# XiandaGuo/OpenStereo

Measured on NVIDIA H100. Metric: stereo_pairs_per_sec_gwcnet_256x512_d192, higher is better.
Workload: dtype f32

## Files before the change

include/openstereo_b200.h:

```cpp
#ifndef OPENSTEREO_B200_H_
#define OPENSTEREO_B200_H_

#include <stddef.h>
#include <stdint.h>

#ifdef __cplusplus
extern "C" {
#endif

#define OSB_OK 0
#define OSB_EINVAL 1
#define OSB_ECUDA 2
#define OSB_EUNSUPPORTED 3

#define OSB_ACT_NONE 0
#define OSB_ACT_RELU 1
#define OSB_ACT_LEAKY 2
#define OSB_ACT_RELU6 3

typedef void* osb_stream_t;

int osb_abi_version(void);
const char* osb_last_error(void);
uint64_t osb_launch_count(void);
int osb_tc_overflow_count(osb_stream_t stream, int reset, unsigned int* count);
int osb_tc_overflow_poll(osb_stream_t stream, unsigned int* host_pinned);
const unsigned int* osb_tc_overflow_flag(void);
float osb_set_rz_kappa(float kappa);
int osb_set_persistent_grid_cap(int cap);
const char* osb_tc_last_variant(void);
const char* osb_volume_last_variant(void);


int osb_gwc_volume_fwd(const float* ref, const float* tgt, float* out, int B, int C, int H, int W,
                       int D, int G, osb_stream_t stream);

int osb_concat_volume_fwd(const float* ref, const float* tgt, float* out, int B, int C, int H,
                          int W, int D, int mask_left, osb_stream_t stream);

int osb_gwc_concat_volume_fwd(const float* ref_gwc, const float* tgt_gwc, const float* ref_cat,
                              const float* tgt_cat, float* out, int B, int Cg, int Cc, int H, int W,
                              int D, int G, osb_stream_t stream);

int osb_corr_volume_fwd(const float* left, const float* right, float* out, int B, int C, int H,
                        int W, int D, osb_stream_t stream);


int osb_softargmin_fwd(const float* cost, float* out, int B, int D, int H, int W, float alpha,
                       float start, float step, int normalize, osb_stream_t stream);

int osb_upsample_softargmin_fwd(const float* cost, float* out, int B, int Dl, int Hl, int Wl, int D,
                                int H, int W, int align_corners, osb_stream_t stream);

int osb_upsample_softargmin_values_fwd(const float* cost, const float* values, float* out, int B, int Dl, int Hl, int Wl,
                                       int D, int H, int W, int align_corners, osb_stream_t stream);

int osb_epe_partial_fwd(const float* pred, const float* gt, float* out, int B, int HW, float maxdisp,
                        osb_stream_t stream);


int osb_conv3d_k3_bn_act_fwd(const float* x, const float* w_packed, const float* scale,
                             const float* shift, const float* residual, const float* gate, float* y,
                             int B, int Cin, int Cout, int D, int H, int W, int stride, int act,
                             osb_stream_t stream);

int osb_deconv3d_bn_act_fwd(const float* x, const float* w_packed, const float* scale,
                            const float* shift, const float* residual, float* y, int B, int Cin,
                            int Cout, int D, int H, int W, int kernel, int act, osb_stream_t stream);

int osb_conv3d_1x1_bn_act_fwd(const float* x0, const float* x1, int Cin0, const float* w_packed,
                              const float* scale, const float* shift, const float* residual,
                              const float* gate, float* y, int B, int Cin, int Cout, int D, int H,
                              int W, int act, int sigmoid_out, osb_stream_t stream);


int osb_conv3d_tc_supported(int Cin, int Cout, int W, int stride);
#define OSB_TC_MIN_WIDTH 24
int osb_tc_general_width(int W);
int osb_conv3d_tc_kc(int Cin, int Cout, int W, int stride);
int osb_conv3d_k3_tc_fwd(const float* x_ndhwc, const void* w_split, const float* scale, const float* shift,
                         const float* residual, float* y, int B, int Cin, int Cout, int D, int H, int W, int act,
                         int out_ndhwc, int res_ndhwc, osb_stream_t stream);
int osb_conv3d_k3_tc_gate_fwd(const float* x_ndhwc, const void* w_split, const float* scale, const float* shift,
                              const float* residual, const float* gate_nhwc, float* y, int B, int Cin, int Cout, int D, int H, int W,
                              int act, osb_stream_t stream);
int osb_conv3d_k3_tc_ncdhw_fwd(const float* x_ncdhw, const void* w_split, const float* scale, const float* shift,
                               const float* residual, float* y, int B, int Cin, int Cout, int D, int H, int W, int act,
                               int out_ndhwc, int res_ndhwc, osb_stream_t stream);
#define OSB_LAYOUT_NCDHW 0
#define OSB_LAYOUT_NDHWC 1
#define OSB_LAYOUT_SPLIT 2
int osb_ncdhw_to_split(const float* x, float* y_split, int B, int C, int D, int H, int W, osb_stream_t stream);
int osb_conv3d_k3_tc_split_fwd(const float* x, const void* w_split, const float* scale, const float* shift, const float* residual,
                               float* y, int B, int Cin, int Cout, int D, int H, int W, int act, int in_layout, int out_layout,
                               int res_layout, osb_stream_t stream);
int osb_conv3d_s2_tc_supported(int Cin, int Cout, int D, int H, int W);
int osb_conv3d_k3_s2_tc_fwd(const float* x_ndhwc, const void* w_split, const float* scale, const float* shift,
                            const float* residual, float* y, int B, int Cin, int Cout, int D, int H, int W, int act,
                            int out_ndhwc, int res_ndhwc, osb_stream_t stream);
int osb_deconv3d_tc_supported(int Cin, int Cout, int W);
int osb_deconv3d_k3_tc_fwd(const float* x_ndhwc, const void* w_split, const float* scale, const float* shift,
                           const float* residual, float* y, int B, int Cin, int Cout, int D, int H, int W, int act,
                           int out_ndhwc, int res_ndhwc, osb_stream_t stream);
int osb_deconv3d_k4_tc_supported(int Cin, int Cout, int W);
int osb_deconv3d_k4_tc_fwd(const float* x_ndhwc, const void* w_split, const float* scale, const float* shift,
                           const float* residual, float* y, int B, int Cin, int Cout, int cout_real, int D, int H, int W, int act,
                           int out_ndhwc, int res_ndhwc, osb_stream_t stream);
int osb_conv3d_k3_tc_cs_fwd(const float* x_ndhwc, const void* w_split, const float* scale, const float* shift, const float* residual,
                            const float* gate_nhwc, float* y, int B, int Cin, int Cout, int D, int H, int W, int act, int ystride,
                            osb_stream_t stream);
int osb_conv3d_k3_s2_tc_cs_fwd(const float* x_ndhwc, const void* w_split, const float* scale, const float* shift, float* y, int B,
                               int Cin, int Cout, int D, int H, int W, int act, int ystride, osb_stream_t stream);
int osb_deconv3d_k4_tc_cs_fwd(const float* x_ndhwc, const void* w_split, const float* scale, const float* shift, float* y, int B,
                              int Cin, int Cout, int D, int H, int W, int act, int ystride, osb_stream_t stream);
int osb_conv1x1_ndhwc_cat_fwd(const float* x0, const float* x1, int C0, int C1, const float* w_packed, const float* scale,
                              const float* shift, float* y, long long voxels, int Cout, int act, osb_stream_t stream);
int osb_conv1x1_ndhwc_fwd(const float* x, const float* w_packed, const float* scale, const float* shift, float* y,
                          long long voxels, int Cin, int Cout, int act, osb_stream_t stream);
int osb_conv3d_k3_c1_ndhwc_fwd(const float* x_ndhwc, const float* w_taps, const float* scale, const float* shift, float* y, int B,
                               int Cin, int D, int H, int W, osb_stream_t stream);
int osb_conv2d_tc_kc(int Cin, int Cout, int W, int dilation);
int osb_conv2d_k3_tc_fwd(const float* x_nhwc, const void* w_split, const float* scale, const float* shift, const float* residual,
                         float* y, int B, int Cin, int Cout, int H, int W, int dilation, int act, int out_nhwc, int res_nhwc,
                         osb_stream_t stream);
int osb_gwc_volume_sum_fwd(const float* ref, const float* tgt, float* out, int B, int C, int H, int W, int D, int G,
                           osb_stream_t stream);
int osb_group_l2_normalize_fwd(const float* x, float* y, int B, int C, int H, int W, int G, float eps, osb_stream_t stream);
int osb_sub_volume_fwd(const float* left, const float* right, float* out, int B, int C, int H, int W, int D, osb_stream_t stream);
int osb_regression_values_fwd(const float* prob, const float* values, float* out, int B, int D, int H, int W, osb_stream_t stream);

int osb_warped_concat_volume_fwd(const float* x, const float* y, const float* disp, float* out, int B, int C, int D, int H, int W,
                                 int mask_left, osb_stream_t stream);
int osb_warped_gwc_concat_volume_fwd(const float* xg, const float* yg, const float* xc, const float* yc, const float* disp,
                                     float* out, int B, int Cg, int G, int Cc, int D, int H, int W, osb_stream_t stream);

int osb_coex_regression_fwd(const float* cost, const float* spx, float* out, int B, int D, int h, int w, int top_k, int spx_is_logits,
                            osb_stream_t stream);
int osb_nearest_resize3d_fwd(const float* x, float* y, int N, int Di, int Hi, int Wi, int Do, int Ho, int Wo, osb_stream_t stream);

int osb_mbv2_block3d_fwd(const float* x, const float* w_exp, const float* scale1, const float* shift1, const float* w_dw,
                         const float* scale2, const float* shift2, const float* w_proj, const float* scale3, const float* shift3,
                         const float* residual, float* y, int B, int Cin, int Chid, int Cout, int D, int H, int W, int stride,
                         int in_layout, int out_layout, osb_stream_t stream);

int osb_gwc_volume_bwd(const float* grad_vol, const float* ref, const float* tgt, float* grad_ref, float* grad_tgt, int B, int C,
                       int H, int W, int D, int G, int reduce_sum, osb_stream_t stream);
int osb_concat_volume_bwd(const float* grad_vol, float* grad_ref, float* grad_tgt, int B, int C, int H, int W, int D, int mask_left,
                          osb_stream_t stream);
int osb_softargmin_bwd(const float* cost, const float* grad_out, float* grad_cost, int B, int D, int H, int W, float alpha,
                       float start, float step, int normalize, osb_stream_t stream);

int osb_dwconv2d_fwd(const float* x, const float* w, const float* scale, const float* shift, const float* residual, float* y, int B,
                     int C, int H, int W, int KH, int KW, int stride, int act, osb_stream_t stream);
int osb_deconv2d_k3s2_fwd(const float* x, const float* w_packed, const float* scale, const float* shift, const float* residual,
                          float* y, int B, int Cin, int Cout, int H, int W, int act, osb_stream_t stream);

int osb_avgpool_pairs_fwd(const float* x, float* y, long long outer, int n, long long inner, osb_stream_t stream);
int osb_geo_lookup_fwd(const float* geo0, const float* geo1, const float* geo2, const float* geo3, const float* corr0,
                       const float* corr1, const float* corr2, const float* corr3, const float* disp, const float* coords,
                       float* out, int B, int C, int D, int H, int W, int W2, int num_levels, int radius, osb_stream_t stream);
int osb_context_upsample_fwd(const float* disp_low, const float* up_weights, float* out, int B, int h, int w, int scale,
                             osb_stream_t stream);
int osb_ncdhw_to_ndhwc(const float* x, float* y, int B, int C, int D, int H, int W, osb_stream_t stream);
int osb_ncdhw_to_ndhwc_pad(const float* x, float* y, int B, int C, int Cpad, int D, int H, int W, osb_stream_t stream);
int osb_feature_att_gate_fwd(const float* feat_nchw, const float* w1_packed, const float* scale1, const float* shift1,
                             const float* w2_packed, const float* scale2, const float* shift2, float* gate_nhwc, int B,
                             int Cf, int Ch, int Cv, int Cpad, int HW, int act1, osb_stream_t stream);

#ifdef __cplusplus
}
#endif
#endif
```

openstereo_b200/_lib.py:

```python
import ctypes
import os

_PKG = os.path.dirname(os.path.abspath(__file__))
LIB_PATH = os.path.join(_PKG, "lib", "libopenstereo_b200.so")

_f32p = ctypes.c_void_p
_i = ctypes.c_int
_f = ctypes.c_float
_s = ctypes.c_void_p

SIGNATURES = {
    "osb_gwc_volume_fwd": [_f32p, _f32p, _f32p, _i, _i, _i, _i, _i, _i, _s],
    "osb_concat_volume_fwd": [_f32p, _f32p, _f32p, _i, _i, _i, _i, _i, _i, _s],
    "osb_gwc_concat_volume_fwd": [_f32p, _f32p, _f32p, _f32p, _f32p, _i, _i, _i, _i, _i, _i, _i, _s],
    "osb_corr_volume_fwd": [_f32p, _f32p, _f32p, _i, _i, _i, _i, _i, _s],
    "osb_softargmin_fwd": [_f32p, _f32p, _i, _i, _i, _i, _f, _f, _f, _i, _s],
    "osb_upsample_softargmin_fwd": [_f32p, _f32p, _i, _i, _i, _i, _i, _i, _i, _i, _s],
    "osb_epe_partial_fwd": [_f32p, _f32p, _f32p, _i, _i, _f, _s],
    "osb_conv3d_k3_bn_act_fwd": [_f32p] * 7 + [_i] * 8 + [_s],
    "osb_deconv3d_bn_act_fwd": [_f32p] * 6 + [_i] * 8 + [_s],
    "osb_conv3d_1x1_bn_act_fwd": [_f32p, _f32p, _i] + [_f32p] * 6 + [_i] * 8 + [_s],
    "osb_conv3d_tc_supported": [_i, _i, _i, _i],
    "osb_conv3d_tc_kc": [_i, _i, _i, _i],
    "osb_tc_general_width": [_i],
    "osb_conv3d_s2_tc_supported": [_i, _i, _i, _i, _i],
    "osb_deconv3d_tc_supported": [_i, _i, _i],
    "osb_deconv3d_k3_tc_fwd": [_f32p] * 6 + [_i] * 9 + [_s],
    "osb_conv3d_k3_s2_tc_fwd": [_f32p] * 6 + [_i] * 9 + [_s],
    "osb_conv3d_k3_tc_fwd": [_f32p] * 6 + [_i] * 9 + [_s],
    "osb_conv3d_k3_tc_ncdhw_fwd": [_f32p] * 6 + [_i] * 9 + [_s],
    "osb_conv3d_k3_tc_split_fwd": [_f32p] * 6 + [_i] * 10 + [_s],
    "osb_ncdhw_to_split": [_f32p, _f32p] + [_i] * 5 + [_s],
    "osb_conv3d_k3_tc_gate_fwd": [_f32p] * 7 + [_i] * 7 + [_s],
    "osb_deconv3d_k4_tc_supported": [_i, _i, _i],
    "osb_conv3d_k3_tc_cs_fwd": [_f32p] * 7 + [_i] * 8 + [_s],
    "osb_conv3d_k3_s2_tc_cs_fwd": [_f32p] * 5 + [_i] * 8 + [_s],
    "osb_deconv3d_k4_tc_cs_fwd": [_f32p] * 5 + [_i] * 8 + [_s],
    "osb_deconv3d_k4_tc_fwd": [_f32p] * 6 + [_i] * 10 + [_s],
    "osb_conv1x1_ndhwc_cat_fwd": [_f32p, _f32p, _i, _i, _f32p, _f32p, _f32p, _f32p, ctypes.c_longlong, _i, _i, _s],
    "osb_feature_att_gate_fwd": [_f32p] * 8 + [_i] * 7 + [_s],
    "osb_ncdhw_to_ndhwc_pad": [_f32p, _f32p, _i, _i, _i, _i, _i, _i, _s],
    "osb_conv1x1_ndhwc_fwd": [_f32p] * 5 + [ctypes.c_longlong, _i, _i, _i, _s],
    "osb_conv3d_k3_c1_ndhwc_fwd": [_f32p] * 5 + [_i] * 5 + [_s],
    "osb_avgpool_pairs_fwd": [_f32p, _f32p, ctypes.c_longlong, _i, ctypes.c_longlong, _s],
    "osb_geo_lookup_fwd": [_f32p] * 11 + [_i] * 8 + [_s],
    "osb_context_upsample_fwd": [_f32p] * 3 + [_i] * 4 + [_s],
    "osb_conv2d_tc_kc": [_i] * 4,
    "osb_conv2d_k3_tc_fwd": [_f32p] * 6 + [_i] * 9 + [_s],
    "osb_ncdhw_to_ndhwc": [_f32p, _f32p, _i, _i, _i, _i, _i, _s],
    "osb_gwc_volume_sum_fwd": [_f32p, _f32p, _f32p, _i, _i, _i, _i, _i, _i, _s],
    "osb_group_l2_normalize_fwd": [_f32p, _f32p, _i, _i, _i, _i, _i, _f, _s],
    "osb_sub_volume_fwd": [_f32p, _f32p, _f32p, _i, _i, _i, _i, _i, _s],
    "osb_regression_values_fwd": [_f32p, _f32p, _f32p, _i, _i, _i, _i, _s],
    "osb_gwc_volume_bwd": [_f32p] * 5 + [_i] * 7 + [_s],
    "osb_concat_volume_bwd": [_f32p] * 3 + [_i] * 6 + [_s],
    "osb_softargmin_bwd": [_f32p] * 3 + [_i] * 4 + [_f, _f, _f, _i, _s],
    "osb_dwconv2d_fwd": [_f32p] * 6 + [_i] * 8 + [_s],
    "osb_deconv2d_k3s2_fwd": [_f32p] * 6 + [_i] * 6 + [_s],
    "osb_upsample_softargmin_values_fwd": [_f32p] * 3 + [_i] * 8 + [_s],
    "osb_warped_concat_volume_fwd": [_f32p] * 4 + [_i] * 6 + [_s],
    "osb_warped_gwc_concat_volume_fwd": [_f32p] * 6 + [_i] * 7 + [_s],
    "osb_coex_regression_fwd": [_f32p] * 3 + [_i] * 6 + [_s],
    "osb_nearest_resize3d_fwd": [_f32p] * 2 + [_i] * 7 + [_s],
    "osb_mbv2_block3d_fwd": [_f32p] * 12 + [_i] * 10 + [_s],
}


class NativeLibraryError(RuntimeError):
    pass


def _load():
    if not os.path.exists(LIB_PATH):
        raise NativeLibraryError(
            "%s not found: build it with `python -m openstereo_b200.build` (there is no CPU/PyTorch fallback)"
            % LIB_PATH)
    lib = ctypes.CDLL(LIB_PATH)
    lib.osb_abi_version.restype = ctypes.c_int
    lib.osb_last_error.restype = ctypes.c_char_p
    lib.osb_launch_count.restype = ctypes.c_uint64
    lib.osb_tc_overflow_count.argtypes = [ctypes.c_void_p, ctypes.c_int, ctypes.POINTER(ctypes.c_uint)]
    lib.osb_tc_overflow_count.restype = ctypes.c_int
    lib.osb_tc_overflow_poll.argtypes = [ctypes.c_void_p, ctypes.c_void_p]
    lib.osb_tc_overflow_poll.restype = ctypes.c_int
    lib.osb_tc_overflow_flag.argtypes = []
    lib.osb_tc_overflow_flag.restype = ctypes.c_void_p
    lib.osb_set_rz_kappa.argtypes = [ctypes.c_float]
    lib.osb_set_rz_kappa.restype = ctypes.c_float
    lib.osb_set_persistent_grid_cap.argtypes = [ctypes.c_int]
    lib.osb_set_persistent_grid_cap.restype = ctypes.c_int
    lib.osb_tc_last_variant.argtypes = []
    lib.osb_tc_last_variant.restype = ctypes.c_char_p
    lib.osb_volume_last_variant.argtypes = []
    lib.osb_volume_last_variant.restype = ctypes.c_char_p
    for name, argtypes in SIGNATURES.items():
        try:
            fn = getattr(lib, name)
        except AttributeError as exc:
            raise NativeLibraryError("%s does not export %s" % (LIB_PATH, name)) from exc
        fn.argtypes = argtypes
        fn.restype = ctypes.c_int
    return lib


lib = _load()

_ERRORS = {1: ValueError, 2: RuntimeError, 3: NotImplementedError}


def call(name, *args):
    if len(args) != len(SIGNATURES[name]):
        raise TypeError("%s takes %d arguments (%d given)" % (name, len(SIGNATURES[name]), len(args)))
    rc = getattr(lib, name)(*args)
    if rc != 0:
# ... 7 lines not shown
```

openstereo_b200/aggregation.py:

```python
import torch

from . import ops
from .ops import ACT_LEAKY, ACT_NONE, ACT_RELU, ACT_RELU6


class _Packed:
    __slots__ = ("w", "scale", "shift", "stride", "kernel", "transposed", "cin", "cout", "_w5", "_tc")

    def __init__(self, conv, bn=None):
        self._tc = {}
        self._w5 = conv.weight.detach() if conv.weight.dim() == 5 else None
        self.cin, self.cout = (conv.in_channels, conv.out_channels)
        self.transposed = isinstance(conv, (torch.nn.ConvTranspose3d, torch.nn.ConvTranspose2d))
        self.kernel = int(conv.kernel_size[0])
        self.stride = int(conv.stride[0])
        self._validate(conv)
        wt = conv.weight
        if wt.dim() == 4:
            wt = wt.unsqueeze(2)
        if self.transposed:
            self.w = ops.pack_deconv_weight(wt)
        else:
            self.w = ops.pack_conv_weight(wt)
        if self.kernel == 1:
            self.w = self.w.reshape(self.w.shape[0], self.w.shape[2]).contiguous()
        self.scale, self.shift = (None, None)
        if bn is not None:
            if bn.training:
                raise RuntimeError("BatchNorm folding is only valid in eval mode (call model.eval())")
            self.scale, self.shift = ops.fold_bn(bn)
        if getattr(conv, "bias", None) is not None:
            bias = conv.bias.detach().float()
            self.shift = bias.contiguous() if self.shift is None else (self.shift + bias * self.scale).contiguous()


def _packed_validate(self, conv):
    ks, st = tuple(conv.kernel_size), tuple(conv.stride)
    ok = len(set(ks)) == 1 and len(set(st)) == 1 and tuple(conv.dilation) == (1,) * len(ks) and conv.groups == 1
    if self.transposed:
        op = tuple(conv.output_padding)
        ok = ok and ((ks[0] == 3 and st[0] == 2 and tuple(conv.padding) == (1,) * len(ks) and op == (1,) * len(ks))
                     or (ks[0] == 4 and st[0] == 2 and tuple(conv.padding) == (1,) * len(ks) and op == (0,) * len(ks)))
    else:
        ok = ok and ks[0] in (1, 3) and st[0] in (1, 2) and tuple(conv.padding) == (ks[0] // 2,) * len(ks)
        ok = ok and getattr(conv, "padding_mode", "zeros") == "zeros"
    if not ok:
        raise NotImplementedError("openstereo_b200: no kernel for %r (supported: Conv k1/k3, stride 1/2, padding k//2, dilation 1, "
                                  "groups 1; ConvTranspose k3 s2 p1 op1 or k4 s2 p1)" % (conv,))


_Packed._validate = _packed_validate


def _conv(layer, x, act=ACT_NONE, residual=None, gate=None):
    if layer.kernel == 1:
        return ops.conv3d_1x1(x, layer.w, layer.scale, layer.shift, residual, gate, act)
    return ops.conv3d_k3(x, layer.w, layer.scale, layer.shift, residual, gate, layer.stride, act)


USE_TENSOR_CORES = True


def _tc_weight(layer, width):
    if not USE_TENSOR_CORES or layer.transposed or layer.kernel != 3 or layer.stride != 1 or layer._w5 is None:
        return None
    kc = ops.conv3d_tc_kc(layer.cin, layer.cout, width)
    if not kc:
        return None
    if kc not in layer._tc:
        layer._tc[kc] = ops.pack_tc_weight(layer._w5, kc, pad_cout_to=16 if layer.cout < 16 else None)
    return layer._tc[kc]


def _tc_ok(layer, width):
    return _tc_weight(layer, width) is not None


def _conv_tc(layer, x_ndhwc, act=ACT_NONE, residual=None, out_ndhwc=True, res_ndhwc=True, in_ncdhw=False, out_split=False):
    wt = _tc_weight(layer, x_ndhwc.shape[4] if in_ncdhw else x_ndhwc.shape[3])
    return ops.conv3d_k3_tc(x_ndhwc, wt, layer.scale, layer.shift, residual, act, out_ndhwc, res_ndhwc, in_ncdhw,
                            out_split=out_split)


def _split_chain_ok(width, *layers):
    return USE_TENSOR_CORES and all(ops.conv3d_tc_kc(l.cin, l.cout, width) == 32 for l in layers)


def _stem_in(layer, volume, act, out_split=False):
    if ops.conv3d_tc_kc(layer.cin, layer.cout, volume.shape[-1]) == 32:
        return _conv_tc(layer, volume, act, in_ncdhw=True, out_split=out_split)
    return _conv_tc(layer, ops.to_ndhwc(volume), act)


def _conv_auto(layer, x, act=ACT_NONE, residual=None):
    if layer.stride == 1 and _tc_ok(layer, x.shape[-1]):
        return _conv_tc(layer, ops.to_ndhwc(x), act, residual, out_ndhwc=False, res_ndhwc=False)
    if (USE_TENSOR_CORES and layer.stride == 2 and layer.kernel == 3 and not layer.transposed and layer._w5 is not None
            and ops.conv3d_s2_tc_supported(layer.cin, layer.cout, x.shape[2], x.shape[3], x.shape[4])):
        if "s2" not in layer._tc:
            layer._tc["s2"] = ops.pack_tc_weight(layer._w5, 16, kw_order=(1, 0, 2))
        return ops.conv3d_k3_s2_tc(ops.to_ndhwc(x), layer._tc["s2"], layer.scale, layer.shift, residual, act)
    return _conv(layer, x, act, residual)


def _deconv(layer, x, act=ACT_NONE, residual=None):
    if (USE_TENSOR_CORES and layer.transposed and layer.kernel == 3 and layer._w5 is not None
            and ops.deconv3d_tc_supported(layer.cin, layer.cout, x.shape[-1])):
        if "dc" not in layer._tc:
            layer._tc["dc"] = ops.pack_tc_deconv_weight(layer._w5)
        return ops.deconv3d_k3_tc(ops.to_ndhwc(x), layer._tc["dc"], layer.scale, layer.shift, residual, act)
    return ops.deconv3d(x, layer.w, layer.scale, layer.shift, residual, layer.kernel, act)


def _versions(module):
    return tuple(p._version for p in module.parameters()) + tuple(b._version for b in module.buffers())


class _Engine:

    def __init__(self, module):
        self.module = module
        self._stamp = None

    def _watch(self, device):
        if USE_TENSOR_CORES:
            mon = ops.TcOverflowMonitor.get(device)
            mon.check()
            return mon
        return None

    def _ensure(self, device):
        stamp = (str(device), _versions(self.module), tuple(p.data_ptr() for p in self.module.parameters()))
        if stamp != self._stamp:
            if self.module.training:
                raise RuntimeError("openstereo_b200 engines run inference only: call model.eval()")
            with torch.no_grad():
                self._pack()
            self._stamp = stamp

    @staticmethod
    def _check(x):
        if not x.is_cuda:
            raise RuntimeError("openstereo_b200: not implemented on the CPU (no fallback); move the model to CUDA")
        return x.detach().float().contiguous()


class _GwcHourglass:
    def __init__(self, m):
        self.conv1, self.conv2 = _Packed(m.conv1[0][0], m.conv1[0][1]), _Packed(m.conv2[0][0], m.conv2[0][1])
        self.conv3, self.conv4 = _Packed(m.conv3[0][0], m.conv3[0][1]), _Packed(m.conv4[0][0], m.conv4[0][1])
        self.conv5, self.conv6 = _Packed(m.conv5[0], m.conv5[1]), _Packed(m.conv6[0], m.conv6[1])
        self.redir1, self.redir2 = _Packed(m.redir1[0], m.redir1[1]), _Packed(m.redir2[0], m.redir2[1])

    def __call__(self, x):
        c1 = _conv_auto(self.conv1, x, ACT_RELU)
        c2 = _conv_auto(self.conv2, c1, ACT_RELU)
        c3 = _conv_auto(self.conv3, c2, ACT_RELU)
        c4 = _conv_auto(self.conv4, c3, ACT_RELU)
        c5 = _deconv(self.conv5, c4, ACT_RELU, residual=_conv(self.redir2, c2))
        return _deconv(self.conv6, c5, ACT_RELU, residual=_conv(self.redir1, x))


def _hg_channels_last_ok(hg, x_shape_ndhwc):
    if not USE_TENSOR_CORES:
        return False
    b, d, h, w, c = x_shape_ndhwc
    if d % 4 or h % 4 or w % 4:
        return False
    return (ops.conv3d_s2_tc_supported(hg.conv1.cin, hg.conv1.cout, d, h, w) and _tc_ok(hg.conv2, w // 2)
            and ops.conv3d_s2_tc_supported(hg.conv3.cin, hg.conv3.cout, d // 2, h // 2, w // 2) and _tc_ok(hg.conv4, w // 4)
            and ops.deconv3d_tc_supported(hg.conv5.cin, hg.conv5.cout, w // 4)
            and ops.deconv3d_tc_supported(hg.conv6.cin, hg.conv6.cout, w // 2)
            and (hg.redir1.cin, hg.redir1.cout) in ((32, 32), (64, 64)) and (hg.redir2.cin, hg.redir2.cout) in ((32, 32), (64, 64)))


def _s2_weight(layer):
    if "s2" not in layer._tc:
        layer._tc["s2"] = ops.pack_tc_weight(layer._w5, 16, kw_order=(1, 0, 2))
    return layer._tc["s2"]


def _dc_weight(layer):
    if "dc" not in layer._tc:
        layer._tc["dc"] = ops.pack_tc_deconv_weight(layer._w5)
    return layer._tc["dc"]


def _gwc_hourglass_channels_last(hg, x):
    c1 = ops.conv3d_k3_s2_tc(x, _s2_weight(hg.conv1), hg.conv1.scale, hg.conv1.shift, None, ACT_RELU, out_ndhwc=True)
    c2 = _conv_tc(hg.conv2, c1, ACT_RELU)
    c3 = ops.conv3d_k3_s2_tc(c2, _s2_weight(hg.conv3), hg.conv3.scale, hg.conv3.shift, None, ACT_RELU, out_ndhwc=True)
    c4 = _conv_tc(hg.conv4, c3, ACT_RELU)
    r2 = ops.conv1x1_ndhwc(c2, hg.redir2.w, hg.redir2.scale, hg.redir2.shift)
    c5 = ops.deconv3d_k3_tc(c4, _dc_weight(hg.conv5), hg.conv5.scale, hg.conv5.shift, r2, ACT_RELU, out_ndhwc=True, res_ndhwc=True)
    r1 = ops.conv1x1_ndhwc(x, hg.redir1.w, hg.redir1.scale, hg.redir1.shift)
    return ops.deconv3d_k3_tc(c5, _dc_weight(hg.conv6), hg.conv6.scale, hg.conv6.shift, r1, ACT_RELU, out_ndhwc=True, res_ndhwc=True)


def _classif3_channels_last(classif3, out):
    head0, cls = classif3
    width = out.shape[3]
    if _tc_ok(cls, width):
        mid = _conv_tc(head0, out, ACT_RELU, out_split=_split_chain_ok(width, head0, cls))
        return _conv_tc(cls, mid, ACT_NONE, out_ndhwc=False, res_ndhwc=False)
    if cls.cin == 32 and cls.cout == 1 and cls._w5 is not None and cls.stride == 1:
        if "c1" not in cls._tc:
            cls._tc["c1"] = ops.pack_c1_weight(cls._w5)
        head = _conv_tc(head0, out, ACT_RELU)
        return ops.conv3d_k3_c1_ndhwc(head, cls._tc["c1"], cls.scale, cls.shift)
    head = _conv_tc(head0, out, ACT_RELU, out_ndhwc=False)
    return _conv(cls, head)


class GwcAggregation(_Engine):

    def _pack(self):
        m = self.module
        self.dres0 = [_Packed(m.dres0[0][0], m.dres0[0][1]), _Packed(m.dres0[2][0], m.dres0[2][1])]
        self.dres1 = [_Packed(m.dres1[0][0], m.dres1[0][1]), _Packed(m.dres1[2][0], m.dres1[2][1])]
        self.hg = [_GwcHourglass(m.dres2), _GwcHourglass(m.dres3), _GwcHourglass(m.dres4)]
        self.classif3 = [_Packed(m.classif3[0][0], m.classif3[0][1]), _Packed(m.classif3[2])]

    def logits(self, volume):
        volume = self._check(volume)
        self._ensure(volume.device)
        width = volume.shape[-1]
        stem_tc = all(_tc_ok(l, width) for l in (self.dres0[0], self.dres0[1], self.dres1[0], self.dres1[1]))
        b, _, dd, hh, ww = volume.shape
        if stem_tc and _tc_ok(self.classif3[0], width) and all(_hg_channels_last_ok(hg, (b, dd, hh, ww, 32)) for hg in self.hg):
            split = _split_chain_ok(width, self.dres0[0], self.dres0[1], self.dres1[0], self.dres1[1])
            c = _conv_tc(self.dres0[1], _stem_in(self.dres0[0], volume, ACT_RELU, out_split=split), ACT_RELU, out_split=split)
            out = _conv_tc(self.dres1[1], _conv_tc(self.dres1[0], c, ACT_RELU, out_split=split), ACT_NONE, residual=c)
            for hg in self.hg:
                out = _gwc_hourglass_channels_last(hg, out)
            return _classif3_channels_last(self.classif3, out)
        if stem_tc:
            c = _conv_tc(self.dres0[1], _stem_in(self.dres0[0], volume, ACT_RELU), ACT_RELU)
            cost0 = _conv_tc(self.dres1[1], _conv_tc(self.dres1[0], c, ACT_RELU), ACT_NONE, residual=c, out_ndhwc=False)
        else:
            c = _conv(self.dres0[1], _conv(self.dres0[0], volume, ACT_RELU), ACT_RELU)
            cost0 = _conv(self.dres1[1], _conv(self.dres1[0], c, ACT_RELU), ACT_NONE, residual=c)
        out = cost0
        for hg in self.hg:
            out = hg(out)
        if _tc_ok(self.classif3[0], width):
            head = _conv_tc(self.classif3[0], ops.to_ndhwc(out), ACT_RELU, out_ndhwc=False)
        else:
            head = _conv(self.classif3[0], out, ACT_RELU)
        return _conv(self.classif3[1], head)

    def __call__(self, volume, h, w):
        mon = self._watch(volume.device)
        out = ops.upsample_softargmin(self.logits(volume), self.module.maxdisp, h, w, align_corners=False)
        if mon is not None:
            mon.poll()
        return out


class CascadeAggregation(GwcAggregation):

    def __call__(self, cost, fine_d, fine_h, fine_w, disp_range_samples):
        mon = self._watch(cost.device)
        assert tuple(disp_range_samples.shape[1:]) == (fine_d, fine_h, fine_w)
        out = ops.upsample_softargmin_values(self.logits(cost), disp_range_samples, align_corners=False)
        if mon is not None:
            mon.poll()
        return out


class _PSMHourglass:
    def __init__(self, m):
        self.conv1, self.conv2 = _Packed(m.conv1[0], m.conv1[1]), _Packed(m.conv2[0], m.conv2[1])
        self.conv3, self.conv4 = _Packed(m.conv3[0], m.conv3[1]), _Packed(m.conv4[0], m.conv4[1])
        self.conv5, self.conv6 = _Packed(m.conv5[0], m.conv5[1]), _Packed(m.conv6[0], m.conv6[1])

    def __call__(self, x, presqu, postsqu, skip):
        out = _conv_auto(self.conv1, x, ACT_RELU)
        pre = _conv_auto(self.conv2, out, ACT_RELU, residual=postsqu)
        out = _conv_auto(self.conv4, _conv_auto(self.conv3, pre, ACT_RELU), ACT_RELU)
        post = _deconv(self.conv5, out, ACT_RELU, residual=presqu if presqu is not None else pre)
        return _deconv(self.conv6, post, ACT_NONE, residual=skip), pre, post


def _psm_hg_channels_last_ok(hg, shape_ndhwc):
    if not USE_TENSOR_CORES:
        return False
    b, d, h, w, c = shape_ndhwc
    if d % 4 or h % 4 or w % 4 or any(l._w5 is None for l in (hg.conv1, hg.conv2, hg.conv3, hg.conv4, hg.conv5, hg.conv6)):
        return False
    return (ops.conv3d_s2_tc_supported(hg.conv1.cin, hg.conv1.cout, d, h, w) and _tc_ok(hg.conv2, w // 2)
            and ops.conv3d_s2_tc_supported(hg.conv3.cin, hg.conv3.cout, d // 2, h // 2, w // 2) and _tc_ok(hg.conv4, w // 4)
            and hg.conv5.kernel == 3 and hg.conv6.kernel == 3
            and ops.deconv3d_tc_supported(hg.conv5.cin, hg.conv5.cout, w // 4)
            and ops.deconv3d_tc_supported(hg.conv6.cin, hg.conv6.cout, w // 2))


def _psm_hourglass_channels_last(hg, x, presqu, postsqu, skip):
    out = ops.conv3d_k3_s2_tc(x, _s2_weight(hg.conv1), hg.conv1.scale, hg.conv1.shift, None, ACT_RELU, out_ndhwc=True)
    pre = _conv_tc(hg.conv2, out, ACT_RELU, residual=postsqu)
    out = ops.conv3d_k3_s2_tc(pre, _s2_weight(hg.conv3), hg.conv3.scale, hg.conv3.shift, None, ACT_RELU, out_ndhwc=True)
    out = _conv_tc(hg.conv4, out, ACT_RELU)
    post = ops.deconv3d_k3_tc(out, _dc_weight(hg.conv5), hg.conv5.scale, hg.conv5.shift, presqu if presqu is not None else pre, ACT_RELU,
                              out_ndhwc=True, res_ndhwc=True)
    out = ops.deconv3d_k3_tc(post, _dc_weight(hg.conv6), hg.conv6.scale, hg.conv6.shift, skip, ACT_NONE, out_ndhwc=True, res_ndhwc=True)
    return out, pre, post


class PSMAggregation(_Engine):

    def _pack(self):
        m = self.module
        self.dres0 = [_Packed(m.dres0[0][0], m.dres0[0][1]), _Packed(m.dres0[1][0], m.dres0[1][1])]
        self.dres1 = [_Packed(m.dres1[0][0], m.dres1[0][1]), _Packed(m.dres1[1][0], m.dres1[1][1])]
        self.hg = [_PSMHourglass(m.dres2), _PSMHourglass(m.dres3), _PSMHourglass(m.dres4)]
        self.heads = [[_Packed(c[0][0], c[0][1]), _Packed(c[1])] for c in (m.classif1, m.classif2, m.classif3)]

    def logits(self, raw_cost):
        raw_cost = self._check(raw_cost)
        self._ensure(raw_cost.device)
        width = raw_cost.shape[-1]
        stem_tc = all(_tc_ok(l, width) for l in (self.dres0[0], self.dres0[1], self.dres1[0], self.dres1[1]))
        b, _, dd, hh, ww = raw_cost.shape
        if (stem_tc and all(_psm_hg_channels_last_ok(hg, (b, dd, hh, ww, 32)) for hg in self.hg)
                and all(_tc_ok(a, width) and _tc_ok(bb, width) for a, bb in self.heads)):
            c = _conv_tc(self.dres0[1], _stem_in(self.dres0[0], raw_cost, ACT_RELU), ACT_RELU)
            cost0 = _conv_tc(self.dres1[1], _conv_tc(self.dres1[0], c, ACT_RELU), ACT_NONE, residual=c)
            out1, pre1, post1 = _psm_hourglass_channels_last(self.hg[0], cost0, None, None, cost0)
            out2, pre2, post2 = _psm_hourglass_channels_last(self.hg[1], out1, pre1, post1, cost0)
            out3, _, _ = _psm_hourglass_channels_last(self.hg[2], out2, pre2, post2, cost0)
            costs, prev = [], None
            for (a, bb), x in zip(self.heads, (out1, out2, out3)):
                prev = _conv_tc(bb, _conv_tc(a, x, ACT_RELU), ACT_NONE, residual=prev, out_ndhwc=False, res_ndhwc=False)
                costs.append(prev)
            return costs
        if stem_tc:
            c = _conv_tc(self.dres0[1], _stem_in(self.dres0[0], raw_cost, ACT_RELU), ACT_RELU)
            cost0 = _conv_tc(self.dres1[1], _conv_tc(self.dres1[0], c, ACT_RELU), ACT_NONE, residual=c, out_ndhwc=False)
        else:
            c = _conv(self.dres0[1], _conv(self.dres0[0], raw_cost, ACT_RELU), ACT_RELU)
            cost0 = _conv(self.dres1[1], _conv(self.dres1[0], c, ACT_RELU), ACT_NONE, residual=c)
        out1, pre1, post1 = self.hg[0](cost0, None, None, cost0)
        out2, pre2, post2 = self.hg[1](out1, pre1, post1, cost0)
        out3, pre3, post3 = self.hg[2](out2, pre2, post2, cost0)

        def head(i, x, prev):
            a, b = self.heads[i]
            if _tc_ok(a, width) and _tc_ok(b, width):
                return _conv_tc(b, _conv_tc(a, ops.to_ndhwc(x), ACT_RELU), ACT_NONE, residual=prev, out_ndhwc=False, res_ndhwc=False)
            if _tc_ok(a, width):
                return _conv(b, _conv_tc(a, ops.to_ndhwc(x), ACT_RELU, out_ndhwc=False), residual=prev)
            return _conv(b, _conv(a, x, ACT_RELU), residual=prev)

        cost1 = head(0, out1, None)
        cost2 = head(1, out2, cost1)
        cost3 = head(2, out3, cost2)
        return [cost1, cost2, cost3]

    def __call__(self, raw_cost):
        b, c, d, h, w = raw_cost.shape
        max_disp = self.module.max_disp
        mon = self._watch(raw_cost.device)
        out = [ops.upsample_softargmin(cost, max_disp, 4 * h, 4 * w, align_corners=True)
               for cost in self.logits(raw_cost)]
        if mon is not None:
            mon.poll()
        return out


class _FeatureAtt:
    def __init__(self, m):
        blk = m.feat_att[0].block
        self.a = _Packed(blk[0], blk[1])
        self.b = _Packed(m.feat_att[1])
        self.act = ACT_LEAKY if any(isinstance(l, torch.nn.LeakyReLU) for l in blk) else ACT_NONE

    def __call__(self, feat):
        hidden = ops.conv3d_1x1(feat, self.a.w, self.a.scale, self.a.shift, act=ACT_LEAKY)
        return ops.conv3d_1x1(hidden, self.b.w, self.b.scale, self.b.shift, sigmoid_out=True)


def _block(m):
    layers = list(m.block)
    bn = layers[1] if len(layers) > 1 and isinstance(layers[1], torch.nn.BatchNorm3d) else None
# ... 509 lines not shown
```

openstereo_b200/csrc/api.cu:

```cuda
#include <atomic>
#include <cstdarg>
#include <cstring>

#include "common.cuh"

namespace osb {

static thread_local char g_error[512] = "";
static std::atomic<uint64_t> g_launches{0};

void set_error(const char* fmt, ...) {
  va_list ap;
  va_start(ap, fmt);
  vsnprintf(g_error, sizeof(g_error), fmt, ap);
  va_end(ap);
}

static std::atomic<float> g_rz_kappa{1.57e-8f};
float rz_kappa() { return g_rz_kappa.load(std::memory_order_relaxed); }

static std::atomic<int> g_grid_cap{0};
long long cap_persistent_grid(long long grid) {
  const int cap = g_grid_cap.load(std::memory_order_relaxed);
  return (cap > 0 && grid > cap) ? cap : grid;
// ... 18 lines not shown
  unsigned int* fresh = nullptr;
  if (cudaMalloc(&fresh, sizeof(unsigned int)) != cudaSuccess || cudaMemset(fresh, 0, sizeof(unsigned int)) != cudaSuccess) {
    set_error("tc_overflow_flag: %s", cudaGetErrorString(cudaGetLastError()));
    return nullptr;
  }
  unsigned int* expected = nullptr;
  if (!g_overflow[dev].compare_exchange_strong(expected, fresh, std::memory_order_acq_rel)) {
    (void)cudaFree(fresh);
    return expected;
  }
  return fresh;
}

int device_index() {
  int dev = 0;
  if (cudaGetDevice(&dev) != cudaSuccess) {
    (void)cudaGetLastError();
    return 0;
  }
  return dev;
}

int sm_count() {
  static std::atomic<int> cache[64];
  const int dev = device_index();
  int n = cache[dev & 63].load(std::memory_order_relaxed);
  if (n > 0) return n;
  if (cudaDeviceGetAttribute(&n, cudaDevAttrMultiProcessorCount, dev) != cudaSuccess || n <= 0) {
    (void)cudaGetLastError();
    n = 132;
  }
  cache[dev & 63].store(n, std::memory_order_relaxed);
  return n;
}

void count_launch(int n) { g_launches.fetch_add((uint64_t)n, std::memory_order_relaxed); }

int check_launch(const char* what) {
  cudaError_t e = cudaGetLastError();
  if (e == cudaSuccess) return OSB_OK;
  set_error("%s: launch failed: %s", what, cudaGetErrorString(e));
  return OSB_ECUDA;
}

typedef CUresult (*EncodeTiledFn)(CUtensorMap*, CUtensorMapDataType, cuuint32_t, void*, const cuuint64_t*,
                                  const cuuint64_t*, const cuuint32_t*, const cuuint32_t*, CUtensorMapInterleave,
                                  CUtensorMapSwizzle, CUtensorMapL2promotion, CUtensorMapFloatOOBfill);

static EncodeTiledFn encode_fn() {
  static EncodeTiledFn fn = [] {
    void* p = nullptr;
    cudaDriverEntryPointQueryResult q;
    cudaError_t e = cudaGetDriverEntryPoint("cuTensorMapEncodeTiled", &p, cudaEnableDefault, &q);
    if (e != cudaSuccess || q != cudaDriverEntryPointSuccess) {
      (void)cudaGetLastError();
      return (EncodeTiledFn) nullptr;
    }
    return reinterpret_cast<EncodeTiledFn>(p);
  }();
  return fn;
}

bool make_tensor_map_3d(CUtensorMap* out, const void* base, uint64_t d0, uint64_t d1, uint64_t d2, uint64_t stride1_bytes,
                        uint64_t stride2_bytes, uint32_t box0, uint32_t box1, uint32_t box2) {
  EncodeTiledFn fn = encode_fn();
  if (!fn) {
    set_error("cuTensorMapEncodeTiled not available from the driver");
    return false;
  }
  const cuuint64_t dims[3] = {d0, d1, d2};
  const cuuint64_t strides[2] = {stride1_bytes, stride2_bytes};
  const cuuint32_t box[3] = {box0, box1, box2};
  const cuuint32_t elem[3] = {1, 1, 1};
  CUresult r = fn(out, CU_TENSOR_MAP_DATA_TYPE_FLOAT32, 3, const_cast<void*>(base), dims, strides, box, elem,
                  CU_TENSOR_MAP_INTERLEAVE_NONE, CU_TENSOR_MAP_SWIZZLE_NONE, CU_TENSOR_MAP_L2_PROMOTION_L2_128B,
                  CU_TENSOR_MAP_FLOAT_OOB_FILL_NONE);
  if (r != CUDA_SUCCESS) {
    set_error("cuTensorMapEncodeTiled failed with CUresult %d", (int)r);
    return false;
  }
  return true;
}

bool make_tensor_map_split(CUtensorMap* out, const void* base, int C, int W, int H, int BD, int kc) {
  EncodeTiledFn fn = encode_fn();
  if (!fn) {
    set_error("cuTensorMapEncodeTiled not available from the driver");
    return false;
  }
  const uint64_t vox = 2ull * C * sizeof(uint16_t);
  const cuuint64_t dims[4] = {2ull * C, (cuuint64_t)W, (cuuint64_t)H, (cuuint64_t)BD};
  const cuuint64_t strides[3] = {vox, vox * W, vox * W * H};
  const cuuint32_t box[4] = {2u * kc, (cuuint32_t)W, 1, 1};
  const cuuint32_t elem[4] = {1, 1, 1, 1};
  CUresult r = fn(out, CU_TENSOR_MAP_DATA_TYPE_FLOAT16, 4, const_cast<void*>(base), dims, strides, box, elem,
                  CU_TENSOR_MAP_INTERLEAVE_NONE, kc == 32 ? CU_TENSOR_MAP_SWIZZLE_128B : CU_TENSOR_MAP_SWIZZLE_64B,
                  CU_TENSOR_MAP_L2_PROMOTION_L2_128B, CU_TENSOR_MAP_FLOAT_OOB_FILL_NONE);
  if (r != CUDA_SUCCESS) {
    set_error("cuTensorMapEncodeTiled (split activations) failed with CUresult %d", (int)r);
    return false;
  }
  return true;
}

}

extern "C" {
int osb_abi_version(void) { return 1; }
const char* osb_last_error(void) { return osb::g_error; }
uint64_t osb_launch_count(void) { return osb::g_launches.load(std::memory_order_relaxed); }
float osb_set_rz_kappa(float kappa) {
  const float old = osb::g_rz_kappa.load(std::memory_order_relaxed);
  if (kappa >= 0.f && kappa < 1e-6f) osb::g_rz_kappa.store(kappa, std::memory_order_relaxed);
  return old;
}
int osb_set_persistent_grid_cap(int cap) { return osb::g_grid_cap.exchange(cap > 0 ? cap : 0, std::memory_order_relaxed); }
const char* osb_tc_last_variant(void) { return osb::g_tc_variant; }
int osb_tc_overflow_count(osb_stream_t stream, int reset, unsigned int* count) {
  using namespace osb;
  OSB_REQUIRE(count, "tc_overflow_count: null pointer");
  unsigned int* flag = tc_overflow_flag();
  if (!flag) return OSB_ECUDA;
  cudaStream_t st = (cudaStream_t)stream;
  cudaError_t e = cudaMemcpyAsync(count, flag, sizeof(unsigned int), cudaMemcpyDeviceToHost, st);
  if (e == cudaSuccess && reset) e = cudaMemsetAsync(flag, 0, sizeof(unsigned int), st);
  if (e == cudaSuccess) e = cudaStreamSynchronize(st);
  if (e != cudaSuccess) {
    set_error("tc_overflow_count: %s", cudaGetErrorString(e));
    return OSB_ECUDA;
  }
  return OSB_OK;
}
const unsigned int* osb_tc_overflow_flag(void) { return osb::tc_overflow_flag(); }
int osb_tc_overflow_poll(osb_stream_t stream, unsigned int* host_pinned) {
  using namespace osb;
  OSB_REQUIRE(host_pinned, "tc_overflow_poll: null pointer");
  unsigned int* flag = tc_overflow_flag();
  if (!flag) return OSB_ECUDA;
  cudaError_t e = cudaMemcpyAsync(host_pinned, flag, sizeof(unsigned int), cudaMemcpyDeviceToHost, (cudaStream_t)stream);
  if (e != cudaSuccess) {
    set_error("tc_overflow_poll: %s", cudaGetErrorString(e));
    return OSB_ECUDA;
  }
  return OSB_OK;
}
}
```

openstereo_b200/csrc/common.cuh:

```cuda
#pragma once
#include <cuda.h>
#include <cuda_runtime.h>
#include <stdint.h>
#include <stdio.h>

#include <string>

#include "../../include/openstereo_b200.h"

namespace osb {

void set_error(const char* fmt, ...);
void count_launch(int n = 1);
int check_launch(const char* what);
int device_index();
int sm_count();
long long cap_persistent_grid(long long grid);
std::string tc_variant_name(const char* fmt, ...);
void set_tc_variant(const char* name);
struct PerDeviceFlag {
  bool done[64] = {};
  bool& here() { return done[device_index() & 63]; }
};

#define OSB_REQUIRE(cond, ...)          \
  do {                                  \
    if (!(cond)) {                      \
      ::osb::set_error(__VA_ARGS__);    \
      return OSB_EINVAL;                \
    }                                   \
  } while (0)

__device__ __forceinline__ uint32_t smem_u32(const void* p) {
  return static_cast<uint32_t>(__cvta_generic_to_shared(p));
}

__device__ __forceinline__ void mbar_init(uint64_t* bar, uint32_t count) {
  asm volatile("mbarrier.init.shared::cta.b64 [%0], %1;" ::"r"(smem_u32(bar)), "r"(count));
}
__device__ __forceinline__ void fence_mbar_init() {
  asm volatile("fence.mbarrier_init.release.cluster;" ::: "memory");
}
__device__ __forceinline__ void fence_proxy_async() {
  asm volatile("fence.proxy.async.shared::cta;" ::: "memory");
}
__device__ __forceinline__ void mbar_arrive_expect_tx(uint64_t* bar, uint32_t bytes) {
  asm volatile("mbarrier.arrive.expect_tx.shared::cta.b64 _, [%0], %1;" ::"r"(smem_u32(bar)), "r"(bytes)
               : "memory");
}
__device__ __forceinline__ void mbar_wait(uint64_t* bar, uint32_t parity) {
  asm volatile(
      "{\n"
      ".reg .pred p;\n"
      "WAIT_LOOP:\n"
      "mbarrier.try_wait.parity.shared::cta.b64 p, [%0], %1;\n"
      "@p bra DONE;\n"
      "bra WAIT_LOOP;\n"
      "DONE:\n"
      "}\n" ::"r"(smem_u32(bar)),
      "r"(parity)
      : "memory");
}
__device__ __forceinline__ void tma_load_3d(void* smem_dst, const CUtensorMap* map, uint64_t* bar, int c0,
                                            int c1, int c2) {
  asm volatile(
      "cp.async.bulk.tensor.3d.shared::cluster.global.mbarrier::complete_tx::bytes [%0], [%1, {%3, %4, %5}], [%2];"
      ::"r"(smem_u32(smem_dst)),
      "l"(reinterpret_cast<uint64_t>(map)), "r"(smem_u32(bar)), "r"(c0), "r"(c1), "r"(c2)
      : "memory");
}
__device__ __forceinline__ void tma_load_4d(void* smem_dst, const CUtensorMap* map, uint64_t* bar, int c0, int c1, int c2, int c3) {
  asm volatile(
      "cp.async.bulk.tensor.4d.shared::cluster.global.mbarrier::complete_tx::bytes [%0], [%1, {%3, %4, %5, %6}], [%2];"
      ::"r"(smem_u32(smem_dst)),
      "l"(reinterpret_cast<uint64_t>(map)), "r"(smem_u32(bar)), "r"(c0), "r"(c1), "r"(c2), "r"(c3)
      : "memory");
}
__device__ __forceinline__ void tma_prefetch_desc(const CUtensorMap* map) {
  asm volatile("prefetch.tensormap [%0];" ::"l"(reinterpret_cast<uint64_t>(map)) : "memory");
}

__device__ __forceinline__ void st_cs_f4(float* p, float4 v) { __stcs(reinterpret_cast<float4*>(p), v); }

bool make_tensor_map_3d(CUtensorMap* out, const void* base, uint64_t d0, uint64_t d1, uint64_t d2, uint64_t stride1_bytes,
                        uint64_t stride2_bytes, uint32_t box0, uint32_t box1, uint32_t box2);
bool make_tensor_map_split(CUtensorMap* out, const void* base, int C, int W, int H, int BD, int kc);

}
```

openstereo_b200/csrc/conv3d_tc.cu:

```cuda
#include <type_traits>

#include "tc_common.cuh"

namespace osb {

constexpr int TC_W = 128;
constexpr int TC_KC = 32;
constexpr int TC_TILES = TC_WGS;
constexpr int TC_ROWS = TC_TILES + 2;
constexpr int TC_STAGES = 4;
constexpr int TC_RAW = 2;
constexpr int TC_ROW_BYTES = TC_W * TC_KC * 4;

struct TcParams {
  CUtensorMap xmap;
  const float* x;
  const void* w;
  const float* scale;
  const float* shift;
  const float* residual;
  float* y;
  int B, D, H, Cin, Cout;
  int act;
  float kappa;
// ... 283 lines not shown
          const int din = d + kd - 1;
          if (din < 0 || din >= p.D) continue;
          for (int ch = 0; ch < nchunk; ++ch, ++phc) {
            for (int kh = 0; kh < 3; ++kh) {
              const uint32_t slot = (phc & 1) * 3 + kh;
              const size_t slice = ((size_t)kd * nchunk + ch) * 3 + kh;
              mbar_wait_relaxed(&b_empty[slot], ((phc >> 1) & 1) ^ 1);
              mbar_arrive_expect_tx(&b_full[slot], B_SLICE);
              bulk_g2s(b_buf + slot * B_SLICE, wsrc + slice * B_SLICE, B_SLICE, &b_full[slot]);
            }
          }
        }
      }
    }
    else if (warp == 4 * TC_WGS + 5 && p.bulk_rows && elect_one()) {
      RowIter ld{(int)blockIdx.x, 0, 0, -1};
      if (ld.it < p.items) ld.kd = (((ld.it / p.hblocks) % p.D) == 0) ? 1 : 0;
      uint32_t rawc = 0;
      while (advance(ld)) {
        const int hb = ld.it % p.hblocks;
        const int d = (ld.it / p.hblocks) % p.D;
        const int b = ld.it / (p.hblocks * p.D);
        const int hin = hb * TC_TILES - 1 + ld.r, din = d + ld.kd - 1;
        const uint32_t slot = rawc % TC_RAW, par = (rawc / TC_RAW) & 1;
        mbar_wait_relaxed(&raw_empty[slot], par ^ 1);
        if (hin >= 0 && hin < p.H && p.in_ncdhw) {
          const size_t plane = (size_t)p.D * p.H * TC_W;
          const float* src = p.x + (((size_t)b * p.Cin + ld.ch * TC_KC) * p.D + din) * p.H * TC_W + (size_t)hin * TC_W;
          mbar_arrive_expect_tx(&raw_full[slot], TC_ROW_BYTES);
          for (int c = 0; c < TC_KC; ++c)
            bulk_g2s(raw_buf + slot * TC_ROW_BYTES + c * (TC_W * 4), src + c * plane, TC_W * 4, &raw_full[slot]);
        } else if (hin >= 0 && hin < p.H) {
          const float* src = p.x + (((size_t)b * p.D + din) * p.H + hin) * (size_t)(TC_W * TC_KC);
          mbar_arrive_expect_tx(&raw_full[slot], TC_ROW_BYTES);
          bulk_g2s(raw_buf + slot * TC_ROW_BYTES, src, TC_ROW_BYTES, &raw_full[slot]);
        } else {
          mbar_arrive(&raw_full[slot]);
        }
        ++rawc;
      }
    }
    __syncwarp();
  }
}

__global__ void __launch_bounds__(256) ncdhw_to_ndhwc_kernel(const float* __restrict__ x, float* __restrict__ y, int C, int Cp,
                                                             size_t vol, uint16_t* __restrict__ ys, unsigned int* overflow) {
  __shared__ float tile[32][33];
  const int b = blockIdx.z;
  const size_t v0 = (size_t)blockIdx.x * 32;
  const int c0 = blockIdx.y * 32;
  const int tx = threadIdx.x & 31, ty = threadIdx.x >> 5;
  float amax = 0.f;
  for (int i = ty; i < 32; i += 8) {
    const int c = c0 + i;
    const size_t v = v0 + tx;
    tile[i][tx] = (c < C && v < vol) ? __ldg(x + ((size_t)b * C + c) * vol + v) : 0.f;
  }
  __syncthreads();
  for (int i = ty; i < 32; i += 8) {
    const size_t v = v0 + i;
    const int c = c0 + tx;
    if (c >= Cp || v >= vol) continue;
    if (!ys) {
      y[((size_t)b * vol + v) * Cp + c] = tile[tx][i];
      continue;
    }
    const float s = tile[tx][i] * TC_ACT_SCALE;
    const uint32_t hl = cvt_f16x2_sat(s, s - f16x2_to_float2(cvt_f16x2_sat(s, 0.f)).x);
    uint16_t* vox = ys + ((size_t)b * vol + v) * 2 * Cp;
    vox[split_index(c)] = (uint16_t)(hl & 0xFFFFu);
    vox[split_index(c) + SPLIT_GRANULE] = (uint16_t)(hl >> 16);
    amax = fmaxf(amax, fabsf(s));
  }
  if (ys) tc_report_overflow(overflow, amax);
}

template <int COUT>
int launch_tc(const TcArgs& a, cudaStream_t stream) {
  TcParams p{};
  p.Cout = a.Cout, p.in_ncdhw = a.in_ncdhw;
  p.in_split = a.in_split, p.out_split = a.out_split, p.res_split = a.res_split;
  p.bulk_rows = !a.in_split && (a.in_ncdhw || a.Cin == TC_KC);
  if (a.in_split && !make_tensor_map_split(&p.xmap, a.x, a.Cin, TC_W, a.H, a.B * a.D, TC_KC)) return OSB_ECUDA;
  p.hblocks = (a.H + TC_TILES - 1) / TC_TILES;
  static const std::string variant = tc_variant_name("tc<%d>", COUT);
  return launch_persistent<conv3d_tc_kernel<COUT>>(a, p, (long long)a.B * a.D * p.hblocks, TcCfg<COUT>::SMEM, variant.c_str(), stream);
}
template int launch_tc<32>(const TcArgs&, cudaStream_t);
template int launch_tc<16>(const TcArgs&, cudaStream_t);

}

extern "C" {

int osb_tc_general_width(int W) { return W >= OSB_TC_MIN_WIDTH ? 1 : 0; }

int osb_conv3d_tc_kc(int Cin, int Cout, int W, int stride) {
  return stride == 1 ? osb::select_conv3d_tc(Cin, Cout, W, 1, false, false).kc : 0;
}

int osb_conv3d_tc_supported(int Cin, int Cout, int W, int stride) { return osb_conv3d_tc_kc(Cin, Cout, W, stride) != 0; }

int osb_ncdhw_to_ndhwc_pad(const float* x, float* y, int B, int C, int Cpad, int D, int H, int W, osb_stream_t stream) {
  using namespace osb;
  OSB_REQUIRE(x && y, "ncdhw_to_ndhwc: null pointer");
  OSB_REQUIRE(B > 0 && C > 0 && Cpad >= C && D > 0 && H > 0 && W > 0 && B <= 65535, "ncdhw_to_ndhwc: bad shape");
  const size_t vol = (size_t)D * H * W;
  dim3 grid((unsigned)((vol + 31) / 32), (Cpad + 31) / 32, B);
  ncdhw_to_ndhwc_kernel<<<grid, 256, 0, (cudaStream_t)stream>>>(x, y, C, Cpad, vol, nullptr, nullptr);
  count_launch();
  return check_launch("ncdhw_to_ndhwc_kernel");
}

int osb_ncdhw_to_split(const float* x, float* y_split, int B, int C, int D, int H, int W, osb_stream_t stream) {
  using namespace osb;
  OSB_REQUIRE(x && y_split, "ncdhw_to_split: null pointer");
  OSB_REQUIRE(B > 0 && C > 0 && C % SPLIT_GRANULE == 0 && D > 0 && H > 0 && W > 0 && B <= 65535,
              "ncdhw_to_split: bad shape (C must be a multiple of %d)", SPLIT_GRANULE);
  unsigned int* flag = tc_overflow_flag();
  if (!flag) return OSB_ECUDA;
  const size_t vol = (size_t)D * H * W;
  dim3 grid((unsigned)((vol + 31) / 32), (C + 31) / 32, B);
  ncdhw_to_ndhwc_kernel<<<grid, 256, 0, (cudaStream_t)stream>>>(x, nullptr, C, C, vol, reinterpret_cast<uint16_t*>(y_split), flag);
  count_launch();
  return check_launch("ncdhw_to_ndhwc_kernel");
}

int osb_ncdhw_to_ndhwc(const float* x, float* y, int B, int C, int D, int H, int W, osb_stream_t stream) {
  return osb_ncdhw_to_ndhwc_pad(x, y, B, C, C, D, H, W, stream);
}

static int conv3d_k3_tc_impl(osb::TcArgs a, int dilation, osb_stream_t stream) {
  using namespace osb;
  const int kc = select_conv3d_tc(a.Cin, a.Cout, a.W, dilation, false, false).kc;
  OSB_REQUIRE(kc, "conv3d_k3_tc: unsupported shape Cin=%d Cout=%d W=%d dilation=%d", a.Cin, a.Cout, a.W, dilation);
  OSB_REQUIRE(!a.in_ncdhw || kc == 32, "conv3d_k3_tc: NCDHW input is served by the W = 128 kernel only");
  OSB_REQUIRE((!a.ystride && !a.gate) || kc == 16, "conv3d_k3_tc: a channel slice or gate needs the 16-channel-chunk kernels");
  OSB_REQUIRE(a.Cout > 16 || (!a.out_ndhwc && (!a.residual || !a.res_ndhwc)), "conv3d_k3_tc: Cout <= 16 writes (and adds) NCDHW tensors only");
  OSB_REQUIRE(!(a.in_split || a.out_split || a.res_split) || (kc == 32 && !a.ystride && !a.gate),
              "conv3d_k3_tc: split activations are served by the W = 128 kernel only");
  OSB_REQUIRE(!a.in_split || !a.in_ncdhw, "conv3d_k3_tc: an input is either NCDHW or split");
  OSB_REQUIRE((!a.out_split || a.out_ndhwc) && (!a.res_split || a.res_ndhwc), "conv3d_k3_tc: split tensors are channels-last");
  OSB_REQUIRE(!(a.out_split || a.res_split) || (a.out_ndhwc && (!a.residual || a.res_ndhwc)),
              "conv3d_k3_tc: a split output or residual needs a channels-last output and residual");
  const TcLaunch launch = select_conv3d_tc(a.Cin, a.Cout, a.W, dilation, a.gate != nullptr, a.slice()).launch;
  const int rc = check_tc_args("conv3d_k3_tc", a, launch);
  return rc != OSB_OK ? rc : launch(a, (cudaStream_t)stream);
}

int osb_conv3d_k3_tc_fwd(const float* x_ndhwc, const void* w_split, const float* scale, const float* shift,
                         const float* residual, float* y, int B, int Cin, int Cout, int D, int H, int W, int act,
                         int out_ndhwc, int res_ndhwc, osb_stream_t stream) {
  return conv3d_k3_tc_impl({x_ndhwc, w_split, scale, shift, residual, nullptr, y, B, Cin, Cout, D, H, W, act, out_ndhwc, res_ndhwc, 0, 0,
                            Cout}, 1, stream);
}

int osb_conv3d_k3_tc_gate_fwd(const float* x_ndhwc, const void* w_split, const float* scale, const float* shift,
                              const float* residual, const float* gate_nhwc, float* y, int B, int Cin, int Cout, int D, int H, int W,
                              int act, osb_stream_t stream) {
  OSB_REQUIRE(gate_nhwc, "conv3d_k3_tc_gate: null gate");
  return conv3d_k3_tc_impl({x_ndhwc, w_split, scale, shift, residual, gate_nhwc, y, B, Cin, Cout, D, H, W, act, 1, 1, 0, 0, Cout}, 1,
                           stream);
}

int osb_conv3d_k3_tc_cs_fwd(const float* x_ndhwc, const void* w_split, const float* scale, const float* shift, const float* residual,
                            const float* gate_nhwc, float* y, int B, int Cin, int Cout, int D, int H, int W, int act, int ystride,
                            osb_stream_t stream) {
  return conv3d_k3_tc_impl({x_ndhwc, w_split, scale, shift, residual, gate_nhwc, y, B, Cin, Cout, D, H, W, act, 1, 1, 0, ystride, Cout},
                           1, stream);
}

int osb_conv3d_k3_tc_ncdhw_fwd(const float* x_ncdhw, const void* w_split, const float* scale, const float* shift,
                               const float* residual, float* y, int B, int Cin, int Cout, int D, int H, int W, int act,
                               int out_ndhwc, int res_ndhwc, osb_stream_t stream) {
  return conv3d_k3_tc_impl({x_ncdhw, w_split, scale, shift, residual, nullptr, y, B, Cin, Cout, D, H, W, act, out_ndhwc, res_ndhwc, 1, 0,
                            Cout}, 1, stream);
}

int osb_conv3d_k3_tc_split_fwd(const float* x, const void* w_split, const float* scale, const float* shift, const float* residual,
                               float* y, int B, int Cin, int Cout, int D, int H, int W, int act, int in_layout, int out_layout,
                               int res_layout, osb_stream_t stream) {
  auto known = [](int l) { return l == OSB_LAYOUT_NCDHW || l == OSB_LAYOUT_NDHWC || l == OSB_LAYOUT_SPLIT; };
  OSB_REQUIRE(known(in_layout) && known(out_layout) && known(res_layout), "conv3d_k3_tc_split: unknown layout");
  osb::TcArgs a{x, w_split, scale, shift, residual, nullptr, y, B, Cin, Cout, D, H, W, act, out_layout != OSB_LAYOUT_NCDHW, res_layout != OSB_LAYOUT_NCDHW,
                in_layout == OSB_LAYOUT_NCDHW, 0, Cout};
  a.in_split = in_layout == OSB_LAYOUT_SPLIT, a.out_split = out_layout == OSB_LAYOUT_SPLIT, a.res_split = res_layout == OSB_LAYOUT_SPLIT;
  return conv3d_k3_tc_impl(a, 1, stream);
}

int osb_conv2d_tc_kc(int Cin, int Cout, int W, int dilation) { return osb::select_conv3d_tc(Cin, Cout, W, dilation, false, false).kc; }

int osb_conv2d_k3_tc_fwd(const float* x_nhwc, const void* w_split, const float* scale, const float* shift, const float* residual,
                         float* y, int B, int Cin, int Cout, int H, int W, int dilation, int act, int out_nhwc, int res_nhwc,
                         osb_stream_t stream) {
  return conv3d_k3_tc_impl({x_nhwc, w_split, scale, shift, residual, nullptr, y, B, Cin, Cout, 1, H, W, act, out_nhwc, res_nhwc, 0, 0,
                            Cout}, dilation, stream);
}
}
```

openstereo_b200/csrc/conv3d_tcg.cu:

```cuda
#include "tc_common.cuh"

namespace osb {

struct TcgParams {
  const float* x;
  const void* w;
  const float* scale;
  const float* shift;
  const float* residual;
  const float* gate;
  float* y;
  int B, D, H, Cin;
  int act;
  float kappa;
  unsigned int* overflow;
  int out_ndhwc, res_ndhwc;
  int items, hblocks;
  int Wr, ctiles;
  int ystride;
};

template <int COUT, int KC, int W, int TILES, int DIL = 1, bool GW = false>
struct TcgCfg {
  static_assert(!GW || W == 128, "general-width tiles are 128-column segments of one image row");
  static constexpr int HALO = GW ? DIL : 0;
  static constexpr int CSTEP = 128 - 2 * HALO;
  static_assert(DIL == 1 || (W == 128 && DIL == 2 && COUT >= 64), "dilation 2 is instantiated for full-width rows only");
  static constexpr int R = 128 / W;
  static constexpr int ROWB = KC * 4;
  static constexpr int UNIT_BYTES = 128 * ROWB;
  static constexpr int N3 = 3 * COUT;
  static constexpr int G = 32;
  static constexpr int NG = COUT / G;
  static constexpr int NG3 = 3 * G;
  static constexpr int B_SLICE = N3 * ROWB;
  static constexpr int B_SUB = NG3 * ROWB;
  static constexpr int NT = TC_WGS * TILES;
  static constexpr int TS = R * DIL;
  static constexpr int HSPAN = NT * TS;
  __host__ __device__ static constexpr int row0(int hb) { return (hb / DIL) * HSPAN + (hb % DIL) * R; }
  __host__ static int hblocks(int H) { return DIL * ((H + HSPAN - 1) / HSPAN); }
  static constexpr int NLW = 4;
  static constexpr int XCHG_FLOATS = 2 * frag_xchg_floats<G, DIL>();
  static constexpr int FIXED_SMEM = 1024 + TC_BSLOTS * 3 * B_SUB + 1024 + TC_WGS * XCHG_FLOATS * 4 + 4 * TC_WGS * FRAG_TP_FLOATS * 4 +
                                    2 * COUT * 4;
  static constexpr int STAGES = (232448 - FIXED_SMEM) / UNIT_BYTES < 10 ? (232448 - FIXED_SMEM) / UNIT_BYTES : 10;
  static_assert(STAGES >= NLW, "the ring must hold at least one unit per loader warp");
  static constexpr int S_FIRST = -DIL;
  static constexpr int S_LAST = (NT - 1) * TS + DIL;
  static constexpr int KSTEPS = KC / 16;
  static constexpr int A_OFF = 0;
  static constexpr int B_OFF = A_OFF + STAGES * UNIT_BYTES;
  static constexpr int BAR_OFF = B_OFF + TC_BSLOTS * 3 * B_SUB;
  static constexpr int THREADS = TC_WG_THREADS;
  static constexpr size_t SMEM = 1024 + (size_t)BAR_OFF + 1024 + TC_WGS * XCHG_FLOATS * 4 + 4 * TC_WGS * FRAG_TP_FLOATS * 4 + 2 * COUT * 4;
  static_assert(SMEM <= 232448, "shared memory budget of one CTA exceeded");
  static_assert(TILES == 1, "a consumer warpgroup holds one accumulator tile");
  static_assert(DIL == 1 || R == 1, "interleaved row blocks assume one image row per tile");
  static_assert(COUT % G == 0, "output channels come in groups of 32");
  static_assert(B_SUB % 1024 == 0 && UNIT_BYTES % 1024 == 0, "operand tiles must stay 1024-byte aligned");
  static constexpr int tile_of(int s, int kh) {
    const int num = s - (kh - 1) * DIL;
    return (num >= 0 && num % TS == 0 && num / TS < NT) ? num / TS : -1;
  }
  static constexpr bool used(int s) { return tile_of(s, 0) >= 0 || tile_of(s, 1) >= 0 || tile_of(s, 2) >= 0; }
  static constexpr int units_per_phase() {
    int n = 0;
    for (int s = S_FIRST; s <= S_LAST; ++s) n += used(s) ? 1 : 0;
    return n;
  }
  static constexpr int NU = units_per_phase();
  static constexpr int unit_s(int j) {
    int k = 0;
    for (int s = S_FIRST; s <= S_LAST; ++s)
      if (used(s)) {
        if (k == j) return s;
        ++k;
      }
    return S_LAST;
  }
};

template <int COUT, int KC, int W, int TILES, int DIL = 1, bool GW = false, bool GATE = false>
__global__ void __launch_bounds__(TcgCfg<COUT, KC, W, TILES, DIL, GW>::THREADS, 1) conv3d_tcg_kernel(const TcgParams p) {
  using C = TcgCfg<COUT, KC, W, TILES, DIL, GW>;
  extern __shared__ __align__(1024) uint8_t smem_raw[];
  uint8_t* smem = reinterpret_cast<uint8_t*>((reinterpret_cast<uintptr_t>(smem_raw) + 1023) & ~static_cast<uintptr_t>(1023));
  uint8_t* a_buf = smem + C::A_OFF;
  uint8_t* b_buf = smem + C::B_OFF;
  uint64_t* bars = reinterpret_cast<uint64_t*>(smem + C::BAR_OFF);
  uint64_t* a_ready = bars;
  uint64_t* a_empty = a_ready + C::STAGES;
  uint64_t* b_full = a_empty + C::STAGES;
  uint64_t* b_empty = b_full + TC_BSLOTS * 3;
  float* xchg = reinterpret_cast<float*>(smem + C::BAR_OFF + 1024);
  float* tiles = xchg + TC_WGS * C::XCHG_FLOATS;
  float* s_scale = tiles + 4 * TC_WGS * FRAG_TP_FLOATS;
  float* s_shift = s_scale + COUT;

  const int warp = threadIdx.x >> 5, lane = threadIdx.x & 31;
  const int nchunk = p.Cin / KC;
  const int Wp = GW ? p.Wr : W;
  const int YS = (W < 32 && p.ystride) ? p.ystride : COUT;
  const int ctiles = GW ? p.ctiles : 1;

  if (threadIdx.x == 0) {
    for (int s = 0; s < C::STAGES; ++s) {
      mbar_init(&a_ready[s], 32);
      mbar_init(&a_empty[s], 4 * TC_WGS);
    }
    for (int k = 0; k < TC_BSLOTS * 3; ++k) {
      mbar_init(&b_full[k], 1);
      mbar_init(&b_empty[k], 4 * TC_WGS);
    }
    fence_mbar_init();
  }
  for (int c = threadIdx.x; c < COUT; c += blockDim.x) {
    s_scale[c] = p.scale ? p.scale[c] : 1.f;
    s_shift[c] = p.shift ? p.shift[c] : 0.f;
  }
  __syncthreads();

  if (warp < 4 * TC_WGS) {
    setmaxnreg_inc<TC_CONSUMER_REGS>();
    const int wg = warp >> 2;
    xchg += wg * C::XCHG_FLOATS;
    const int bar_xchg = 1 + wg;
    const uint64_t dbase = (KC == 32) ? desc_sw128_base() : desc_sw64_base();
    constexpr uint32_t A_HALF = 64 * C::ROWB / 16;
    const uint32_t b16 = (smem_u32(b_buf) & 0x3FFFF) >> 4;
    const int q = warp & 3;
    uint32_t unitc = 0, phc = 0, exc = 0;
    for (int it = blockIdx.x; it < p.items; it += gridDim.x) {
      const int cg = (it % C::NG) * C::G;
      const int it0 = it / C::NG;
      const int ct = it0 % ctiles;
      const int hb = (it0 / ctiles) % p.hblocks;
      const int d = (it0 / (ctiles * p.hblocks)) % p.D;
      const int b = it0 / (ctiles * p.hblocks * p.D);
      auto tile_row = [&](int m, int& h, int& col) {
        h = C::row0(hb) + wg * C::TS + m / W;
        col = GW ? ct * C::CSTEP - C::HALO + m : m % W;
        return h < p.H && (!GW || (m >= C::HALO && m < 128 - C::HALO && col < Wp));
      };
      {
        int h, col;
        if (tile_row(q * 32 + lane, h, col)) {
          const ptrdiff_t vox = (((ptrdiff_t)b * p.D + d) * p.H + h) * Wp + col;
          if (p.residual && p.res_ndhwc) asm volatile("prefetch.global.L2 [%0];" ::"l"(p.residual + vox * YS + cg));
          if (GATE && p.gate) asm volatile("prefetch.global.L2 [%0];" ::"l"(p.gate + (((ptrdiff_t)b * p.H + h) * Wp + col) * YS + cg));
        }
      }
      float acc[2][C::NG3 / 2];
      uint32_t accum = 0;
      for (int kd = 0; kd < 3; ++kd) {
        const int din = d + kd - 1;
        if (din < 0 || din >= p.D) continue;
        for (int ch = 0; ch < nchunk; ++ch, ++phc) {
#pragma unroll
          for (int s = C::S_FIRST; s <= C::S_LAST; ++s) {
            if (!C::used(s)) continue;
            const uint32_t slot = unitc % C::STAGES, par = (unitc / C::STAGES) & 1;
            mbar_wait(&a_ready[slot], par);
            const uint64_t da0 = dbase | (uint64_t)((smem_u32(a_buf + slot * C::UNIT_BYTES) & 0x3FFFF) >> 4);
#pragma unroll
            for (int kh = 0; kh < 3; ++kh) {
              if (C::tile_of(s, kh) != wg) continue;
              const uint32_t bslot = (phc & 1) * 3 + kh;
              mbar_wait(&b_full[bslot], (phc >> 1) & 1);
              const uint64_t db0 = dbase | (uint64_t)(b16 + (bslot * C::B_SUB) / 16);
              wg_fence();
#pragma unroll
              for (int ks = 0; ks < C::KSTEPS; ++ks)
                wg_mma_split<C::NG3>(acc, da0 + TcK<KC>::A_KSTEP * ks, A_HALF, TcK<KC>::A_LO, db0 + 2 * ks, TcK<KC>::B_LO, ks > 0 ? 1u : accum);
              wg_commit();
              wg_wait_all();
              accum = 1;
              wg_release(&b_empty[bslot], lane);
            }
            wg_release(&a_empty[slot], lane);
            ++unitc;
          }
        }
      }
      const float corr = 1.f + p.kappa * (float)(((d > 0) + 1 + (d + 1 < p.D)) * nchunk * 3 * C::KSTEPS * 3);
      frag_unshift<C::G, DIL, W>(acc, xchg + (exc & 1) * (C::XCHG_FLOATS / 2), q, lane, corr, bar_xchg);
      ++exc;
      const size_t plane = (size_t)p.D * p.H * Wp;
      auto rows = [&](int m, ptrdiff_t& yo, ptrdiff_t& ro, ptrdiff_t& go) {
        int h, col;
        const bool ok = tile_row(m, h, col);
        const ptrdiff_t vox = (((ptrdiff_t)b * p.D + d) * p.H + h) * Wp + col;
        const ptrdiff_t ncdhw = (ptrdiff_t)b * COUT * plane + ((ptrdiff_t)d * p.H + h) * Wp + col;
        yo = p.out_ndhwc ? vox * YS : ncdhw;
        ro = p.res_ndhwc ? vox * YS : ncdhw;
        go = (((ptrdiff_t)b * p.H + h) * Wp + col) * YS;
        return ok;
      };
      frag_epilogue<C::G>(acc, lane, q, tiles + warp * FRAG_TP_FLOATS, s_scale + cg, s_shift + cg, p.act, p.y + (p.out_ndhwc ? (size_t)cg : cg * plane),
                          p.out_ndhwc ? 1 : plane, p.residual ? p.residual + (p.res_ndhwc ? (size_t)cg : cg * plane) : nullptr,
                          p.res_ndhwc ? 1 : plane, (GATE && p.gate) ? p.gate + cg : nullptr, rows, C::G);
    }
  }
  else if (warp < 4 * TC_WGS + C::NLW) {
    setmaxnreg_dec<TC_LOADER_REGS>();
    const int lw = warp - 4 * TC_WGS;
    static_assert(KC == 16, "lane_voxel / unit-row mapping below is written for 64-byte operand rows");
    constexpr int CPR = KC / 4;
    constexpr int VPL = 32 / CPR;
    constexpr int NLD = 128 / VPL;
    static_assert(W % VPL == 0, "a load instruction must not straddle image rows");
    const int v0 = lane_voxel<KC>(lane), c = lane % CPR;
    float amax = 0.f;
    uint32_t ubase = 0;
    int first = lw;
    auto fill = [&](const float* base, size_t rstride, size_t cstride, int h_first, int h_step, uint32_t u, int col0) {
      float4 v[NLD];
#pragma unroll
      for (int j = 0; j < NLD; ++j) {
        const int hin = h_first + h_step * ((VPL * j) / W);
        const size_t off = (size_t)((VPL * j) / W) * rstride + (size_t)((VPL * j) % W) * cstride;
        bool ok = hin >= 0 && hin < p.H;
        if (GW) ok = ok && (unsigned)(col0 + VPL * j) < (unsigned)Wp;
        v[j] = ok ? __ldg(reinterpret_cast<const float4*>(base + (ptrdiff_t)off)) : make_float4(0.f, 0.f, 0.f, 0.f);
      }
      const uint32_t slot = u % C::STAGES, ph = (u / C::STAGES) & 1;
      mbar_wait_relaxed(&a_empty[slot], ph ^ 1);
      uint8_t* tile = a_buf + slot * C::UNIT_BYTES;
#pragma unroll
      for (int j = 0; j < NLD; ++j) stage_f16_split<KC>(tile, v0 + VPL * j, c, v[j], amax);
      fence_proxy_async();
      mbar_arrive(&a_ready[slot]);
    };
    for (int it = blockIdx.x; it < p.items; it += gridDim.x) {
      const int it0 = it / C::NG;
      const int ct = it0 % ctiles;
      const int hb = (it0 / ctiles) % p.hblocks;
      const int d = (it0 / (ctiles * p.hblocks)) % p.D;
      const int b = it0 / (ctiles * p.hblocks * p.D);
      const int h0 = C::row0(hb);
      const int col0 = ct * C::CSTEP - C::HALO + v0;
      for (int kd = 0; kd < 3; ++kd) {
        const int din = d + kd - 1;
        if (din < 0 || din >= p.D) continue;
        const float* plane = p.x + ((size_t)b * p.D + din) * p.H * (size_t)Wp * p.Cin;
        for (int ch = 0; ch < nchunk; ++ch) {
#pragma unroll 1
          for (int j = first; j < C::NU; j += C::NLW) {
            const int s = C::unit_s(j);
            const float* base = plane + ((ptrdiff_t)(h0 + s) * Wp + col0) * p.Cin + ch * KC + c * 4;
            fill(base, (size_t)Wp * p.Cin, (size_t)p.Cin, h0 + s, 1, ubase + j, col0);
          }
          ubase += C::NU;
          first = (first + C::NLW - C::NU % C::NLW) % C::NLW;
        }
      }
    }
    tc_report_overflow(p.overflow, amax);
  }
  else {
    setmaxnreg_dec<TC_PRODUCER_REGS>();
    if (warp == 4 * TC_WGS + C::NLW && elect_one()) {
      const uint8_t* wsrc = reinterpret_cast<const uint8_t*>(p.w);
      uint32_t phc = 0;
      for (int it = blockIdx.x; it < p.items; it += gridDim.x) {
        const int cg = (it % C::NG) * C::G;
        const int d = (it / C::NG / (ctiles * p.hblocks)) % p.D;
        for (int kd = 0; kd < 3; ++kd) {
          const int din = d + kd - 1;
          if (din < 0 || din >= p.D) continue;
          for (int ch = 0; ch < nchunk; ++ch, ++phc) {
            for (int kh = 0; kh < 3; ++kh) {
              const uint32_t slot = (phc & 1) * 3 + kh;
              const size_t slice = ((size_t)kd * nchunk + ch) * 3 + kh;
              mbar_wait_relaxed(&b_empty[slot], ((phc >> 1) & 1) ^ 1);
              mbar_arrive_expect_tx(&b_full[slot], C::B_SUB);
#pragma unroll
              for (int kw = 0; kw < 3; ++kw)
                bulk_g2s(b_buf + slot * C::B_SUB + kw * C::G * C::ROWB, wsrc + slice * C::B_SLICE + (size_t)(kw * COUT + cg) * C::ROWB,
                         C::G * C::ROWB, &b_full[slot]);
            }
          }
        }
      }
    }
    __syncwarp();
  }
}

template <int COUT, int KC, int W, int TILES, int DIL = 1, bool GW = false, bool GATE = false>
static int launch_tcg(const TcArgs& a, cudaStream_t stream) {
  using C = TcgCfg<COUT, KC, W, TILES, DIL, GW>;
  TcgParams p{};
  p.gate = a.gate, p.ystride = a.ystride;
  p.hblocks = C::hblocks(a.H);
  p.Wr = GW ? a.W : W;
  p.ctiles = GW ? (a.W + C::CSTEP - 1) / C::CSTEP : 1;
  static const std::string variant = tc_variant_name("tcg<%d,%d,%d,%d,%d,%d,%d>", COUT, KC, W, TILES, DIL, (int)GW, (int)GATE);
  return launch_persistent<conv3d_tcg_kernel<COUT, KC, W, TILES, DIL, GW, GATE>>(
      a, p, (long long)a.B * a.D * p.hblocks * p.ctiles * C::NG, C::SMEM, variant.c_str(), stream);
}

TcRoute select_conv3d_tc(int Cin, int Cout, int W, int dilation, bool gate, bool slice) {
  if (dilation == 1 && W == 128 && Cin % 32 == 0 && Cin >= 32 && !gate && !slice) {
    if (Cout == 32) return {launch_tc<32>, 32};
    if (Cout >= 1 && Cout <= 16) return {launch_tc<16>, 32};
  }
  if (Cin % 16 != 0 || Cin < 16) return {};
  if (dilation == 2)
    return (W == 128 && Cout == 128 && !gate && !slice) ? TcRoute{launch_tcg<128, 16, 128, 1, 2>, 16} : TcRoute{};
  if (dilation != 1) return {};
  if (W == 16) {
    if (Cout == 96) return {launch_tcg<96, 16, 16, 1, 1, false, true>, 16};
    if (Cout == 64) return {launch_tcg<64, 16, 16, 1, 1, false, true>, 16};
    return {};
  }
  if (slice) return {};
  if (gate) {
    if (W == 64 && Cout == 64) return {launch_tcg<64, 16, 64, 1, 1, false, true>, 16};
    if (W == 32 && Cout == 96) return {launch_tcg<96, 16, 32, 1, 1, false, true>, 16};
    return {};
  }
  if (W == 64 && Cout == 64) return {launch_tcg<64, 16, 64, 1>, 16};
  if (W == 32 && Cout == 64) return {launch_tcg<64, 16, 32, 1>, 16};
  if (W == 32 && Cout == 128) return {launch_tcg<128, 16, 32, 1>, 16};
  if (W == 32 && Cout == 96) return {launch_tcg<96, 16, 32, 1>, 16};
  if (W == 128 && Cout == 64) return {launch_tcg<64, 16, 128, 1>, 16};
  if (W == 128 && Cout == 128) return {launch_tcg<128, 16, 128, 1>, 16};
  if (!osb_tc_general_width(W)) return {};
  if (Cout == 32) return {launch_tcg<32, 16, 128, 1, 1, true>, 16};
  if (Cout == 64) return {launch_tcg<64, 16, 128, 1, 1, true>, 16};
  if (Cout == 128) return {launch_tcg<128, 16, 128, 1, 1, true>, 16};
  return {};
}

}
```

openstereo_b200/csrc/conv3d_tcs2.cu:

```cuda
#include "tc_common.cuh"

namespace osb {

struct Tcs2Params {
  const float* x;
  const void* w;
  const float* scale;
  const float* shift;
  const float* residual;
  float* y;
  int B, D, H, Cin;
  int act;
  float kappa;
  unsigned int* overflow;
  int out_ndhwc, res_ndhwc;
  int items, hblocks;
  int Wr, ctiles;
  int ystride;
};

template <int COUT, int KC, int W, int TILES, bool GW = false>
struct Tcs2Cfg {
  static_assert(!GW || W == 128, "general-width tiles are 128-column segments of one output row");
  static constexpr int HALO = GW ? 1 : 0;
  static constexpr int CSTEP = 128 - HALO;
  static constexpr int R = 128 / W;
  static constexpr int ROWB = KC * 4;
  static constexpr int UNIT_BYTES = 128 * ROWB;
  static constexpr int N3 = 3 * COUT;
  static constexpr int G = 32;
  static constexpr int NG = COUT / G;
  static constexpr int NP = (NG + TC_WGS - 1) / TC_WGS;
  static constexpr int B_SLICE = N3 * ROWB;
  static constexpr int B_SUB = 3 * G * ROWB;
  static constexpr int B_SLOT = TC_WGS * B_SUB;
  static constexpr int PC = 16;
  static constexpr int NPASS = G / PC;
  static constexpr int LD = 3 * PC + 4;
  static constexpr int XCHG_FLOATS = 2 * 4 * PC;
  static constexpr int NLW = 4;
  static constexpr int FIXED_SMEM = 1024 + TC_BSLOTS * 3 * B_SLOT + TC_WGS * 128 * LD * 4 + 1024 + TC_WGS * XCHG_FLOATS * 4 + 3 * COUT * 4;
  static constexpr int STAGES = (232448 - FIXED_SMEM) / UNIT_BYTES < 10 ? (232448 - FIXED_SMEM) / UNIT_BYTES : 10;
  static_assert(STAGES >= NLW, "the ring must hold at least one unit per loader warp");
  static constexpr int NU = TILES * 3 * 2;
  static constexpr int HBLK = TILES * R;
  static constexpr int KSTEPS = KC / 16;
  static constexpr int A_OFF = 0;
  static constexpr int B_OFF = A_OFF + STAGES * UNIT_BYTES;
  static constexpr int STAGE_OFF = B_OFF + TC_BSLOTS * 3 * B_SLOT;
  static constexpr int BAR_OFF = STAGE_OFF + TC_WGS * 128 * LD * 4;
  static constexpr int THREADS = TC_WG_THREADS;
  static constexpr size_t SMEM = 1024 + (size_t)BAR_OFF + 1024 + TC_WGS * XCHG_FLOATS * 4 + 3 * COUT * 4;
  static_assert(SMEM <= 232448, "shared memory budget of one CTA exceeded");
  static_assert(TILES == 1, "a consumer warpgroup holds one accumulator tile");
  static_assert(COUT % G == 0, "output channels come in groups of 32");
  static_assert(32 * LD >= TP_WARP_FLOATS, "store_ndhwc_chunk32 transposes through the warp's own rows of the staging tile");
  static_assert(B_SUB % 1024 == 0 && UNIT_BYTES % 1024 == 0, "operand tiles must stay 1024-byte aligned");
};

template <int N>
__device__ __forceinline__ void s2_stage16(float* stage, int ld, const float (&acc)[2][N / 2], int c0, int dst, int wq, int lane) {
#pragma unroll
  for (int h = 0; h < 2; ++h) {
    float* r0 = stage + (64 * h + 16 * wq + (lane >> 2)) * ld + 2 * (lane & 3) + dst;
#pragma unroll
    for (int jj = 0; jj < 2; ++jj) {
      const int j = c0 / 8 + jj;
      *reinterpret_cast<float2*>(r0 + 8 * jj) = make_float2(acc[h][4 * j], acc[h][4 * j + 1]);
      *reinterpret_cast<float2*>(r0 + 8 * ld + 8 * jj) = make_float2(acc[h][4 * j + 2], acc[h][4 * j + 3]);
    }
  }
}

template <int COUT, int KC, int W, int TILES, bool GW = false>
__global__ void __launch_bounds__(Tcs2Cfg<COUT, KC, W, TILES, GW>::THREADS, 1) conv3d_tcs2_kernel(const Tcs2Params p) {
  using C = Tcs2Cfg<COUT, KC, W, TILES, GW>;
  extern __shared__ __align__(1024) uint8_t smem_raw[];
  uint8_t* smem = smem_raw + ((1024u - (smem_u32(smem_raw) & 1023u)) & 1023u);
  uint8_t* a_buf = smem + C::A_OFF;
  uint8_t* b_buf = smem + C::B_OFF;
  float* stage = reinterpret_cast<float*>(smem + C::STAGE_OFF);
  uint64_t* bars = reinterpret_cast<uint64_t*>(smem + C::BAR_OFF);
  uint64_t* a_ready = bars;
  uint64_t* a_empty = a_ready + C::STAGES;
  uint64_t* b_full = a_empty + C::STAGES;
  uint64_t* b_empty = b_full + TC_BSLOTS * 3;
  float* xchg = reinterpret_cast<float*>(smem + C::BAR_OFF + 1024);
  float* s_scale = xchg + TC_WGS * C::XCHG_FLOATS;
  float* s_shift = s_scale + COUT;
  float* zeros = s_shift + COUT;

  const int warp = threadIdx.x >> 5, lane = threadIdx.x & 31;
  const int nchunk = p.Cin / KC;
  const int Wp = GW ? p.Wr : W;
  const int YS = (W < 32 && p.ystride) ? p.ystride : COUT;
  const int ctiles = GW ? p.ctiles : 1;

  if (threadIdx.x == 0) {
    for (int s = 0; s < C::STAGES; ++s) {
      mbar_init(&a_ready[s], 32);
      mbar_init(&a_empty[s], 4 * TC_WGS);
// ... 38 lines not shown
      float acc_e[2][C::G / 2], acc_o[2][C::G];
      uint32_t accum_e = 0, accum_o = 0;
      for (int kd = 0; kd < 3; ++kd) {
        const int din = 2 * d + kd - 1;
        if (din < 0 || din >= p.D) continue;
        for (int ch = 0; ch < nchunk; ++ch, ++phc) {
#pragma unroll
          for (int kh = 0; kh < 3; ++kh) {
            const uint32_t bslot = (phc & 1) * 3 + kh;
#pragma unroll
            for (int par = 0; par < 2; ++par) {
              const uint32_t slot = unitc % C::STAGES, ph = (unitc / C::STAGES) & 1;
              mbar_wait(&a_ready[slot], ph);
              if (par == 0) mbar_wait(&b_full[bslot], (phc >> 1) & 1);
              if (has_group) {
                const uint64_t da0 = dbase | (uint64_t)((smem_u32(a_buf + slot * C::UNIT_BYTES) & 0x3FFFF) >> 4);
                const uint64_t db0 = dbase | (uint64_t)(b16 + (bslot * C::B_SLOT + wg * C::B_SUB + (par ? C::G * C::ROWB : 0)) / 16);
                wg_fence();
#pragma unroll
                for (int ks = 0; ks < C::KSTEPS; ++ks) {
                  if (par == 0) wg_mma_split<C::G>(acc_e, da0 + TcK<KC>::A_KSTEP * ks, A_HALF, TcK<KC>::A_LO, db0 + 2 * ks, TcK<KC>::B_LO, ks > 0 ? 1u : accum_e);
                  else wg_mma_split<2 * C::G>(acc_o, da0 + TcK<KC>::A_KSTEP * ks, A_HALF, TcK<KC>::A_LO, db0 + 2 * ks, TcK<KC>::B_LO, ks > 0 ? 1u : accum_o);
                }
                wg_commit();
                wg_wait_all();
                if (par == 0) accum_e = 1;
                else accum_o = 1;
              }
              wg_release(&a_empty[slot], lane);
              if (par == 1) wg_release(&b_empty[bslot], lane);
              ++unitc;
            }
          }
        }
      }
      if (!has_group) continue;
      const int h = hb * C::HBLK + rr;
      const bool live = h < Ho;
      const int col = GW ? ct * C::CSTEP - C::HALO + m : wcol;
      const bool cvalid = !GW || (m >= C::HALO && col < Wp);
      const uint32_t vmask = GW ? __ballot_sync(0xffffffffu, cvalid) : 0xffffffffu;
      const float corr = 1.f + p.kappa * (float)(((d > 0) + 1 + (2 * d + 1 < p.D)) * nchunk * 3 * C::KSTEPS * 3);
      const ptrdiff_t vox = (((ptrdiff_t)b * Do + d) * Ho + h) * Wp + col;
      const size_t plane = (size_t)Do * Ho * Wp;
      const ptrdiff_t ncdhw0 = (ptrdiff_t)b * COUT * plane + ((ptrdiff_t)d * Ho + h) * Wp + col;
      float out[32];
#pragma unroll
      for (int pass = 0; pass < C::NPASS; ++pass) {
        named_bar_sync(bar_stage, 128);
        s2_stage16<C::G>(stage, C::LD, acc_e, pass * C::PC, 0, q, lane);
        s2_stage16<2 * C::G>(stage, C::LD, acc_o, pass * C::PC, C::PC, q, lane);
        s2_stage16<2 * C::G>(stage, C::LD, acc_o, C::G + pass * C::PC, 2 * C::PC, q, lane);
        named_bar_sync(bar_stage, 128);
        const float* srow = stage + m * C::LD;
        float* xb = xchg + (exc & 1) * (4 * C::PC);
        ++exc;
        if (lane == 31) {
#pragma unroll
          for (int i = 0; i < C::PC; i += 4)
            *reinterpret_cast<float4*>(xb + q * C::PC + i) = *reinterpret_cast<const float4*>(srow + C::PC + i);
        }
        named_bar_sync(bar_xchg, 128);
        const float* xl = has_left_q ? xb + (q - 1) * C::PC : zeros;
#pragma unroll
        for (int i0 = 0; i0 < C::PC; i0 += 4) {
          const float4 l4 = *reinterpret_cast<const float4*>(xl + i0);
          const float4 p14 = *reinterpret_cast<const float4*>(srow + i0);
          const float4 p04 = *reinterpret_cast<const float4*>(srow + C::PC + i0);
          const float4 p24 = *reinterpret_cast<const float4*>(srow + 2 * C::PC + i0);
          const float le[4] = {l4.x, l4.y, l4.z, l4.w};
          const float p0[4] = {p04.x, p04.y, p04.z, p04.w}, p1[4] = {p14.x, p14.y, p14.z, p14.w}, p2[4] = {p24.x, p24.y, p24.z, p24.w};
#pragma unroll
          for (int k = 0; k < 4; ++k) {
            float left = __shfl_up_sync(0xffffffffu, p0[k], 1);
            left = (lane == 0) ? le[k] : left;
            if (W < 32) left = (wcol == 0) ? 0.f : left;
            out[pass * C::PC + i0 + k] = ((left + p1[k]) + p2[k]) * corr;
          }
        }
      }
      const uint32_t vm = (W < 32) ? __ballot_sync(0xffffffffu, live) : (live ? vmask : 0u);
      if (vm && p.out_ndhwc && (!p.residual || p.res_ndhwc)) {
        store_ndhwc_chunk32(stage + q * 32 * C::LD, lane, out, p.y + (vox - lane) * YS + cg,
                            p.residual ? p.residual + (vox - lane) * YS + cg : nullptr, YS, s_scale + cg, s_shift + cg, p.act, vm);
      } else if (live && cvalid) {
#pragma unroll
        for (int i = 0; i < 32; ++i) out[i] = fmaf(out[i], s_scale[cg + i], s_shift[cg + i]);
        if (p.residual) {
          if (p.res_ndhwc) {
            const float4* rp = reinterpret_cast<const float4*>(p.residual + vox * YS + cg);
#pragma unroll
            for (int i = 0; i < 8; ++i) {
              const float4 rv = __ldg(rp + i);
              out[4 * i] += rv.x, out[4 * i + 1] += rv.y, out[4 * i + 2] += rv.z, out[4 * i + 3] += rv.w;
            }
          } else {
#pragma unroll
            for (int i = 0; i < 32; ++i) out[i] += __ldg(p.residual + ncdhw0 + (size_t)(cg + i) * plane);
          }
        }
        if (p.act == OSB_ACT_RELU) {
#pragma unroll
          for (int i = 0; i < 32; ++i) out[i] = fmaxf(out[i], 0.f);
        } else if (p.act == OSB_ACT_LEAKY) {
#pragma unroll
          for (int i = 0; i < 32; ++i) out[i] = out[i] > 0.f ? out[i] : 0.01f * out[i];
        }
        if (p.out_ndhwc) {
          float4* yp = reinterpret_cast<float4*>(p.y + vox * YS + cg);
#pragma unroll
          for (int i = 0; i < 8; ++i) yp[i] = make_float4(out[4 * i], out[4 * i + 1], out[4 * i + 2], out[4 * i + 3]);
        } else {
#pragma unroll
          for (int i = 0; i < 32; ++i) p.y[ncdhw0 + (size_t)(cg + i) * plane] = out[i];
        }
      }
    }
  }
  else if (warp < 4 * TC_WGS + C::NLW) {
    setmaxnreg_dec<TC_LOADER_REGS>();
    const int lw = warp - 4 * TC_WGS;
    static_assert(KC == 16, "lane_voxel / unit-row mapping below is written for 64-byte operand rows");
    constexpr int CPR = KC / 4;
    constexpr int VPL = 32 / CPR;
    constexpr int NLD = 128 / VPL;
    static_assert(W % VPL == 0, "a load instruction must not straddle image rows");
    const int v0 = lane_voxel<KC>(lane), c = lane % CPR;
    float amax = 0.f;
    const int WI = 2 * Wp;
    const int Do = p.D / 2;
    uint32_t ubase = 0;
    int first = lw;
    auto fill = [&](const float* base, size_t rstride, size_t cstride, int h_first, int h_step, uint32_t u, int col0) {
      float4 v[NLD];
#pragma unroll
      for (int j = 0; j < NLD; ++j) {
        const int hin = h_first + h_step * ((VPL * j) / W);
        const size_t off = (size_t)((VPL * j) / W) * rstride + (size_t)((VPL * j) % W) * cstride;
        bool ok = hin >= 0 && hin < p.H;
        if (GW) ok = ok && (unsigned)(col0 + VPL * j) < (unsigned)Wp;
        v[j] = ok ? __ldg(reinterpret_cast<const float4*>(base + (ptrdiff_t)off)) : make_float4(0.f, 0.f, 0.f, 0.f);
      }
      const uint32_t slot = u % C::STAGES, ph = (u / C::STAGES) & 1;
      mbar_wait_relaxed(&a_empty[slot], ph ^ 1);
      uint8_t* tile = a_buf + slot * C::UNIT_BYTES;
#pragma unroll
      for (int j = 0; j < NLD; ++j) stage_f16_split<KC>(tile, v0 + VPL * j, c, v[j], amax);
      fence_proxy_async();
      mbar_arrive(&a_ready[slot]);
    };
    for (int it = blockIdx.x; it < p.items; it += gridDim.x) {
      const int it0 = it / C::NP;
      const int ct = it0 % ctiles;
      const int hb = (it0 / ctiles) % p.hblocks;
      const int od = (it0 / (ctiles * p.hblocks)) % Do;
      const int b = it0 / (ctiles * p.hblocks * Do);
      const int h0 = hb * C::HBLK;
      const int col0 = ct * C::CSTEP - C::HALO + v0;
      for (int kd = 0; kd < 3; ++kd) {
        const int din = 2 * od + kd - 1;
        if (din < 0 || din >= p.D) continue;
        const float* plane = p.x + ((size_t)b * p.D + din) * p.H * (size_t)WI * p.Cin;
        for (int ch = 0; ch < nchunk; ++ch) {
#pragma unroll 1
          for (int j = first; j < C::NU; j += C::NLW) {
            const int t = j / 6, kh = (j >> 1) % 3, par = j & 1;
            const int h_first = 2 * (h0 + t * C::R) + kh - 1;
            const float* base = plane + ((ptrdiff_t)h_first * WI + 2 * col0 + par) * p.Cin + ch * KC + c * 4;
            fill(base, (size_t)2 * WI * p.Cin, (size_t)2 * p.Cin, h_first, 2, ubase + j, col0);
          }
          ubase += C::NU;
          first = (first + C::NLW - C::NU % C::NLW) % C::NLW;
        }
      }
    }
    tc_report_overflow(p.overflow, amax);
  }
  else {
    setmaxnreg_dec<TC_PRODUCER_REGS>();
    if (warp == 4 * TC_WGS + C::NLW && elect_one()) {
      const uint8_t* wsrc = reinterpret_cast<const uint8_t*>(p.w);
      uint32_t phc = 0;
      for (int it = blockIdx.x; it < p.items; it += gridDim.x) {
        const int g0 = (it % C::NP) * TC_WGS;
        const int ngr = min(TC_WGS, C::NG - g0);
        const int od = (it / C::NP / (ctiles * p.hblocks)) % (p.D / 2);
        for (int kd = 0; kd < 3; ++kd) {
          const int din = 2 * od + kd - 1;
          if (din < 0 || din >= p.D) continue;
          for (int ch = 0; ch < nchunk; ++ch, ++phc) {
            for (int kh = 0; kh < 3; ++kh) {
              const uint32_t slot = (phc & 1) * 3 + kh;
              const size_t slice = ((size_t)kd * nchunk + ch) * 3 + kh;
              mbar_wait_relaxed(&b_empty[slot], ((phc >> 1) & 1) ^ 1);
              mbar_arrive_expect_tx(&b_full[slot], ngr * C::B_SUB);
              for (int t = 0; t < ngr; ++t)
#pragma unroll
                for (int kw = 0; kw < 3; ++kw)
                  bulk_g2s(b_buf + slot * C::B_SLOT + t * C::B_SUB + kw * C::G * C::ROWB,
                           wsrc + slice * C::B_SLICE + (size_t)(kw * COUT + (g0 + t) * C::G) * C::ROWB, C::G * C::ROWB, &b_full[slot]);
            }
          }
        }
      }
    }
    __syncwarp();
  }
}

template <int COUT, int KC, int W, int TILES, bool GW = false>
static int launch_tcs2(const TcArgs& a, cudaStream_t stream) {
  using C = Tcs2Cfg<COUT, KC, W, TILES, GW>;
  Tcs2Params p{};
  p.ystride = a.ystride;
  p.hblocks = (a.H / 2 + C::HBLK - 1) / C::HBLK;
  p.Wr = GW ? a.W / 2 : W;
  p.ctiles = GW ? (p.Wr + C::CSTEP - 1) / C::CSTEP : 1;
  static const std::string variant = tc_variant_name("tcs2<%d,%d,%d,%d,%d>", COUT, KC, W, TILES, (int)GW);
  return launch_persistent<conv3d_tcs2_kernel<COUT, KC, W, TILES, GW>>(
      a, p, (long long)a.B * (a.D / 2) * p.hblocks * p.ctiles * C::NP, C::SMEM, variant.c_str(), stream);
}

static TcLaunch select_conv3d_s2_tc(int Cin, int Cout, int D, int H, int W, bool slice) {
  if (Cin % 16 != 0 || Cin < 16 || D % 2 || H % 2 || W % 2) return nullptr;
  if (W == 32 && Cout == 96) return launch_tcs2<96, 16, 16, 1>;
  if (W == 32 && Cout == 64) return launch_tcs2<64, 16, 16, 1>;
  if (slice) return nullptr;
  if (W == 128 && Cout == 64) return launch_tcs2<64, 16, 64, 1>;
  if (W == 64 && Cout == 64) return launch_tcs2<64, 16, 32, 1>;
  if (W == 64 && Cout == 128) return launch_tcs2<128, 16, 32, 1>;
  if (W == 64 && Cout == 96) return launch_tcs2<96, 16, 32, 1>;
  if (!osb_tc_general_width(W / 2)) return nullptr;
  if (Cout == 64) return launch_tcs2<64, 16, 128, 1, true>;
  if (Cout == 128) return launch_tcs2<128, 16, 128, 1, true>;
  return nullptr;
}

static int conv3d_k3_s2_tc_impl(TcArgs a, cudaStream_t stream) {
  OSB_REQUIRE(select_conv3d_s2_tc(a.Cin, a.Cout, a.D, a.H, a.W, false), "conv3d_k3_s2_tc: unsupported shape Cin=%d Cout=%d D=%d H=%d W=%d",
              a.Cin, a.Cout, a.D, a.H, a.W);
  const TcLaunch launch = select_conv3d_s2_tc(a.Cin, a.Cout, a.D, a.H, a.W, a.slice());
  const int rc = check_tc_args("conv3d_k3_s2_tc", a, launch);
  return rc != OSB_OK ? rc : launch(a, stream);
}

}

extern "C" {

int osb_conv3d_s2_tc_supported(int Cin, int Cout, int D, int H, int W) {
  return osb::select_conv3d_s2_tc(Cin, Cout, D, H, W, false) ? 1 : 0;
}

int osb_conv3d_k3_s2_tc_fwd(const float* x_ndhwc, const void* w_split, const float* scale, const float* shift,
                            const float* residual, float* y, int B, int Cin, int Cout, int D, int H, int W, int act,
                            int out_ndhwc, int res_ndhwc, osb_stream_t stream) {
  return osb::conv3d_k3_s2_tc_impl({x_ndhwc, w_split, scale, shift, residual, nullptr, y, B, Cin, Cout, D, H, W, act, out_ndhwc, res_ndhwc,
                                    0, 0, Cout}, (cudaStream_t)stream);
}

int osb_conv3d_k3_s2_tc_cs_fwd(const float* x_ndhwc, const void* w_split, const float* scale, const float* shift, float* y, int B,
                               int Cin, int Cout, int D, int H, int W, int act, int ystride, osb_stream_t stream) {
  return osb::conv3d_k3_s2_tc_impl({x_ndhwc, w_split, scale, shift, nullptr, nullptr, y, B, Cin, Cout, D, H, W, act, 1, 1, 0, ystride,
                                    Cout}, (cudaStream_t)stream);
}
}
```

openstereo_b200/csrc/tc_common.cuh:

```cuda
#pragma once
#include "common.cuh"

namespace osb {

__device__ __forceinline__ void mbar_wait_relaxed(uint64_t* bar, uint32_t parity) {
  uint32_t done;
  for (;;) {
    asm volatile(
        "{\n.reg .pred p;\nmbarrier.try_wait.parity.shared::cta.b64 p, [%1], %2;\nselp.u32 %0, 1, 0, p;\n}\n"
        : "=r"(done)
        : "r"(smem_u32(bar)), "r"(parity)
        : "memory");
    if (done) return;
    __nanosleep(64);
  }
}
__device__ __forceinline__ void mbar_arrive(uint64_t* bar) {
  asm volatile("mbarrier.arrive.shared::cta.b64 _, [%0];" ::"r"(smem_u32(bar)) : "memory");
}
__device__ __forceinline__ uint64_t desc_sw128_base() {
  uint64_t d = 0;
  d |= (uint64_t)1 << 16;
  d |= (uint64_t)(1024 >> 4) << 32;
  d |= (uint64_t)1 << 62;
// ... 105 lines not shown
  const uint32_t n = valid ? 16u : 0u;
  asm volatile("cp.async.ca.shared.global [%0], [%1], 16, %2;" ::"r"(smem_u32(smem_dst)), "l"(gsrc), "r"(n) : "memory");
}
__device__ __forceinline__ void cp_async_commit() { asm volatile("cp.async.commit_group;" ::: "memory"); }
template <int N>
__device__ __forceinline__ void cp_async_wait() {
  asm volatile("cp.async.wait_group %0;" ::"n"(N) : "memory");
}
constexpr int TC_BSLOTS = 2;
__device__ __forceinline__ void named_bar_sync(int id, int threads) {
  asm volatile("bar.sync %0, %1;" ::"r"(id), "r"(threads) : "memory");
}
__device__ __forceinline__ void named_bar_arrive(int id, int threads) {
  asm volatile("bar.arrive %0, %1;" ::"r"(id), "r"(threads) : "memory");
}
constexpr int TC_WGS = 2;
constexpr int TC_CONSUMER_REGS = 184;
constexpr int TC_LOADER_REGS = 112;
constexpr int TC_PRODUCER_REGS = 32;
constexpr int TC_WG_THREADS = 512;
template <int N>
__device__ __forceinline__ void setmaxnreg_inc() {
  asm volatile("setmaxnreg.inc.sync.aligned.u32 %0;" ::"n"(N));
}
template <int N>
__device__ __forceinline__ void setmaxnreg_dec() {
  asm volatile("setmaxnreg.dec.sync.aligned.u32 %0;" ::"n"(N));
}
__device__ __forceinline__ bool elect_one() {
  uint32_t pred;
  asm volatile("{\n.reg .pred p;\nelect.sync _|p, 0xffffffff;\nselp.u32 %0, 1, 0, p;\n}\n" : "=r"(pred));
  return pred != 0;
}
constexpr float TC_ACT_SCALE = 16.f;
constexpr float TC_F16_MAX = 65504.f;
__device__ __forceinline__ uint32_t cvt_f16x2_sat(float a, float b) {
  uint32_t r;
  asm("cvt.rn.satfinite.f16x2.f32 %0, %1, %2;" : "=r"(r) : "f"(b), "f"(a));
  return r;
}
__device__ __forceinline__ float2 f16x2_to_float2(uint32_t h) {
  float2 f;
  asm("{\n.reg .b16 l, u;\nmov.b32 {l, u}, %2;\ncvt.f32.f16 %0, l;\ncvt.f32.f16 %1, u;\n}\n" : "=f"(f.x), "=f"(f.y) : "r"(h));
  return f;
}
__device__ __forceinline__ void f16_split4(const float4 v, uint2& hi, uint2& lo, float& amax) {
  const float x0 = v.x * TC_ACT_SCALE, x1 = v.y * TC_ACT_SCALE, x2 = v.z * TC_ACT_SCALE, x3 = v.w * TC_ACT_SCALE;
  amax = fmaxf(amax, fmaxf(fmaxf(fabsf(x0), fabsf(x1)), fmaxf(fabsf(x2), fabsf(x3))));
  hi.x = cvt_f16x2_sat(x0, x1);
  hi.y = cvt_f16x2_sat(x2, x3);
  const float2 h01 = f16x2_to_float2(hi.x), h23 = f16x2_to_float2(hi.y);
  lo.x = cvt_f16x2_sat(x0 - h01.x, x1 - h01.y);
  lo.y = cvt_f16x2_sat(x2 - h23.x, x3 - h23.y);
}
unsigned int* tc_overflow_flag();
__device__ __forceinline__ void tc_report_overflow(unsigned int* flag, float amax) {
  if (amax > TC_F16_MAX) atomicAdd(flag, 1u);
}

float rz_kappa();


template <int KC>
__device__ __forceinline__ int swz_offset(int row, int c) {
  if constexpr (KC == 32) return row * 128 + ((c ^ (row & 7)) << 4);
  else return row * 64 + ((c ^ ((row >> 1) & 3)) << 4);
}


constexpr int SPLIT_GRANULE = 16;
__device__ __forceinline__ int split_index(int c) { return (c / SPLIT_GRANULE) * 2 * SPLIT_GRANULE + c % SPLIT_GRANULE; }
__device__ __forceinline__ void split_store4(uint16_t* vox, int c, const float4 v, float& amax) {
  uint2 hi, lo;
  f16_split4(v, hi, lo, amax);
  *reinterpret_cast<uint2*>(vox + split_index(c)) = hi;
  *reinterpret_cast<uint2*>(vox + split_index(c) + SPLIT_GRANULE) = lo;
}
__device__ __forceinline__ float4 split_load4(const uint16_t* vox, int c) {
  const uint2 hi = __ldg(reinterpret_cast<const uint2*>(vox + split_index(c)));
  const uint2 lo = __ldg(reinterpret_cast<const uint2*>(vox + split_index(c) + SPLIT_GRANULE));
  const float2 h01 = f16x2_to_float2(hi.x), h23 = f16x2_to_float2(hi.y), l01 = f16x2_to_float2(lo.x), l23 = f16x2_to_float2(lo.y);
  constexpr float inv = 1.f / TC_ACT_SCALE;
  return make_float4((h01.x + l01.x) * inv, (h01.y + l01.y) * inv, (h23.x + l23.x) * inv, (h23.y + l23.y) * inv);
}

template <int KC>
__device__ __forceinline__ void stage_f16_split(uint8_t* tile, int row, int q, const float4 v, float& amax) {
  uint2 hi, lo;
  f16_split4(v, hi, lo, amax);
  const int sub = (q & 1) << 3, chunk = 4 * (q >> 2) + ((q >> 1) & 1);
  *reinterpret_cast<uint2*>(tile + swz_offset<KC>(row, chunk) + sub) = hi;
  *reinterpret_cast<uint2*>(tile + swz_offset<KC>(row, chunk + 2) + sub) = lo;
}
template <int KC>
__device__ __forceinline__ int lane_voxel(int lane) {
  if constexpr (KC == 32) return (((lane >> 3) & 1) << 1) | (lane >> 4);
  else return ((lane >> 2) & 1) | (((lane >> 3) & 1) << 2) | ((lane >> 4) << 1);
}
template <int KC>
struct TcK {
  static constexpr int KSTEPS = KC / 16;
  static constexpr int A_KSTEP = 4;
  static constexpr int A_LO = 2;
  static constexpr int B_LO = KC / 8;
};

template <int G, int DIL>
constexpr int frag_xchg_floats() { return 8 * 2 * DIL * G; }
template <int G, int DIL, int W>
__device__ __forceinline__ void frag_unshift(float (&acc)[2][3 * G / 2], float* xb, int wq, int lane, float corr, int bar) {
  constexpr int SIDE = DIL * G;
  const int l4 = lane >> 2, c0 = 2 * (lane & 3);
#pragma unroll
  for (int h = 0; h < 2; ++h) {
    float* grp = xb + (4 * h + wq) * 2 * SIDE;
    if (l4 >= 8 - DIL) {
#pragma unroll
      for (int j = 0; j < G / 8; ++j)
        *reinterpret_cast<float2*>(grp + (l4 - 8 + DIL) * G + 8 * j + c0) = make_float2(acc[h][4 * j + 2], acc[h][4 * j + 3]);
    }
    if (l4 < DIL) {
#pragma unroll
      for (int j = 0; j < G / 8; ++j)
        *reinterpret_cast<float2*>(grp + SIDE + l4 * G + 8 * j + c0) =
            make_float2(acc[h][4 * (j + G / 4)], acc[h][4 * (j + G / 4) + 1]);
    }
  }
  named_bar_sync(bar, 128);
  const int src_l = (lane - 4 * DIL) & 31, src_r = (lane + 4 * DIL) & 31;
  const bool wrap_l = l4 >= 8 - DIL, wrap_r = l4 < DIL;
#pragma unroll
  for (int h = 0; h < 2; ++h) {
    const int g = 4 * h + wq;
    const float* xl = xb + (g > 0 ? g - 1 : 0) * 2 * SIDE + (l4 < DIL ? l4 : 0) * G + c0;
    const float* xr = xb + (g < 7 ? g + 1 : 7) * 2 * SIDE + SIDE + (l4 >= 8 - DIL ? l4 - 8 + DIL : 0) * G + c0;
    const int mlo = (64 * h + 16 * wq + l4) % W, mhi = (64 * h + 16 * wq + 8 + l4) % W;
#pragma unroll
    for (int j = 0; j < G / 8; ++j) {
      const float2 sl = *reinterpret_cast<const float2*>(xl + 8 * j);
      const float2 sr = *reinterpret_cast<const float2*>(xr + 8 * j);
#pragma unroll
      for (int c2 = 0; c2 < 2; ++c2) {
        const float p0lo = acc[h][4 * j + c2], p0hi = acc[h][4 * j + 2 + c2];
        const float p2lo = acc[h][4 * (j + G / 4) + c2], p2hi = acc[h][4 * (j + G / 4) + 2 + c2];
        float llo = __shfl_sync(0xffffffffu, p0lo, src_l);
        float lhi = __shfl_sync(0xffffffffu, wrap_l ? p0lo : p0hi, src_l);
        float rlo = __shfl_sync(0xffffffffu, wrap_r ? p2hi : p2lo, src_r);
        float rhi = __shfl_sync(0xffffffffu, p2hi, src_r);
        llo = (l4 < DIL) ? (c2 ? sl.y : sl.x) : llo;
        rhi = (l4 >= 8 - DIL) ? (c2 ? sr.y : sr.x) : rhi;
        llo = (mlo < DIL) ? 0.f : llo;
        lhi = (mhi < DIL) ? 0.f : lhi;
        rlo = (mlo >= W - DIL) ? 0.f : rlo;
        rhi = (mhi >= W - DIL) ? 0.f : rhi;
        float& olo = acc[h][4 * (j + G / 8) + c2];
        float& ohi = acc[h][4 * (j + G / 8) + 2 + c2];
        olo = ((llo + olo) + rlo) * corr;
        ohi = ((lhi + ohi) + rhi) * corr;
      }
    }
  }
}
constexpr int FRAG_TP_STRIDE = 40;
constexpr int FRAG_TP_FLOATS = 16 * FRAG_TP_STRIDE;
template <int G, class Rows>
__device__ __forceinline__ void frag_epilogue(const float (&acc)[2][3 * G / 2], int lane, int wq, float* tbuf, const float* sc,
                                              const float* sh, int act, float* y, size_t ycs, const float* res, size_t rcs,
                                              const float* gate, Rows rows, int nch, bool y_split = false, bool res_split = false,
                                              unsigned int* overflow = nullptr) {
  const int c0 = 2 * (lane & 3), l4 = lane >> 2;
  if constexpr (G == 32) {
    if (ycs == 1 && (!res || rcs == 1)) {
      const int c4 = 4 * (lane & 7), sub = lane >> 3;
      const float4 a = *reinterpret_cast<const float4*>(sc + c4);
      const float4 b = *reinterpret_cast<const float4*>(sh + c4);
      float amax = 0.f;
#pragma unroll
      for (int h = 0; h < 2; ++h) {
        __syncwarp();
#pragma unroll
        for (int j = 0; j < 4; ++j)
#pragma unroll
          for (int rh = 0; rh < 2; ++rh)
            *reinterpret_cast<float2*>(tbuf + (8 * rh + l4) * FRAG_TP_STRIDE + 8 * j + c0) =
                make_float2(acc[h][4 * (j + 4) + 2 * rh], acc[h][4 * (j + 4) + 2 * rh + 1]);
        __syncwarp();
        float4 o[4];
        ptrdiff_t yo[4], ro[4], go[4];
        bool ok[4];
#pragma unroll
        for (int i = 0; i < 4; ++i) {
          ok[i] = rows(64 * h + 16 * wq + 4 * i + sub, yo[i], ro[i], go[i]);
          o[i] = *reinterpret_cast<const float4*>(tbuf + (4 * i + sub) * FRAG_TP_STRIDE + c4);
          o[i].x = fmaf(o[i].x, a.x, b.x), o[i].y = fmaf(o[i].y, a.y, b.y), o[i].z = fmaf(o[i].z, a.z, b.z), o[i].w = fmaf(o[i].w, a.w, b.w);
        }
        if (res) {
          float4 r[4];
#pragma unroll
          for (int i = 0; i < 4; ++i)
            r[i] = !ok[i] ? make_float4(0.f, 0.f, 0.f, 0.f)
                 : res_split ? split_load4(reinterpret_cast<const uint16_t*>(res + ro[i]), c4)
                             : __ldg(reinterpret_cast<const float4*>(res + ro[i] + c4));
#pragma unroll
          for (int i = 0; i < 4; ++i) o[i].x += r[i].x, o[i].y += r[i].y, o[i].z += r[i].z, o[i].w += r[i].w;
        }
        if (act == OSB_ACT_RELU) {
#pragma unroll
          for (int i = 0; i < 4; ++i) o[i].x = fmaxf(o[i].x, 0.f), o[i].y = fmaxf(o[i].y, 0.f), o[i].z = fmaxf(o[i].z, 0.f), o[i].w = fmaxf(o[i].w, 0.f);
        } else if (act == OSB_ACT_LEAKY) {
#pragma unroll
          for (int i = 0; i < 4; ++i) {
            o[i].x = o[i].x > 0.f ? o[i].x : 0.01f * o[i].x, o[i].y = o[i].y > 0.f ? o[i].y : 0.01f * o[i].y;
            o[i].z = o[i].z > 0.f ? o[i].z : 0.01f * o[i].z, o[i].w = o[i].w > 0.f ? o[i].w : 0.01f * o[i].w;
          }
        }
        if (gate) {
          float4 g[4];
#pragma unroll
          for (int i = 0; i < 4; ++i) g[i] = ok[i] ? __ldg(reinterpret_cast<const float4*>(gate + go[i] + c4)) : make_float4(1.f, 1.f, 1.f, 1.f);
#pragma unroll
          for (int i = 0; i < 4; ++i) o[i].x *= g[i].x, o[i].y *= g[i].y, o[i].z *= g[i].z, o[i].w *= g[i].w;
        }
#pragma unroll
        for (int i = 0; i < 4; ++i) {
          if (!ok[i]) continue;
          if (y_split) split_store4(reinterpret_cast<uint16_t*>(y + yo[i]), c4, o[i], amax);
          else *reinterpret_cast<float4*>(y + yo[i] + c4) = o[i];
        }
      }
      if (y_split) tc_report_overflow(overflow, amax);
      return;
    }
  }
#pragma unroll
  for (int h = 0; h < 2; ++h) {
    float2 rv[G / 8][2], gv[G / 8][2];
#pragma unroll
    for (int j = 0; j < G / 8; ++j)
#pragma unroll
      for (int rh = 0; rh < 2; ++rh) {
        const int c = 8 * j + c0;
        ptrdiff_t yo, ro, go;
        const bool live = rows(64 * h + 16 * wq + l4 + 8 * rh, yo, ro, go);
        rv[j][rh] = make_float2(0.f, 0.f);
        gv[j][rh] = make_float2(1.f, 1.f);
        if (res) {
          if (rcs == 1) {
            if (live) rv[j][rh] = __ldg(reinterpret_cast<const float2*>(res + ro + c));
          } else {
            if (live && c < nch) rv[j][rh].x = __ldg(res + ro + (size_t)c * rcs);
            if (live && c + 1 < nch) rv[j][rh].y = __ldg(res + ro + (size_t)(c + 1) * rcs);
          }
        }
        if (gate && live) gv[j][rh] = __ldg(reinterpret_cast<const float2*>(gate + go + c));
      }
#pragma unroll
    for (int j = 0; j < G / 8; ++j) {
      const int c = 8 * j + c0;
      const float2 a = *reinterpret_cast<const float2*>(sc + c);
      const float2 b = *reinterpret_cast<const float2*>(sh + c);
#pragma unroll
      for (int rh = 0; rh < 2; ++rh) {
        ptrdiff_t yo, ro, go;
        const bool live = rows(64 * h + 16 * wq + l4 + 8 * rh, yo, ro, go);
        float v0 = fmaf(acc[h][4 * (j + G / 8) + 2 * rh], a.x, b.x);
        float v1 = fmaf(acc[h][4 * (j + G / 8) + 2 * rh + 1], a.y, b.y);
        if (res) v0 += rv[j][rh].x, v1 += rv[j][rh].y;
        if (act == OSB_ACT_RELU) {
          v0 = fmaxf(v0, 0.f), v1 = fmaxf(v1, 0.f);
        } else if (act == OSB_ACT_LEAKY) {
          v0 = v0 > 0.f ? v0 : 0.01f * v0, v1 = v1 > 0.f ? v1 : 0.01f * v1;
        }
        if (gate) v0 *= gv[j][rh].x, v1 *= gv[j][rh].y;
        if (!live) continue;
        if (ycs == 1) {
          *reinterpret_cast<float2*>(y + yo + c) = make_float2(v0, v1);
        } else {
          if (c < nch) y[yo + (size_t)c * ycs] = v0;
          if (c + 1 < nch) y[yo + (size_t)(c + 1) * ycs] = v1;
        }
      }
    }
  }
}

constexpr int TP_STRIDE = 36;
constexpr int TP_WARP_FLOATS = 32 * TP_STRIDE;

__device__ __forceinline__ void store_ndhwc_chunk32(float* tbuf, int lane, const float (&sum)[32], float* y0, const float* res0,
                                                    size_t vstride, const float* sc, const float* sh, int act,
                                                    uint32_t vmask = 0xffffffffu, const float* gate0 = nullptr) {
  const int c4 = 4 * (lane & 7), sub = lane >> 3;
  __syncwarp();
  float4* row = reinterpret_cast<float4*>(tbuf + lane * TP_STRIDE);
#pragma unroll
  for (int i = 0; i < 8; ++i) row[i] = make_float4(sum[4 * i], sum[4 * i + 1], sum[4 * i + 2], sum[4 * i + 3]);
  __syncwarp();
  const float4 a = *reinterpret_cast<const float4*>(sc + c4);
  const float4 b = *reinterpret_cast<const float4*>(sh + c4);
  float4 o[8];
#pragma unroll
  for (int j = 0; j < 8; ++j) {
    o[j] = *reinterpret_cast<const float4*>(tbuf + (4 * j + sub) * TP_STRIDE + c4);
    o[j].x = fmaf(o[j].x, a.x, b.x), o[j].y = fmaf(o[j].y, a.y, b.y), o[j].z = fmaf(o[j].z, a.z, b.z), o[j].w = fmaf(o[j].w, a.w, b.w);
  }
  if (res0) {
    float4 r[8];
#pragma unroll
    for (int j = 0; j < 8; ++j)
      r[j] = ((vmask >> (4 * j + sub)) & 1u) ? __ldg(reinterpret_cast<const float4*>(res0 + (size_t)(4 * j + sub) * vstride + c4))
                                             : make_float4(0.f, 0.f, 0.f, 0.f);
#pragma unroll
    for (int j = 0; j < 8; ++j) o[j].x += r[j].x, o[j].y += r[j].y, o[j].z += r[j].z, o[j].w += r[j].w;
  }
  if (act == OSB_ACT_RELU) {
#pragma unroll
    for (int j = 0; j < 8; ++j) o[j].x = fmaxf(o[j].x, 0.f), o[j].y = fmaxf(o[j].y, 0.f), o[j].z = fmaxf(o[j].z, 0.f), o[j].w = fmaxf(o[j].w, 0.f);
  } else if (act == OSB_ACT_LEAKY) {
#pragma unroll
    for (int j = 0; j < 8; ++j) {
      o[j].x = o[j].x > 0.f ? o[j].x : 0.01f * o[j].x, o[j].y = o[j].y > 0.f ? o[j].y : 0.01f * o[j].y;
      o[j].z = o[j].z > 0.f ? o[j].z : 0.01f * o[j].z, o[j].w = o[j].w > 0.f ? o[j].w : 0.01f * o[j].w;
    }
  }
  if (gate0) {
#pragma unroll
    for (int j = 0; j < 8; ++j) {
      if (!((vmask >> (4 * j + sub)) & 1u)) continue;
      const float4 g = __ldg(reinterpret_cast<const float4*>(gate0 + (size_t)(4 * j + sub) * vstride + c4));
      o[j].x *= g.x, o[j].y *= g.y, o[j].z *= g.z, o[j].w *= g.w;
    }
  }
#pragma unroll
  for (int j = 0; j < 8; ++j)
    if ((vmask >> (4 * j + sub)) & 1u) *reinterpret_cast<float4*>(y0 + (size_t)(4 * j + sub) * vstride + c4) = o[j];
}

struct TcArgs {
  const float* x;
  const void* w;
  const float* scale;
  const float* shift;
  const float* residual;
  const float* gate;
  float* y;
  int B, Cin, Cout, D, H, W;
  int act, out_ndhwc, res_ndhwc;
  int in_ncdhw;
  int ystride;
  int cout_real;
  float kappa;
  unsigned int* overflow;
  int in_split = 0, out_split = 0, res_split = 0;
  bool slice() const { return ystride != 0 && ystride != Cout; }
};
using TcLaunch = int (*)(const TcArgs&, cudaStream_t);

inline int check_tc_args(const char* what, TcArgs& a, TcLaunch launch) {
  auto aligned = [](const void* p) { return (reinterpret_cast<uintptr_t>(p) & 15) == 0; };
  OSB_REQUIRE(a.x && a.w && a.y, "%s: null pointer", what);
  OSB_REQUIRE(a.B > 0 && a.D > 0 && a.H > 0, "%s: empty shape", what);
  OSB_REQUIRE(a.act >= 0 && a.act <= 2, "%s: unknown activation %d", what, a.act);
  OSB_REQUIRE(aligned(a.x) && aligned(a.w) && aligned(a.y) && aligned(a.residual) && aligned(a.gate),
              "%s: pointers must be 16-byte aligned", what);
  const bool channels_last = a.out_ndhwc && (!a.residual || a.res_ndhwc);
  OSB_REQUIRE(a.ystride == 0 || (a.ystride >= a.Cout && a.ystride % 4 == 0 && channels_last),
              "%s: a channel slice (ystride %d) needs channels-last tensors", what, a.ystride);
  OSB_REQUIRE(!a.gate || channels_last, "%s: the gate operand needs a channels-last output (and residual)", what);
  OSB_REQUIRE(a.cout_real == a.Cout || (a.cout_real >= 1 && a.cout_real < a.Cout && !a.out_ndhwc && (!a.residual || !a.res_ndhwc)),
              "%s: only NCDHW tensors may hold fewer (%d) channels than the packed %d", what, a.cout_real, a.Cout);
  if (!launch) {
    set_error("%s: no instantiation serves Cout=%d W=%d with gate=%d ystride=%d", what, a.Cout, a.W, a.gate != nullptr, a.ystride);
    return OSB_EUNSUPPORTED;
  }
  a.kappa = rz_kappa();
  a.overflow = tc_overflow_flag();
  return a.overflow ? OSB_OK : OSB_ECUDA;
}

template <auto KERNEL, class P>
int launch_persistent(const TcArgs& a, P p, long long items, size_t smem, const char* variant, cudaStream_t stream) {
  OSB_REQUIRE(items < (1ll << 31), "%s: too many work items", variant);
  static PerDeviceFlag configured;
  if (!configured.here()) {
    const cudaError_t e = cudaFuncSetAttribute(KERNEL, cudaFuncAttributeMaxDynamicSharedMemorySize, (int)smem);
    if (e != cudaSuccess) {
      set_error("%s: cannot reserve %zu bytes of shared memory: %s", variant, smem, cudaGetErrorString(e));
      return OSB_ECUDA;
    }
    configured.here() = true;
  }
  p.x = a.x, p.w = a.w, p.scale = a.scale, p.shift = a.shift, p.residual = a.residual, p.y = a.y;
  p.B = a.B, p.D = a.D, p.H = a.H, p.Cin = a.Cin, p.act = a.act, p.out_ndhwc = a.out_ndhwc, p.res_ndhwc = a.res_ndhwc;
  p.kappa = a.kappa, p.overflow = a.overflow;
  p.items = (int)items;
  const int sms = sm_count();
  set_tc_variant(variant);
  KERNEL<<<(int)cap_persistent_grid(p.items < sms ? p.items : sms), TC_WG_THREADS, smem, stream>>>(p);
  count_launch();
  const cudaError_t e = cudaGetLastError();
  if (e != cudaSuccess) {
    cudaFuncAttributes fa{};
    (void)cudaFuncGetAttributes(&fa, KERNEL);
    set_error("%s: launch failed: %s (threads %d, kernel maxThreadsPerBlock %d, regs %d, static smem %zu, dynamic smem %zu, "
              "max dynamic %d)", variant, cudaGetErrorString(e), TC_WG_THREADS, fa.maxThreadsPerBlock, fa.numRegs,
              fa.sharedSizeBytes, smem, fa.maxDynamicSharedSizeBytes);
    return OSB_ECUDA;
  }
  return OSB_OK;
}

struct TcRoute {
  TcLaunch launch;
  int kc;
};
TcRoute select_conv3d_tc(int Cin, int Cout, int W, int dilation, bool gate, bool slice);
template <int COUT>
int launch_tc(const TcArgs& a, cudaStream_t stream);

}
```

openstereo_b200/host_models.py:

```python
import torch
import torch.nn as nn
import torch.nn.functional as F

from . import aggregation as _agg
from . import ops
from .aggregation import GwcAggregation, PSMAggregation


USE_TC_BACKBONE = True


def _cfg_get(cfgs, key, default=None):
    if isinstance(cfgs, dict):
        return cfgs.get(key, default)
    return getattr(cfgs, key, default)


def _cb(cin, cout, k, stride, pad, dilation, bias=False):
    return nn.Sequential(nn.Conv2d(cin, cout, kernel_size=k, stride=stride, padding=dilation if dilation > 1 else pad,
                                   dilation=dilation, bias=bias), nn.BatchNorm2d(cout))


def _front_tc_ok(net, x):
    return (getattr(net, "_osb_folded", False) and x.is_cuda and x.dim() == 4 and x.shape[2] == 2 * ops.TC_WIDTH and x.shape[3] % 2 == 0
            and _agg.USE_TENSOR_CORES and USE_TC_BACKBONE and x.dtype == torch.float32 and ops.conv3d_tc_kc(32, 32, ops.TC_WIDTH) == 32)


def _front_tc(net, x):
    convs = [m for m in net.firstconv.modules() if isinstance(m, nn.Conv2d)]
    blocks = list(net.layer1.children())
    y = F.relu(convs[0](x))
    t = y.permute(0, 3, 2, 1).contiguous()
    t = _tc2d(net, convs[2], _tc2d(net, convs[1], t, ops.ACT_RELU, transpose=True), ops.ACT_RELU, transpose=True)
    for i, blk in enumerate(blocks):
        c1, c2 = _block_convs(blk)
        assert blk.downsample is None
        t = _tc2d(net, c2, _tc2d(net, c1, t, ops.ACT_RELU, transpose=True), ops.ACT_NONE, residual=t, last=(i == len(blocks) - 1),
                  transpose=True)
    return t.transpose(2, 3).contiguous()


def _tc2d(net, conv, t, act, residual=None, last=False, transpose=False):
    cache = net.__dict__.setdefault("_osb_tc2d", {})
    dil = conv.dilation[0]
    if id(conv) not in cache:
        assert conv.kernel_size == (3, 3) and conv.stride == (1, 1) and conv.padding == (dil, dil) and conv.dilation == (dil, dil)
        w5 = torch.zeros(conv.out_channels, conv.in_channels, 3, 3, 3, dtype=torch.float32, device=conv.weight.device)
        w2 = conv.weight.detach().float()
        w5[:, :, 1] = w2.transpose(2, 3) if transpose else w2
        kc = ops.conv2d_tc_kc(conv.in_channels, conv.out_channels, ops.TC_WIDTH, dil)
        cache[id(conv)] = (ops.pack_tc_weight(w5, kc), None if conv.bias is None else conv.bias.detach().float().contiguous())
    wp, bias = cache[id(conv)]
    return ops.conv2d_k3_tc(t, wp, None, bias, residual, act, dil, out_nhwc=not last, res_nhwc=True)


def _block_convs(blk):
    c1 = [m for m in blk.conv1.modules() if isinstance(m, nn.Conv2d)][0]
    c2 = [m for m in blk.conv2.modules() if isinstance(m, nn.Conv2d)][0]
    return c1, c2


def _block_tc_ok(blk, c):
    if blk.downsample is not None:
        return False
    c1, c2 = _block_convs(blk)
    dil = c1.dilation[0]
    return all(cv.kernel_size == (3, 3) and cv.stride == (1, 1) and cv.dilation == (dil, dil) and cv.padding == (dil, dil)
               and cv.in_channels == c and cv.out_channels == c for cv in (c1, c2)) and ops.conv2d_tc_kc(c, c, ops.TC_WIDTH, dil) != 0


def _stage_tc(net, stage, x):
    blocks = list(stage.children())
    usable = getattr(net, "_osb_folded", False) and x.is_cuda and x.dtype == torch.float32 and _agg.USE_TENSOR_CORES and USE_TC_BACKBONE
    y, rest = x, blocks
    if not (usable and x.shape[3] == ops.TC_WIDTH and _block_tc_ok(blocks[0], x.shape[1])):
        y, rest = blocks[0](x), blocks[1:]
    c = y.shape[1]
    if not (usable and rest and y.shape[3] == ops.TC_WIDTH and all(_block_tc_ok(b, c) for b in rest)):
        for b in rest:
            y = b(y)
        return y
    t = ops.to_ndhwc(y.unsqueeze(2).contiguous()).squeeze(1)
    for i, b in enumerate(rest):
        c1, c2 = _block_convs(b)
        t = _tc2d(net, c2, _tc2d(net, c1, t, ops.ACT_RELU), ops.ACT_NONE, residual=t, last=(i == len(rest) - 1))
    return t


def _lastconv_tc_ok(net, x):
    convs = [m for m in net.lastconv.modules() if isinstance(m, nn.Conv2d)]
    return (getattr(net, "_osb_folded", False) and x.is_cuda and x.dtype == torch.float32 and _agg.USE_TENSOR_CORES and USE_TC_BACKBONE
            and x.shape[3] == ops.TC_WIDTH and len(convs) == 2 and convs[0].kernel_size == (3, 3) and convs[0].stride == (1, 1)
            and convs[0].dilation == (1, 1) and convs[0].padding == (1, 1) and convs[1].kernel_size == (1, 1)
            and ops.conv2d_tc_kc(convs[0].in_channels, convs[0].out_channels, ops.TC_WIDTH, 1) != 0)


def _lastconv_tc(net, x):
    convs = [m for m in net.lastconv.modules() if isinstance(m, nn.Conv2d)]
    t = ops.to_ndhwc(x.unsqueeze(2).contiguous()).squeeze(1)
    return convs[1](_tc2d(net, convs[0], t, ops.ACT_RELU, last=True))


def gwc_extract(net, x):
    x = _front_tc(net, x) if _front_tc_ok(net, x) else net.layer1(net.firstconv(x))
    l2 = _stage_tc(net, net.layer2, x)
    l3 = _stage_tc(net, net.layer3, l2)
    l4 = _stage_tc(net, net.layer4, l3)
    gwc = torch.cat((l2, l3, l4), dim=1)
    out = {"gwc_feature": gwc}
    if net.concat_feature:
        out["concat_feature"] = _lastconv_tc(net, gwc) if _lastconv_tc_ok(net, gwc) else net.lastconv(gwc)
    return out


def psm_extract(net, x):
    o2 = _front_tc(net, x) if _front_tc_ok(net, x) else net.layer1(net.firstconv(x))
    o4_0 = _stage_tc(net, net.layer2, o2)
    o8 = _stage_tc(net, net.layer4, _stage_tc(net, net.layer3, o4_0))
    size = (o8.size()[2], o8.size()[3])
    up = [F.interpolate(getattr(net, "branch%d" % i)(o8), size, mode="bilinear", align_corners=True) for i in (1, 2, 3, 4)]
    cat = torch.cat((o4_0, o8, up[3], up[2], up[1], up[0]), 1)
    return _lastconv_tc(net, cat) if _lastconv_tc_ok(net, cat) else net.lastconv(cat)


class _ResBlock(nn.Module):

    def __init__(self, conv1, conv2, downsample):
        super().__init__()
        self.conv1, self.conv2, self.downsample = conv1, conv2, downsample

    def forward(self, x):
        out = self.conv2(self.conv1(x))
        if self.downsample is not None:
            x = self.downsample(x)
        out += x
        return out


def _stage(make_block, make_down, inplanes, planes, blocks, stride):
    down = make_down(inplanes, planes, stride) if (stride != 1 or inplanes != planes) else None
    layers = [make_block(inplanes, planes, stride, down)]
    layers += [make_block(planes, planes, 1, None) for _ in range(1, blocks)]
    return nn.Sequential(*layers)


class _GwcFeatureExtraction(nn.Module):
    def __init__(self, concat_feature, concat_channels):
        super().__init__()
        self.concat_feature = concat_feature
        r = lambda: nn.ReLU(inplace=True)
        self.firstconv = nn.Sequential(_cb(3, 32, 3, 2, 1, 1), r(), _cb(32, 32, 3, 1, 1, 1), r(), _cb(32, 32, 3, 1, 1, 1), r())

        def block(dil):
            return lambda i, o, s, d: _ResBlock(nn.Sequential(_cb(i, o, 3, s, 1, dil), r()), _cb(o, o, 3, 1, 1, dil), d)

        down = lambda i, o, s: nn.Sequential(nn.Conv2d(i, o, kernel_size=1, stride=s, bias=False), nn.BatchNorm2d(o))
        self.layer1 = _stage(block(1), down, 32, 32, 3, 1)
        self.layer2 = _stage(block(1), down, 32, 64, 16, 2)
        self.layer3 = _stage(block(1), down, 64, 128, 3, 1)
        self.layer4 = _stage(block(2), down, 128, 128, 3, 1)
        if concat_feature:
            self.lastconv = nn.Sequential(_cb(320, 128, 3, 1, 1, 1), r(),
                                          nn.Conv2d(128, concat_channels, kernel_size=1, padding=0, stride=1, bias=False))

    def forward(self, x):
        return gwc_extract(self, x)


# ... 245 lines not shown
```

openstereo_b200/ops.py:

```python
import math

import torch

from . import _lib

ACT_NONE, ACT_RELU, ACT_LEAKY, ACT_RELU6 = 0, 1, 2, 3
TC_WIDTH = 128
TC_KC = 32


_LAUNCH_DEVICE = [None]


def _stream(t):
    _LAUNCH_DEVICE[0] = t.device.index
    return torch.cuda.current_stream(t.device).cuda_stream


def _same_device(*tensors):
    devs = {t.device for t in tensors if t is not None}
    if len(devs) > 1:
        raise RuntimeError("openstereo_b200: operands live on different devices: %s" % sorted(str(d) for d in devs))


# ... 533 lines not shown
    w = w.contiguous()
    hi = w.to(torch.float16)
    lo = (w - hi.float()).to(torch.float16)
    return hi, lo


class TcWeight:
    __slots__ = ("data", "inv", "kc", "cout", "cout_real", "ksize", "_eff")

    def __init__(self, data, inv, kc, cout, cout_real=None, ksize=3):
        self.data, self.inv, self.kc, self.cout, self._eff = data, inv, kc, cout, None
        self.cout_real = cout if cout_real is None else cout_real
        self.ksize = ksize

    def eff_scale(self, scale):
        key = None if scale is None else (scale.data_ptr(), scale._version)
        if self._eff is None or self._eff[0] != key:
            if scale is not None and scale.numel() < self.inv.numel():
                scale = torch.cat((scale.float(), scale.new_ones(self.inv.numel() - scale.numel()).float()))
            eff = self.inv if scale is None else scale.float() * self.inv
            self._eff = (key, eff.contiguous())
        return self._eff[1]


def pack_tc_weight(weight, kc=None, kw_order=(0, 1, 2), pad_cout_to=None):
    w = weight.detach().float()
    cout_real, cin = w.shape[:2]
    k = int(w.shape[2])
    if pad_cout_to is not None and cout_real < pad_cout_to:
        w = torch.cat((w, w.new_zeros((pad_cout_to - cout_real,) + tuple(w.shape[1:]))), 0)
    cout = w.shape[0]
    kc = TC_KC if kc is None else kc
    assert kc in (16, 32) and cin % kc == 0 and k in (3, 4) and tuple(w.shape[2:]) == (k, k, k) and len(kw_order) == k
    amax = w.abs().amax(dim=(1, 2, 3, 4))
    _, ex = torch.frexp(amax)
    e = torch.where(amax > 0, TC_WEIGHT_TOP_LOG2 - ex, torch.zeros_like(ex)).clamp(-40, 40)
    ws = torch.ldexp(w, e.view(-1, 1, 1, 1, 1))
    hi, lo = f16_split(ws)
    both = torch.stack((hi, lo), 0)
    both = both[..., list(kw_order)]
    both = both.contiguous().view(2, cout, cin // kc, kc, k, k, k)
    both = both.permute(4, 2, 5, 6, 1, 0, 3)
    data = both.reshape(k, cin // kc, k, k * cout, 2 * kc).contiguous()
    cpr = (2 * kc) // 8
    rows = torch.arange(k * cout, device=data.device)
    key = (rows & 7) if kc == 32 else ((rows >> 1) & 3)
    src = torch.arange(cpr, device=data.device).view(1, cpr) ^ key.view(-1, 1)
    data = data.view(k, cin // kc, k, k * cout, cpr, 8)
    data = torch.gather(data, 4, src.view(1, 1, 1, k * cout, cpr, 1).expand(k, cin // kc, k, k * cout, cpr, 8).contiguous())
    data = data.reshape(k, cin // kc, k, k * cout, 2 * kc).contiguous()
    inv = torch.ldexp(torch.ones_like(amax), -(e + TC_ACT_SCALE_LOG2))
    return TcWeight(data, inv.contiguous(), kc, cout, cout_real, ksize=k)


def _tc_args(w_split, cin, kc, scale):
    assert isinstance(w_split, TcWeight) and w_split.kc == kc
    k = w_split.ksize
    assert tuple(w_split.data.shape) == (k, cin // kc, k, k * w_split.cout, 2 * kc) and w_split.data.dtype == torch.float16
    assert w_split.data.is_contiguous() and w_split.data.is_cuda
    return w_split.data.data_ptr(), w_split.eff_scale(scale)


def to_ndhwc(x, pad_to=None):
    assert x.is_cuda and x.dtype == torch.float32 and x.is_contiguous() and x.dim() == 5
    b, c, d, h, w = x.shape
    cp = c if pad_to is None else int(pad_to)
    assert cp >= c
    y = torch.empty((b, d, h, w, cp), dtype=torch.float32, device=x.device)
    if cp == c:
        _call("osb_ncdhw_to_ndhwc", x.data_ptr(), y.data_ptr(), b, c, d, h, w, _stream(y))
    else:
        _call("osb_ncdhw_to_ndhwc_pad", x.data_ptr(), y.data_ptr(), b, c, cp, d, h, w, _stream(y))
    return y


SPLIT_GRANULE = 16
LAYOUT_NCDHW, LAYOUT_NDHWC, LAYOUT_SPLIT = 0, 1, 2


def is_split(t):
    return t.dtype == torch.float16 and t.dim() == 5


def to_split(x):
    assert x.is_cuda and x.dtype == torch.float32 and x.is_contiguous() and x.dim() == 5
    b, c, d, h, w = x.shape
    assert c % SPLIT_GRANULE == 0, "split activations need a multiple of %d channels" % SPLIT_GRANULE
    y = torch.empty((b, d, h, w, 2 * c), dtype=torch.float16, device=x.device)
    _call("osb_ncdhw_to_split", x.data_ptr(), y.data_ptr(), b, c, d, h, w, _stream(y))
    return y


def from_split(x_split):
    assert is_split(x_split) and x_split.shape[4] % (2 * SPLIT_GRANULE) == 0
    g = x_split.shape[4] // (2 * SPLIT_GRANULE)
    v = x_split.view(*x_split.shape[:4], g, 2, SPLIT_GRANULE).float()
    return ((v[..., 0, :] + v[..., 1, :]) * (1.0 / 16)).reshape(*x_split.shape[:4], g * SPLIT_GRANULE).contiguous()


def conv3d_k3_tc(x_ndhwc, w_split, scale=None, shift=None, residual=None, act=ACT_NONE, out_ndhwc=True, res_ndhwc=True,
                 in_ncdhw=False, gate=None, out_split=False):
    assert x_ndhwc.is_cuda and x_ndhwc.dtype in (torch.float32, torch.float16) and x_ndhwc.is_contiguous() and x_ndhwc.dim() == 5
    in_split = is_split(x_ndhwc)
    assert not (in_split and in_ncdhw)
    if in_ncdhw:
        b, cin, d, h, w = x_ndhwc.shape
    else:
        b, d, h, w, cin = x_ndhwc.shape
        if in_split:
            cin = w_split.data.shape[1] * w_split.kc
            if x_ndhwc.shape[4] != 2 * cin:
                raise ValueError("conv3d_k3_tc: an fp16 input is read as split activations (ops.to_split), 2 * Cin = %d entries per "
                                 "voxel for this weight; got %d" % (2 * cin, x_ndhwc.shape[4]))
    cout = w_split.cout_real
    kc = conv3d_tc_kc(cin, cout, w)
    assert kc
    wptr, scale = _tc_args(w_split, cin, kc, scale)
    if shift is not None and shift.numel() < w_split.cout:
        shift = torch.cat((shift.float(), shift.new_zeros(w_split.cout - shift.numel()).float()))
    res_split = residual is not None and is_split(residual)
    if residual is not None:
        want = (b, d, h, w, 2 * cout if res_split else cout) if res_ndhwc else (b, cout, d, h, w)
        assert tuple(residual.shape) == want and residual.is_contiguous() and (res_split or residual.dtype == torch.float32)
    if in_split or out_split or res_split:
        assert gate is None and (out_ndhwc or not out_split)
        shape = (b, d, h, w, 2 * cout if out_split else cout) if out_ndhwc else (b, cout, d, h, w)
        y = torch.empty(shape, dtype=torch.float16 if out_split else torch.float32, device=x_ndhwc.device)
        layout = lambda split, ndhwc: LAYOUT_SPLIT if split else (LAYOUT_NDHWC if ndhwc else LAYOUT_NCDHW)
        _call("osb_conv3d_k3_tc_split_fwd", x_ndhwc.data_ptr(), wptr, _ptr(scale), _ptr(shift), _ptr(residual), y.data_ptr(),
              b, cin, cout, d, h, w, act, layout(in_split, not in_ncdhw), layout(out_split, out_ndhwc), layout(res_split, res_ndhwc),
              _stream(y), profile_as="osb_conv3d_k3_tc_ncdhw_fwd" if in_ncdhw else "osb_conv3d_k3_tc_fwd")
        return y
    shape = (b, d, h, w, cout) if out_ndhwc else (b, cout, d, h, w)
    y = torch.empty(shape, dtype=torch.float32, device=x_ndhwc.device)
    assert not in_ncdhw or kc == 32
    if gate is not None:
        assert kc == 16 and out_ndhwc and res_ndhwc and not in_ncdhw
        assert tuple(gate.shape) == (b, h, w, cout) and gate.is_contiguous() and gate.dtype == torch.float32 and gate.is_cuda
        _call("osb_conv3d_k3_tc_gate_fwd", x_ndhwc.data_ptr(), wptr, _ptr(scale), _ptr(shift), _ptr(residual), gate.data_ptr(),
              y.data_ptr(), b, cin, cout, d, h, w, act, _stream(y))
        return y
    _call("osb_conv3d_k3_tc_ncdhw_fwd" if in_ncdhw else "osb_conv3d_k3_tc_fwd", x_ndhwc.data_ptr(), wptr, _ptr(scale), _ptr(shift), _ptr(residual),
          y.data_ptr(), b, cin, cout, d, h, w, act, 1 if out_ndhwc else 0, 1 if res_ndhwc else 0, _stream(y))
    return y


def conv3d_s2_tc_supported(cin, cout, d, h, w):
    return bool(_lib.lib.osb_conv3d_s2_tc_supported(int(cin), int(cout), int(d), int(h), int(w)))


def conv3d_k3_s2_tc(x_ndhwc, w_split, scale=None, shift=None, residual=None, act=ACT_NONE, out_ndhwc=False, res_ndhwc=False):
    assert x_ndhwc.is_cuda and x_ndhwc.dtype == torch.float32 and x_ndhwc.is_contiguous() and x_ndhwc.dim() == 5
    b, d, h, w, cin = x_ndhwc.shape
    cout = w_split.cout
    wptr, scale = _tc_args(w_split, cin, 16, scale)
    do, ho, wo = d // 2, h // 2, w // 2
    shape = (b, do, ho, wo, cout) if out_ndhwc else (b, cout, do, ho, wo)
    y = torch.empty(shape, dtype=torch.float32, device=x_ndhwc.device)
    if residual is not None:
        want = (b, do, ho, wo, cout) if res_ndhwc else (b, cout, do, ho, wo)
        assert tuple(residual.shape) == want and residual.is_contiguous()
    _call("osb_conv3d_k3_s2_tc_fwd", x_ndhwc.data_ptr(), wptr, _ptr(scale), _ptr(shift), _ptr(residual),
          y.data_ptr(), b, cin, cout, d, h, w, act, 1 if out_ndhwc else 0, 1 if res_ndhwc else 0, _stream(y))
    return y


def deconv3d_tc_supported(cin, cout, w):
    return bool(_lib.lib.osb_deconv3d_tc_supported(int(cin), int(cout), int(w)))


def pack_tc_deconv_weight(weight):
    w = weight.detach().float().permute(1, 0, 2, 3, 4).contiguous()
    return pack_tc_weight(w, 16, kw_order=(1, 2, 0) if w.shape[2] == 3 else (1, 3, 2, 0))


def deconv3d_k4_tc_supported(cin, cout, w):
    return bool(_lib.lib.osb_deconv3d_k4_tc_supported(int(cin), int(cout), int(w)))


def deconv3d_k4_tc(x_ndhwc, w_split, scale=None, shift=None, residual=None, act=ACT_NONE, out_ndhwc=True, res_ndhwc=True,
                   cout_real=None):
    assert x_ndhwc.is_cuda and x_ndhwc.dtype == torch.float32 and x_ndhwc.is_contiguous() and x_ndhwc.dim() == 5
    b, d, h, w, cin = x_ndhwc.shape
    cout = w_split.cout
    creal = cout if cout_real is None else int(cout_real)
    assert w_split.ksize == 4 and (out_ndhwc is False or creal == cout)
    wptr, scale = _tc_args(w_split, cin, 16, scale)
    shape = (b, 2 * d, 2 * h, 2 * w, cout) if out_ndhwc else (b, creal, 2 * d, 2 * h, 2 * w)
    y = torch.empty(shape, dtype=torch.float32, device=x_ndhwc.device)
    if residual is not None:
        want = (b, 2 * d, 2 * h, 2 * w, cout) if res_ndhwc else (b, creal, 2 * d, 2 * h, 2 * w)
        assert tuple(residual.shape) == want and residual.is_contiguous()
    _call("osb_deconv3d_k4_tc_fwd", x_ndhwc.data_ptr(), wptr, _ptr(scale), _ptr(shift), _ptr(residual),
          y.data_ptr(), b, cin, cout, creal, d, h, w, act, 1 if out_ndhwc else 0, 1 if res_ndhwc else 0, _stream(y))
    return y


def tc_slice(kind, x_ndhwc, w_split, scale, shift, y, coff, act=ACT_NONE, gate=None):
    assert x_ndhwc.is_cuda and x_ndhwc.dtype == torch.float32 and x_ndhwc.is_contiguous() and x_ndhwc.dim() == 5
    assert y.is_contiguous() and y.dtype == torch.float32 and y.dim() == 5
    b, d, h, w, cin = x_ndhwc.shape
    cout, ctot = w_split.cout, y.shape[-1]
    assert 0 <= coff and coff + cout <= ctot and coff % 4 == 0
    wptr, scale = _tc_args(w_split, cin, 16, scale)
    yp = y.data_ptr() + 4 * coff
    if kind == "s1":
        assert tuple(y.shape[:4]) == (b, d, h, w)
        gp = None
        if gate is not None:
            assert tuple(gate.shape) == (b, h, w, ctot) and gate.is_contiguous()
            gp = gate.data_ptr() + 4 * coff
        _call("osb_conv3d_k3_tc_cs_fwd", x_ndhwc.data_ptr(), wptr, _ptr(scale), _ptr(shift), None, gp, yp, b, cin, cout, d, h, w, act,
              ctot, _stream(y))
    elif kind == "s2":
        assert tuple(y.shape[:4]) == (b, d // 2, h // 2, w // 2) and gate is None
        _call("osb_conv3d_k3_s2_tc_cs_fwd", x_ndhwc.data_ptr(), wptr, _ptr(scale), _ptr(shift), yp, b, cin, cout, d, h, w, act, ctot,
              _stream(y))
    else:
        assert kind == "dc4" and tuple(y.shape[:4]) == (b, 2 * d, 2 * h, 2 * w) and gate is None and w_split.ksize == 4
        _call("osb_deconv3d_k4_tc_cs_fwd", x_ndhwc.data_ptr(), wptr, _ptr(scale), _ptr(shift), yp, b, cin, cout, d, h, w, act, ctot,
              _stream(y))
    return y


def feature_att_gate(feat, w1, scale1, shift1, w2, scale2, shift2, pad_to=None, act1=ACT_LEAKY):
    assert feat.is_cuda and feat.dtype == torch.float32 and feat.is_contiguous() and feat.dim() == 4
    b, cf, h, w = feat.shape
    ch, cv = w1.shape[1], w2.shape[1]
    assert w1.shape[0] == cf and w2.shape[0] == ch and w1.is_contiguous() and w2.is_contiguous()
    cp = cv if pad_to is None else int(pad_to)
    gate = torch.empty((b, h, w, cp), dtype=torch.float32, device=feat.device)
    _call("osb_feature_att_gate_fwd", feat.data_ptr(), w1.data_ptr(), _ptr(scale1), _ptr(shift1), w2.data_ptr(), _ptr(scale2),
          _ptr(shift2), gate.data_ptr(), b, cf, ch, cv, cp, h * w, act1, _stream(gate))
    return gate


def conv1x1_ndhwc_cat(x0, x1, w_packed, scale=None, shift=None, act=ACT_NONE):
    assert x0.is_cuda and x0.dtype == torch.float32 and x0.is_contiguous() and x1.is_contiguous() and x0.shape[:-1] == x1.shape[:-1]
    c0, c1 = x0.shape[-1], x1.shape[-1]
    cin, cout = w_packed.shape
    assert cin == c0 + c1 and w_packed.is_contiguous()
    y = torch.empty(x0.shape[:-1] + (cout,), dtype=torch.float32, device=x0.device)
    _call("osb_conv1x1_ndhwc_cat_fwd", x0.data_ptr(), x1.data_ptr(), c0, c1, w_packed.data_ptr(), _ptr(scale), _ptr(shift),
          y.data_ptr(), x0.numel() // c0, cout, act, _stream(y))
# ... 37 lines not shown
    y = torch.empty((b, 1, d, h, w), dtype=torch.float32, device=x_ndhwc.device)
    _call("osb_conv3d_k3_c1_ndhwc_fwd", x_ndhwc.data_ptr(), w_taps.data_ptr(), _ptr(scale), _ptr(shift), y.data_ptr(), b, cin, d, h, w,
          _stream(y))
    return y


def dwconv2d(x, weight, scale=None, shift=None, residual=None, stride=1, act=ACT_NONE, out=None):
    assert x.is_cuda and x.dtype == torch.float32 and x.is_contiguous() and x.dim() == 4
    b, c, h, w = x.shape
    kh, kw = weight.shape[-2:]
    wt = weight.detach().float().reshape(c, kh, kw).contiguous()
    ho, wo = (h - 1) // stride + 1, (w - 1) // stride + 1
    y = torch.empty((b, c, ho, wo), dtype=torch.float32, device=x.device) if out is None else out
    if residual is not None:
        assert residual.shape == y.shape and residual.is_contiguous()
    _call("osb_dwconv2d_fwd", x.data_ptr(), wt.data_ptr(), _ptr(scale), _ptr(shift), _ptr(residual), y.data_ptr(), b, c, h, w,
          int(kh), int(kw), int(stride), act, _stream(y))
    return y


def pack_deconv2d_weight(weight):
    ci, co = weight.shape[:2]
    assert tuple(weight.shape[2:]) == (3, 3)
    return weight.detach().float().permute(0, 2, 3, 1).reshape(ci, 9, co).contiguous()


def deconv2d_k3s2(x, w_packed, scale=None, shift=None, residual=None, act=ACT_NONE):
    assert x.is_cuda and x.dtype == torch.float32 and x.is_contiguous() and x.dim() == 4
    b, cin, h, w = x.shape
    assert w_packed.shape[0] == cin and w_packed.shape[1] == 9
    cout = w_packed.shape[2]
    y = torch.empty((b, cout, 2 * h, 2 * w), dtype=torch.float32, device=x.device)
    if residual is not None:
        assert residual.shape == y.shape and residual.is_contiguous()
    _call("osb_deconv2d_k3s2_fwd", x.data_ptr(), w_packed.data_ptr(), _ptr(scale), _ptr(shift), _ptr(residual), y.data_ptr(), b, cin,
          cout, h, w, act, _stream(y))
    return y


def avgpool_pairs(x, axis):
    assert x.is_cuda and x.dtype == torch.float32 and x.is_contiguous()
    axis = axis % x.dim()
    n = x.shape[axis]
    outer, inner = math.prod(x.shape[:axis]), math.prod(x.shape[axis + 1:])
    y = torch.empty(x.shape[:axis] + (n // 2,) + x.shape[axis + 1:], dtype=torch.float32, device=x.device)
    _call("osb_avgpool_pairs_fwd", x.data_ptr(), y.data_ptr(), outer, n, inner, _stream(y))
    return y


def geo_lookup(geo_levels, corr_levels, disp, coords, radius):
    levels = len(geo_levels)
    assert levels == len(corr_levels) and 1 <= levels <= 4
    b, c, d, h, w = geo_levels[0].shape
    w2 = corr_levels[0].shape[-1]
    for i in range(levels):
        g, cr = geo_levels[i], corr_levels[i]
        assert g.is_cuda and g.dtype == torch.float32 and g.is_contiguous() and tuple(g.shape) == (b, c, d >> i, h, w)
        assert cr.is_cuda and cr.dtype == torch.float32 and cr.is_contiguous() and tuple(cr.shape) == (b, h, w, w2 >> i)
    disp = disp.contiguous().float()
    coords = coords.reshape(b, h, w).contiguous().float()
    assert tuple(disp.shape) == (b, 1, h, w)
    out = torch.empty((b, levels * (c + 1) * (2 * radius + 1), h, w), dtype=torch.float32, device=disp.device)
    gp = [geo_levels[i].data_ptr() if i < levels else None for i in range(4)]
    cp = [corr_levels[i].data_ptr() if i < levels else None for i in range(4)]
    _call("osb_geo_lookup_fwd", *gp, *cp, disp.data_ptr(), coords.data_ptr(), out.data_ptr(), b, c, d, h, w, w2, levels, radius,
          _stream(out))
    return out


def context_upsample(disp_low, up_weights, scale_factor=4):
    assert disp_low.is_cuda and disp_low.dim() == 4 and disp_low.shape[1] == 1
    b, _, h, w = disp_low.shape
    assert tuple(up_weights.shape) == (b, 9, h * scale_factor, w * scale_factor)
    disp_low, up_weights = disp_low.contiguous().float(), up_weights.contiguous().float()
    out = torch.empty((b, h * scale_factor, w * scale_factor), dtype=torch.float32, device=disp_low.device)
    _call("osb_context_upsample_fwd", disp_low.data_ptr(), up_weights.data_ptr(), out.data_ptr(), b, h, w, scale_factor, _stream(out))
    return out


def conv2d_tc_kc(cin, cout, w, dilation=1):
    return int(_lib.lib.osb_conv2d_tc_kc(int(cin), int(cout), int(w), int(dilation)))


def conv2d_k3_tc(x_nhwc, w_split, scale=None, shift=None, residual=None, act=ACT_NONE, dilation=1, out_nhwc=True, res_nhwc=True):
    assert x_nhwc.is_cuda and x_nhwc.dtype == torch.float32 and x_nhwc.is_contiguous() and x_nhwc.dim() == 4
    b, h, w, cin = x_nhwc.shape
    cout = w_split.cout
    kc = conv2d_tc_kc(cin, cout, w, dilation)
    assert kc
    wptr, scale = _tc_args(w_split, cin, kc, scale)
    y = torch.empty((b, h, w, cout) if out_nhwc else (b, cout, h, w), dtype=torch.float32, device=x_nhwc.device)
    if residual is not None:
        assert residual.is_contiguous() and residual.numel() == y.numel()
    _call("osb_conv2d_k3_tc_fwd", x_nhwc.data_ptr(), wptr, _ptr(scale), _ptr(shift), _ptr(residual), y.data_ptr(), b, cin,
          cout, h, w, dilation, act, int(out_nhwc), int(res_nhwc), _stream(y))
    return y
```

Before: 298.0.

## Extend split fp16 activation layout to stride-2 convs, tcg kernel, and 2D backbone

Adds split-layout (pre-split fp16 hi/lo pairs) support to the stride-2 conv3d path, the tcg kernel (loaded by TMA with multi-row boxes), and the 2D residual backbone convs. Hourglass stride-2 convs now emit split outputs when the next conv can consume them, and wide 2D backbone blocks chain split activations between convs. The aim is to drop the per-layer fp32-to-split conversion in loader warps and halve activation traffic. In exchange the code paths and route checks get more complex, with overflow reporting on split stores.

```diff
diff --git a/include/openstereo_b200.h b/include/openstereo_b200.h
--- a/include/openstereo_b200.h
+++ b/include/openstereo_b200.h
@@ -91,6 +91,7 @@
 #define OSB_LAYOUT_NDHWC 1
 #define OSB_LAYOUT_SPLIT 2
 int osb_ncdhw_to_split(const float* x, float* y_split, int B, int C, int D, int H, int W, osb_stream_t stream);
+int osb_conv3d_tc_split_ok(int Cin, int Cout, int W, int dilation);
 int osb_conv3d_k3_tc_split_fwd(const float* x, const void* w_split, const float* scale, const float* shift, const float* residual,
                                float* y, int B, int Cin, int Cout, int D, int H, int W, int act, int in_layout, int out_layout,
                                int res_layout, osb_stream_t stream);
@@ -98,6 +99,9 @@
 int osb_conv3d_k3_s2_tc_fwd(const float* x_ndhwc, const void* w_split, const float* scale, const float* shift,
                             const float* residual, float* y, int B, int Cin, int Cout, int D, int H, int W, int act,
                             int out_ndhwc, int res_ndhwc, osb_stream_t stream);
+int osb_conv3d_k3_s2_tc_split_fwd(const float* x_ndhwc, const void* w_split, const float* scale, const float* shift,
+                                  const float* residual, float* y, int B, int Cin, int Cout, int D, int H, int W, int act,
+                                  int out_layout, int res_layout, osb_stream_t stream);
 int osb_deconv3d_tc_supported(int Cin, int Cout, int W);
 int osb_deconv3d_k3_tc_fwd(const float* x_ndhwc, const void* w_split, const float* scale, const float* shift,
                            const float* residual, float* y, int B, int Cin, int Cout, int D, int H, int W, int act,
@@ -123,6 +127,9 @@
 int osb_conv2d_k3_tc_fwd(const float* x_nhwc, const void* w_split, const float* scale, const float* shift, const float* residual,
                          float* y, int B, int Cin, int Cout, int H, int W, int dilation, int act, int out_nhwc, int res_nhwc,
                          osb_stream_t stream);
+int osb_conv2d_k3_tc_split_fwd(const float* x, const void* w_split, const float* scale, const float* shift, const float* residual,
+                               float* y, int B, int Cin, int Cout, int H, int W, int dilation, int act, int in_layout, int out_layout,
+                               int res_layout, osb_stream_t stream);
 int osb_gwc_volume_sum_fwd(const float* ref, const float* tgt, float* out, int B, int C, int H, int W, int D, int G,
                            osb_stream_t stream);
 int osb_group_l2_normalize_fwd(const float* x, float* y, int B, int C, int H, int W, int G, float eps, osb_stream_t stream);
diff --git a/openstereo_b200/_lib.py b/openstereo_b200/_lib.py
--- a/openstereo_b200/_lib.py
+++ b/openstereo_b200/_lib.py
@@ -30,6 +30,9 @@
     "osb_conv3d_k3_tc_fwd": [_f32p] * 6 + [_i] * 9 + [_s],
     "osb_conv3d_k3_tc_ncdhw_fwd": [_f32p] * 6 + [_i] * 9 + [_s],
     "osb_conv3d_k3_tc_split_fwd": [_f32p] * 6 + [_i] * 10 + [_s],
+    "osb_conv2d_k3_tc_split_fwd": [_f32p] * 6 + [_i] * 10 + [_s],
+    "osb_conv3d_k3_s2_tc_split_fwd": [_f32p] * 6 + [_i] * 9 + [_s],
+    "osb_conv3d_tc_split_ok": [_i] * 4,
     "osb_ncdhw_to_split": [_f32p, _f32p] + [_i] * 5 + [_s],
     "osb_conv3d_k3_tc_gate_fwd": [_f32p] * 7 + [_i] * 7 + [_s],
     "osb_deconv3d_k4_tc_supported": [_i, _i, _i],
diff --git a/openstereo_b200/aggregation.py b/openstereo_b200/aggregation.py
--- a/openstereo_b200/aggregation.py
+++ b/openstereo_b200/aggregation.py
@@ -83,7 +83,11 @@
 
 
 def _split_chain_ok(width, *layers):
-    return USE_TENSOR_CORES and all(ops.conv3d_tc_kc(l.cin, l.cout, width) == 32 for l in layers)
+    return width == ops.TC_WIDTH and all(_split_in_ok(width, l) for l in layers)
+
+
+def _split_in_ok(width, layer):
+    return USE_TENSOR_CORES and ops.conv3d_tc_split_ok(layer.cin, layer.cout, width)
 
 
 def _stem_in(layer, volume, act, out_split=False):
@@ -187,9 +191,12 @@
 
 
 def _gwc_hourglass_channels_last(hg, x):
-    c1 = ops.conv3d_k3_s2_tc(x, _s2_weight(hg.conv1), hg.conv1.scale, hg.conv1.shift, None, ACT_RELU, out_ndhwc=True)
+    w = x.shape[3]
+    c1 = ops.conv3d_k3_s2_tc(x, _s2_weight(hg.conv1), hg.conv1.scale, hg.conv1.shift, None, ACT_RELU, out_ndhwc=True,
+                             out_split=_split_in_ok(w // 2, hg.conv2))
     c2 = _conv_tc(hg.conv2, c1, ACT_RELU)
-    c3 = ops.conv3d_k3_s2_tc(c2, _s2_weight(hg.conv3), hg.conv3.scale, hg.conv3.shift, None, ACT_RELU, out_ndhwc=True)
+    c3 = ops.conv3d_k3_s2_tc(c2, _s2_weight(hg.conv3), hg.conv3.scale, hg.conv3.shift, None, ACT_RELU, out_ndhwc=True,
+                             out_split=_split_in_ok(w // 4, hg.conv4))
     c4 = _conv_tc(hg.conv4, c3, ACT_RELU)
     r2 = ops.conv1x1_ndhwc(c2, hg.redir2.w, hg.redir2.scale, hg.redir2.shift)
     c5 = ops.deconv3d_k3_tc(c4, _dc_weight(hg.conv5), hg.conv5.scale, hg.conv5.shift, r2, ACT_RELU, out_ndhwc=True, res_ndhwc=True)
@@ -296,9 +303,12 @@
 
 
 def _psm_hourglass_channels_last(hg, x, presqu, postsqu, skip):
-    out = ops.conv3d_k3_s2_tc(x, _s2_weight(hg.conv1), hg.conv1.scale, hg.conv1.shift, None, ACT_RELU, out_ndhwc=True)
+    w = x.shape[3]
+    out = ops.conv3d_k3_s2_tc(x, _s2_weight(hg.conv1), hg.conv1.scale, hg.conv1.shift, None, ACT_RELU, out_ndhwc=True,
+                              out_split=_split_in_ok(w // 2, hg.conv2))
     pre = _conv_tc(hg.conv2, out, ACT_RELU, residual=postsqu)
-    out = ops.conv3d_k3_s2_tc(pre, _s2_weight(hg.conv3), hg.conv3.scale, hg.conv3.shift, None, ACT_RELU, out_ndhwc=True)
+    out = ops.conv3d_k3_s2_tc(pre, _s2_weight(hg.conv3), hg.conv3.scale, hg.conv3.shift, None, ACT_RELU, out_ndhwc=True,
+                              out_split=_split_in_ok(w // 4, hg.conv4))
     out = _conv_tc(hg.conv4, out, ACT_RELU)
     post = ops.deconv3d_k3_tc(out, _dc_weight(hg.conv5), hg.conv5.scale, hg.conv5.shift, presqu if presqu is not None else pre, ACT_RELU,
                               out_ndhwc=True, res_ndhwc=True)
diff --git a/openstereo_b200/csrc/api.cu b/openstereo_b200/csrc/api.cu
--- a/openstereo_b200/csrc/api.cu
+++ b/openstereo_b200/csrc/api.cu
@@ -124,7 +124,7 @@
   return true;
 }
 
-bool make_tensor_map_split(CUtensorMap* out, const void* base, int C, int W, int H, int BD, int kc) {
+bool make_tensor_map_split(CUtensorMap* out, const void* base, int C, int W, int H, int BD, int kc, int rows) {
   EncodeTiledFn fn = encode_fn();
   if (!fn) {
     set_error("cuTensorMapEncodeTiled not available from the driver");
@@ -133,7 +133,7 @@
   const uint64_t vox = 2ull * C * sizeof(uint16_t);
   const cuuint64_t dims[4] = {2ull * C, (cuuint64_t)W, (cuuint64_t)H, (cuuint64_t)BD};
   const cuuint64_t strides[3] = {vox, vox * W, vox * W * H};
-  const cuuint32_t box[4] = {2u * kc, (cuuint32_t)W, 1, 1};
+  const cuuint32_t box[4] = {2u * kc, (cuuint32_t)W, (cuuint32_t)rows, 1};
   const cuuint32_t elem[4] = {1, 1, 1, 1};
   CUresult r = fn(out, CU_TENSOR_MAP_DATA_TYPE_FLOAT16, 4, const_cast<void*>(base), dims, strides, box, elem,
                   CU_TENSOR_MAP_INTERLEAVE_NONE, kc == 32 ? CU_TENSOR_MAP_SWIZZLE_128B : CU_TENSOR_MAP_SWIZZLE_64B,
diff --git a/openstereo_b200/csrc/common.cuh b/openstereo_b200/csrc/common.cuh
--- a/openstereo_b200/csrc/common.cuh
+++ b/openstereo_b200/csrc/common.cuh
@@ -84,6 +84,6 @@
 
 bool make_tensor_map_3d(CUtensorMap* out, const void* base, uint64_t d0, uint64_t d1, uint64_t d2, uint64_t stride1_bytes,
                         uint64_t stride2_bytes, uint32_t box0, uint32_t box1, uint32_t box2);
-bool make_tensor_map_split(CUtensorMap* out, const void* base, int C, int W, int H, int BD, int kc);
+bool make_tensor_map_split(CUtensorMap* out, const void* base, int C, int W, int H, int BD, int kc, int rows);
 
 }
diff --git a/openstereo_b200/csrc/conv3d_tc.cu b/openstereo_b200/csrc/conv3d_tc.cu
--- a/openstereo_b200/csrc/conv3d_tc.cu
+++ b/openstereo_b200/csrc/conv3d_tc.cu
@@ -389,7 +389,7 @@
   p.Cout = a.Cout, p.in_ncdhw = a.in_ncdhw;
   p.in_split = a.in_split, p.out_split = a.out_split, p.res_split = a.res_split;
   p.bulk_rows = !a.in_split && (a.in_ncdhw || a.Cin == TC_KC);
-  if (a.in_split && !make_tensor_map_split(&p.xmap, a.x, a.Cin, TC_W, a.H, a.B * a.D, TC_KC)) return OSB_ECUDA;
+  if (a.in_split && !make_tensor_map_split(&p.xmap, a.x, a.Cin, TC_W, a.H, a.B * a.D, TC_KC, 1)) return OSB_ECUDA;
   p.hblocks = (a.H + TC_TILES - 1) / TC_TILES;
   static const std::string variant = tc_variant_name("tc<%d>", COUT);
   return launch_persistent<conv3d_tc_kernel<COUT>>(a, p, (long long)a.B * a.D * p.hblocks, TcCfg<COUT>::SMEM, variant.c_str(), stream);
@@ -445,15 +445,18 @@
   OSB_REQUIRE(!a.in_ncdhw || kc == 32, "conv3d_k3_tc: NCDHW input is served by the W = 128 kernel only");
   OSB_REQUIRE((!a.ystride && !a.gate) || kc == 16, "conv3d_k3_tc: a channel slice or gate needs the 16-channel-chunk kernels");
   OSB_REQUIRE(a.Cout > 16 || (!a.out_ndhwc && (!a.residual || !a.res_ndhwc)), "conv3d_k3_tc: Cout <= 16 writes (and adds) NCDHW tensors only");
-  OSB_REQUIRE(!(a.in_split || a.out_split || a.res_split) || (kc == 32 && !a.ystride && !a.gate),
-              "conv3d_k3_tc: split activations are served by the W = 128 kernel only");
+  const TcRoute route = select_conv3d_tc(a.Cin, a.Cout, a.W, dilation, a.gate != nullptr, a.slice());
+  OSB_REQUIRE(!(a.in_split || a.out_split || a.res_split) || !route.launch || route.split,
+              "conv3d_k3_tc: split activations need a whole-row tile without gate or channel slice (Cin=%d Cout=%d W=%d, gate=%d, "
+              "ystride=%d)", a.Cin, a.Cout, a.W, a.gate != nullptr, a.ystride);
+  OSB_REQUIRE(!(a.out_split || a.res_split) || a.W == 128,
+              "conv3d_k3_tc: W = %d layers read split input and write fp32; as an output or residual, split activations are served "
+              "by the W = 128 kernel only (conv3d_tc, or conv3d_tcg for Cout = 64 | 128)", a.W);
   OSB_REQUIRE(!a.in_split || !a.in_ncdhw, "conv3d_k3_tc: an input is either NCDHW or split");
   OSB_REQUIRE((!a.out_split || a.out_ndhwc) && (!a.res_split || a.res_ndhwc), "conv3d_k3_tc: split tensors are channels-last");
-  OSB_REQUIRE(!(a.out_split || a.res_split) || (a.out_ndhwc && (!a.residual || a.res_ndhwc)),
-              "conv3d_k3_tc: a split output or residual needs a channels-last output and residual");
-  const TcLaunch launch = select_conv3d_tc(a.Cin, a.Cout, a.W, dilation, a.gate != nullptr, a.slice()).launch;
-  const int rc = check_tc_args("conv3d_k3_tc", a, launch);
-  return rc != OSB_OK ? rc : launch(a, (cudaStream_t)stream);
+  OSB_REQUIRE(!a.out_split || !a.residual || a.res_ndhwc, "conv3d_k3_tc: a split output needs a channels-last residual");
+  const int rc = check_tc_args("conv3d_k3_tc", a, route.launch);
+  return rc != OSB_OK ? rc : route.launch(a, (cudaStream_t)stream);
 }
 
 int osb_conv3d_k3_tc_fwd(const float* x_ndhwc, const void* w_split, const float* scale, const float* shift,
@@ -485,15 +488,33 @@
                             Cout}, 1, stream);
 }
 
+static int conv3d_k3_tc_layouts(const char* what, const float* x, const void* w_split, const float* scale, const float* shift,
+                                const float* residual, float* y, int B, int Cin, int Cout, int D, int H, int W, int dilation, int act,
+                                int in_layout, int out_layout, int res_layout, osb_stream_t stream) {
+  auto known = [](int l) { return l == OSB_LAYOUT_NCDHW || l == OSB_LAYOUT_NDHWC || l == OSB_LAYOUT_SPLIT; };
+  OSB_REQUIRE(known(in_layout) && known(out_layout) && known(res_layout), "%s: unknown layout", what);
+  osb::TcArgs a{x, w_split, scale, shift, residual, nullptr, y, B, Cin, Cout, D, H, W, act, out_layout != OSB_LAYOUT_NCDHW, res_layout != OSB_LAYOUT_NCDHW,
+                in_layout == OSB_LAYOUT_NCDHW, 0, Cout};
+  a.in_split = in_layout == OSB_LAYOUT_SPLIT, a.out_split = out_layout == OSB_LAYOUT_SPLIT, a.res_split = res_layout == OSB_LAYOUT_SPLIT;
+  return conv3d_k3_tc_impl(a, dilation, stream);
+}
+
 int osb_conv3d_k3_tc_split_fwd(const float* x, const void* w_split, const float* scale, const float* shift, const float* residual,
                                float* y, int B, int Cin, int Cout, int D, int H, int W, int act, int in_layout, int out_layout,
                                int res_layout, osb_stream_t stream) {
-  auto known = [](int l) { return l == OSB_LAYOUT_NCDHW || l == OSB_LAYOUT_NDHWC || l == OSB_LAYOUT_SPLIT; };
-  OSB_REQUIRE(known(in_layout) && known(out_layout) && known(res_layout), "conv3d_k3_tc_split: unknown layout");
-  osb::TcArgs a{x, w_split, scale, shift, residual, nullptr, y, B, Cin, Cout, D, H, W, act, out_layout != OSB_LAYOUT_NCDHW, res_layout != OSB_LAYOUT_NCDHW,
-                in_layout == OSB_LAYOUT_NCDHW, 0, Cout};
-  a.in_split = in_layout == OSB_LAYOUT_SPLIT, a.out_split = out_layout == OSB_LAYOUT_SPLIT, a.res_split = res_layout == OSB_LAYOUT_SPLIT;
-  return conv3d_k3_tc_impl(a, 1, stream);
+  return conv3d_k3_tc_layouts("conv3d_k3_tc_split", x, w_split, scale, shift, residual, y, B, Cin, Cout, D, H, W, 1, act, in_layout,
+                              out_layout, res_layout, stream);
+}
+
+int osb_conv2d_k3_tc_split_fwd(const float* x, const void* w_split, const float* scale, const float* shift, const float* residual,
+                               float* y, int B, int Cin, int Cout, int H, int W, int dilation, int act, int in_layout, int out_layout,
+                               int res_layout, osb_stream_t stream) {
+  return conv3d_k3_tc_layouts("conv2d_k3_tc_split", x, w_split, scale, shift, residual, y, B, Cin, Cout, 1, H, W, dilation, act,
+                              in_layout, out_layout, res_layout, stream);
+}
+
+int osb_conv3d_tc_split_ok(int Cin, int Cout, int W, int dilation) {
+  return osb::select_conv3d_tc(Cin, Cout, W, dilation, false, false).split ? 1 : 0;
 }
 
 int osb_conv2d_tc_kc(int Cin, int Cout, int W, int dilation) { return osb::select_conv3d_tc(Cin, Cout, W, dilation, false, false).kc; }
diff --git a/openstereo_b200/csrc/conv3d_tcg.cu b/openstereo_b200/csrc/conv3d_tcg.cu
--- a/openstereo_b200/csrc/conv3d_tcg.cu
+++ b/openstereo_b200/csrc/conv3d_tcg.cu
@@ -3,6 +3,7 @@
 namespace osb {
 
 struct TcgParams {
+  CUtensorMap xmap;
   const float* x;
   const void* w;
   const float* scale;
@@ -18,6 +19,7 @@
   int items, hblocks;
   int Wr, ctiles;
   int ystride;
+  int in_split, out_split, res_split;
 };
 
 template <int COUT, int KC, int W, int TILES, int DIL = 1, bool GW = false>
@@ -82,7 +84,7 @@
 };
 
 template <int COUT, int KC, int W, int TILES, int DIL = 1, bool GW = false, bool GATE = false>
-__global__ void __launch_bounds__(TcgCfg<COUT, KC, W, TILES, DIL, GW>::THREADS, 1) conv3d_tcg_kernel(const TcgParams p) {
+__global__ void __launch_bounds__(TcgCfg<COUT, KC, W, TILES, DIL, GW>::THREADS, 1) conv3d_tcg_kernel(const __grid_constant__ TcgParams p) {
   using C = TcgCfg<COUT, KC, W, TILES, DIL, GW>;
   extern __shared__ __align__(1024) uint8_t smem_raw[];
   uint8_t* smem = reinterpret_cast<uint8_t*>((reinterpret_cast<uintptr_t>(smem_raw) + 1023) & ~static_cast<uintptr_t>(1023));
@@ -106,7 +108,7 @@
 
   if (threadIdx.x == 0) {
     for (int s = 0; s < C::STAGES; ++s) {
-      mbar_init(&a_ready[s], 32);
+      mbar_init(&a_ready[s], p.in_split ? 1 : 32);
       mbar_init(&a_empty[s], 4 * TC_WGS);
     }
     for (int k = 0; k < TC_BSLOTS * 3; ++k) {
@@ -199,11 +201,37 @@
       };
       frag_epilogue<C::G>(acc, lane, q, tiles + warp * FRAG_TP_FLOATS, s_scale + cg, s_shift + cg, p.act, p.y + (p.out_ndhwc ? (size_t)cg : cg * plane),
                           p.out_ndhwc ? 1 : plane, p.residual ? p.residual + (p.res_ndhwc ? (size_t)cg : cg * plane) : nullptr,
-                          p.res_ndhwc ? 1 : plane, (GATE && p.gate) ? p.gate + cg : nullptr, rows, C::G);
+                          p.res_ndhwc ? 1 : plane, (GATE && p.gate) ? p.gate + cg : nullptr, rows, C::G, p.out_split, p.res_split,
+                          p.overflow);
     }
   }
   else if (warp < 4 * TC_WGS + C::NLW) {
     setmaxnreg_dec<TC_LOADER_REGS>();
+    if (!GW && !GATE && p.in_split) {
+      if (warp == 4 * TC_WGS && elect_one()) {
+        uint32_t u = 0;
+        for (int it = blockIdx.x; it < p.items; it += gridDim.x) {
+          const int it0 = it / C::NG;
+          const int hb = it0 % p.hblocks;
+          const int d = (it0 / p.hblocks) % p.D;
+          const int b = it0 / (p.hblocks * p.D);
+          for (int kd = 0; kd < 3; ++kd) {
+            const int din = d + kd - 1;
+            if (din < 0 || din >= p.D) continue;
+            for (int ch = 0; ch < nchunk; ++ch)
+              for (int j = 0; j < C::NU; ++j, ++u) {
+                const uint32_t slot = u % C::STAGES, ph = (u / C::STAGES) & 1;
+                mbar_wait_relaxed(&a_empty[slot], ph ^ 1);
+                mbar_arrive_expect_tx(&a_ready[slot], C::UNIT_BYTES);
+                tma_load_4d(a_buf + slot * C::UNIT_BYTES, &p.xmap, &a_ready[slot], 2 * KC * ch, 0, C::row0(hb) + C::unit_s(j),
+                            b * p.D + din);
+              }
+          }
+        }
+      }
+      __syncwarp();
+      return;
+    }
     const int lw = warp - 4 * TC_WGS;
     static_assert(KC == 16, "lane_voxel / unit-row mapping below is written for 64-byte operand rows");
     constexpr int CPR = KC / 4;
@@ -293,6 +321,8 @@
   using C = TcgCfg<COUT, KC, W, TILES, DIL, GW>;
   TcgParams p{};
   p.gate = a.gate, p.ystride = a.ystride;
+  p.in_split = a.in_split, p.out_split = a.out_split, p.res_split = a.res_split;
+  if (a.in_split && !make_tensor_map_split(&p.xmap, a.x, a.Cin, W, a.H, a.B * a.D, KC, C::R)) return OSB_ECUDA;
   p.hblocks = C::hblocks(a.H);
   p.Wr = GW ? a.W : W;
   p.ctiles = GW ? (a.W + C::CSTEP - 1) / C::CSTEP : 1;
@@ -303,34 +333,34 @@
 
 TcRoute select_conv3d_tc(int Cin, int Cout, int W, int dilation, bool gate, bool slice) {
   if (dilation == 1 && W == 128 && Cin % 32 == 0 && Cin >= 32 && !gate && !slice) {
-    if (Cout == 32) return {launch_tc<32>, 32};
-    if (Cout >= 1 && Cout <= 16) return {launch_tc<16>, 32};
+    if (Cout == 32) return {launch_tc<32>, 32, true};
+    if (Cout >= 1 && Cout <= 16) return {launch_tc<16>, 32, true};
   }
   if (Cin % 16 != 0 || Cin < 16) return {};
   if (dilation == 2)
-    return (W == 128 && Cout == 128 && !gate && !slice) ? TcRoute{launch_tcg<128, 16, 128, 1, 2>, 16} : TcRoute{};
+    return (W == 128 && Cout == 128 && !gate && !slice) ? TcRoute{launch_tcg<128, 16, 128, 1, 2>, 16, true} : TcRoute{};
   if (dilation != 1) return {};
   if (W == 16) {
-    if (Cout == 96) return {launch_tcg<96, 16, 16, 1, 1, false, true>, 16};
-    if (Cout == 64) return {launch_tcg<64, 16, 16, 1, 1, false, true>, 16};
+    if (Cout == 96) return {launch_tcg<96, 16, 16, 1, 1, false, true>, 16, false};
+    if (Cout == 64) return {launch_tcg<64, 16, 16, 1, 1, false, true>, 16, false};
     return {};
   }
   if (slice) return {};
   if (gate) {
-    if (W == 64 && Cout == 64) return {launch_tcg<64, 16, 64, 1, 1, false, true>, 16};
-    if (W == 32 && Cout == 96) return {launch_tcg<96, 16, 32, 1, 1, false, true>, 16};
+    if (W == 64 && Cout == 64) return {launch_tcg<64, 16, 64, 1, 1, false, true>, 16, false};
+    if (W == 32 && Cout == 96) return {launch_tcg<96, 16, 32, 1, 1, false, true>, 16, false};
     return {};
   }
-  if (W == 64 && Cout == 64) return {launch_tcg<64, 16, 64, 1>, 16};
-  if (W == 32 && Cout == 64) return {launch_tcg<64, 16, 32, 1>, 16};
-  if (W == 32 && Cout == 128) return {launch_tcg<128, 16, 32, 1>, 16};
-  if (W == 32 && Cout == 96) return {launch_tcg<96, 16, 32, 1>, 16};
-  if (W == 128 && Cout == 64) return {launch_tcg<64, 16, 128, 1>, 16};
-  if (W == 128 && Cout == 128) return {launch_tcg<128, 16, 128, 1>, 16};
+  if (W == 64 && Cout == 64) return {launch_tcg<64, 16, 64, 1>, 16, true};
+  if (W == 32 && Cout == 64) return {launch_tcg<64, 16, 32, 1>, 16, true};
+  if (W == 32 && Cout == 128) return {launch_tcg<128, 16, 32, 1>, 16, true};
+  if (W == 32 && Cout == 96) return {launch_tcg<96, 16, 32, 1>, 16, false};
+  if (W == 128 && Cout == 64) return {launch_tcg<64, 16, 128, 1>, 16, true};
+  if (W == 128 && Cout == 128) return {launch_tcg<128, 16, 128, 1>, 16, true};
   if (!osb_tc_general_width(W)) return {};
-  if (Cout == 32) return {launch_tcg<32, 16, 128, 1, 1, true>, 16};
-  if (Cout == 64) return {launch_tcg<64, 16, 128, 1, 1, true>, 16};
-  if (Cout == 128) return {launch_tcg<128, 16, 128, 1, 1, true>, 16};
+  if (Cout == 32) return {launch_tcg<32, 16, 128, 1, 1, true>, 16, false};
+  if (Cout == 64) return {launch_tcg<64, 16, 128, 1, 1, true>, 16, false};
+  if (Cout == 128) return {launch_tcg<128, 16, 128, 1, 1, true>, 16, false};
   return {};
 }
 
diff --git a/openstereo_b200/csrc/conv3d_tcs2.cu b/openstereo_b200/csrc/conv3d_tcs2.cu
--- a/openstereo_b200/csrc/conv3d_tcs2.cu
+++ b/openstereo_b200/csrc/conv3d_tcs2.cu
@@ -17,6 +17,7 @@
   int items, hblocks;
   int Wr, ctiles;
   int ystride;
+  int out_split;
 };
 
 template <int COUT, int KC, int W, int TILES, bool GW = false>
@@ -221,7 +222,8 @@
       const uint32_t vm = (W < 32) ? __ballot_sync(0xffffffffu, live) : (live ? vmask : 0u);
       if (vm && p.out_ndhwc && (!p.residual || p.res_ndhwc)) {
         store_ndhwc_chunk32(stage + q * 32 * C::LD, lane, out, p.y + (vox - lane) * YS + cg,
-                            p.residual ? p.residual + (vox - lane) * YS + cg : nullptr, YS, s_scale + cg, s_shift + cg, p.act, vm);
+                            p.residual ? p.residual + (vox - lane) * YS + cg : nullptr, YS, s_scale + cg, s_shift + cg, p.act, vm,
+                            nullptr, p.out_split, p.overflow);
       } else if (live && cvalid) {
 #pragma unroll
         for (int i = 0; i < 32; ++i) out[i] = fmaf(out[i], s_scale[cg + i], s_shift[cg + i]);
@@ -351,7 +353,7 @@
 static int launch_tcs2(const TcArgs& a, cudaStream_t stream) {
   using C = Tcs2Cfg<COUT, KC, W, TILES, GW>;
   Tcs2Params p{};
-  p.ystride = a.ystride;
+  p.ystride = a.ystride, p.out_split = a.out_split;
   p.hblocks = (a.H / 2 + C::HBLK - 1) / C::HBLK;
   p.Wr = GW ? a.W / 2 : W;
   p.ctiles = GW ? (p.Wr + C::CSTEP - 1) / C::CSTEP : 1;
@@ -378,6 +380,8 @@
 static int conv3d_k3_s2_tc_impl(TcArgs a, cudaStream_t stream) {
   OSB_REQUIRE(select_conv3d_s2_tc(a.Cin, a.Cout, a.D, a.H, a.W, false), "conv3d_k3_s2_tc: unsupported shape Cin=%d Cout=%d D=%d H=%d W=%d",
               a.Cin, a.Cout, a.D, a.H, a.W);
+  OSB_REQUIRE(!a.out_split || (a.out_ndhwc && (!a.residual || a.res_ndhwc) && !a.slice()),
+              "conv3d_k3_s2_tc: a split output needs channels-last tensors and no channel slice");
   const TcLaunch launch = select_conv3d_s2_tc(a.Cin, a.Cout, a.D, a.H, a.W, a.slice());
   const int rc = check_tc_args("conv3d_k3_s2_tc", a, launch);
   return rc != OSB_OK ? rc : launch(a, stream);
@@ -398,6 +402,18 @@
                                     0, 0, Cout}, (cudaStream_t)stream);
 }
 
+int osb_conv3d_k3_s2_tc_split_fwd(const float* x_ndhwc, const void* w_split, const float* scale, const float* shift,
+                                  const float* residual, float* y, int B, int Cin, int Cout, int D, int H, int W, int act,
+                                  int out_layout, int res_layout, osb_stream_t stream) {
+  OSB_REQUIRE((out_layout == OSB_LAYOUT_NCDHW || out_layout == OSB_LAYOUT_NDHWC || out_layout == OSB_LAYOUT_SPLIT) &&
+                  (res_layout == OSB_LAYOUT_NCDHW || res_layout == OSB_LAYOUT_NDHWC),
+              "conv3d_k3_s2_tc_split: unknown layout (the input and residual are fp32)");
+  osb::TcArgs a{x_ndhwc, w_split, scale, shift, residual, nullptr, y, B, Cin, Cout, D, H, W, act, out_layout != OSB_LAYOUT_NCDHW,
+                res_layout != OSB_LAYOUT_NCDHW, 0, 0, Cout};
+  a.out_split = out_layout == OSB_LAYOUT_SPLIT;
+  return osb::conv3d_k3_s2_tc_impl(a, (cudaStream_t)stream);
+}
+
 int osb_conv3d_k3_s2_tc_cs_fwd(const float* x_ndhwc, const void* w_split, const float* scale, const float* shift, float* y, int B,
                                int Cin, int Cout, int D, int H, int W, int act, int ystride, osb_stream_t stream) {
   return osb::conv3d_k3_s2_tc_impl({x_ndhwc, w_split, scale, shift, nullptr, nullptr, y, B, Cin, Cout, D, H, W, act, 1, 1, 0, ystride,
diff --git a/openstereo_b200/csrc/tc_common.cuh b/openstereo_b200/csrc/tc_common.cuh
--- a/openstereo_b200/csrc/tc_common.cuh
+++ b/openstereo_b200/csrc/tc_common.cuh
@@ -211,6 +211,12 @@
   const float2 h01 = f16x2_to_float2(hi.x), h23 = f16x2_to_float2(hi.y), l01 = f16x2_to_float2(lo.x), l23 = f16x2_to_float2(lo.y);
   constexpr float inv = 1.f / TC_ACT_SCALE;
   return make_float4((h01.x + l01.x) * inv, (h01.y + l01.y) * inv, (h23.x + l23.x) * inv, (h23.y + l23.y) * inv);
+}
+__device__ __forceinline__ float2 split_load2(const uint16_t* vox, int c) {
+  const float2 h = f16x2_to_float2(__ldg(reinterpret_cast<const unsigned int*>(vox + split_index(c))));
+  const float2 l = f16x2_to_float2(__ldg(reinterpret_cast<const unsigned int*>(vox + split_index(c) + SPLIT_GRANULE)));
+  constexpr float inv = 1.f / TC_ACT_SCALE;
+  return make_float2((h.x + l.x) * inv, (h.y + l.y) * inv);
 }
 
 template <int KC>
@@ -375,7 +381,8 @@
         gv[j][rh] = make_float2(1.f, 1.f);
         if (res) {
           if (rcs == 1) {
-            if (live) rv[j][rh] = __ldg(reinterpret_cast<const float2*>(res + ro + c));
+            if (live) rv[j][rh] = res_split ? split_load2(reinterpret_cast<const uint16_t*>(res + ro), c)
+                                            : __ldg(reinterpret_cast<const float2*>(res + ro + c));
           } else {
             if (live && c < nch) rv[j][rh].x = __ldg(res + ro + (size_t)c * rcs);
             if (live && c + 1 < nch) rv[j][rh].y = __ldg(res + ro + (size_t)(c + 1) * rcs);
@@ -418,7 +425,8 @@
 
 __device__ __forceinline__ void store_ndhwc_chunk32(float* tbuf, int lane, const float (&sum)[32], float* y0, const float* res0,
                                                     size_t vstride, const float* sc, const float* sh, int act,
-                                                    uint32_t vmask = 0xffffffffu, const float* gate0 = nullptr) {
+                                                    uint32_t vmask = 0xffffffffu, const float* gate0 = nullptr, bool y_split = false,
+                                                    unsigned int* overflow = nullptr) {
   const int c4 = 4 * (lane & 7), sub = lane >> 3;
   __syncwarp();
   float4* row = reinterpret_cast<float4*>(tbuf + lane * TP_STRIDE);
@@ -460,9 +468,15 @@
       o[j].x *= g.x, o[j].y *= g.y, o[j].z *= g.z, o[j].w *= g.w;
     }
   }
-#pragma unroll
-  for (int j = 0; j < 8; ++j)
-    if ((vmask >> (4 * j + sub)) & 1u) *reinterpret_cast<float4*>(y0 + (size_t)(4 * j + sub) * vstride + c4) = o[j];
+  float amax = 0.f;
+#pragma unroll
+  for (int j = 0; j < 8; ++j) {
+    if (!((vmask >> (4 * j + sub)) & 1u)) continue;
+    float* yv = y0 + (size_t)(4 * j + sub) * vstride;
+    if (y_split) split_store4(reinterpret_cast<uint16_t*>(yv), c4, o[j], amax);
+    else *reinterpret_cast<float4*>(yv + c4) = o[j];
+  }
+  if (y_split) tc_report_overflow(overflow, amax);
 }
 
 struct TcArgs {
@@ -542,6 +556,7 @@
 struct TcRoute {
   TcLaunch launch;
   int kc;
+  bool split;
 };
 TcRoute select_conv3d_tc(int Cin, int Cout, int W, int dilation, bool gate, bool slice);
 template <int COUT>
diff --git a/openstereo_b200/host_models.py b/openstereo_b200/host_models.py
--- a/openstereo_b200/host_models.py
+++ b/openstereo_b200/host_models.py
@@ -8,6 +8,7 @@
 
 
 USE_TC_BACKBONE = True
+SPLIT_MIN_CHANNELS = 128
 
 
 def _cfg_get(cfgs, key, default=None):
@@ -40,7 +41,7 @@
     return t.transpose(2, 3).contiguous()
 
 
-def _tc2d(net, conv, t, act, residual=None, last=False, transpose=False):
+def _tc2d(net, conv, t, act, residual=None, last=False, transpose=False, out_split=False):
     cache = net.__dict__.setdefault("_osb_tc2d", {})
     dil = conv.dilation[0]
     if id(conv) not in cache:
@@ -51,7 +52,7 @@
         kc = ops.conv2d_tc_kc(conv.in_channels, conv.out_channels, ops.TC_WIDTH, dil)
         cache[id(conv)] = (ops.pack_tc_weight(w5, kc), None if conv.bias is None else conv.bias.detach().float().contiguous())
     wp, bias = cache[id(conv)]
-    return ops.conv2d_k3_tc(t, wp, None, bias, residual, act, dil, out_nhwc=not last, res_nhwc=True)
+    return ops.conv2d_k3_tc(t, wp, None, bias, residual, act, dil, out_nhwc=not last, res_nhwc=True, out_split=out_split and not last)
 
 
 def _block_convs(blk):
@@ -81,9 +82,12 @@
             y = b(y)
         return y
     t = ops.to_ndhwc(y.unsqueeze(2).contiguous()).squeeze(1)
+    dil = _block_convs(rest[0])[0].dilation[0]
+    split = c >= SPLIT_MIN_CHANNELS and ops.conv3d_tc_split_ok(c, c, ops.TC_WIDTH, dil)
     for i, b in enumerate(rest):
         c1, c2 = _block_convs(b)
-        t = _tc2d(net, c2, _tc2d(net, c1, t, ops.ACT_RELU), ops.ACT_NONE, residual=t, last=(i == len(rest) - 1))
+        t = _tc2d(net, c2, _tc2d(net, c1, t, ops.ACT_RELU, out_split=split), ops.ACT_NONE, residual=t, last=(i == len(rest) - 1),
+                  out_split=split)
     return t
 
 
diff --git a/openstereo_b200/ops.py b/openstereo_b200/ops.py
--- a/openstereo_b200/ops.py
+++ b/openstereo_b200/ops.py
@@ -639,6 +639,14 @@
     return t.dtype == torch.float16 and t.dim() == 5
 
 
+def conv3d_tc_split_ok(cin, cout, w, dilation=1):
+    return bool(_lib.lib.osb_conv3d_tc_split_ok(int(cin), int(cout), int(w), int(dilation)))
+
+
+def _layout(split, channels_last):
+    return LAYOUT_SPLIT if split else (LAYOUT_NDHWC if channels_last else LAYOUT_NCDHW)
+
+
 def to_split(x):
     assert x.is_cuda and x.dtype == torch.float32 and x.is_contiguous() and x.dim() == 5
     b, c, d, h, w = x.shape
@@ -683,9 +691,8 @@
         assert gate is None and (out_ndhwc or not out_split)
         shape = (b, d, h, w, 2 * cout if out_split else cout) if out_ndhwc else (b, cout, d, h, w)
         y = torch.empty(shape, dtype=torch.float16 if out_split else torch.float32, device=x_ndhwc.device)
-        layout = lambda split, ndhwc: LAYOUT_SPLIT if split else (LAYOUT_NDHWC if ndhwc else LAYOUT_NCDHW)
         _call("osb_conv3d_k3_tc_split_fwd", x_ndhwc.data_ptr(), wptr, _ptr(scale), _ptr(shift), _ptr(residual), y.data_ptr(),
-              b, cin, cout, d, h, w, act, layout(in_split, not in_ncdhw), layout(out_split, out_ndhwc), layout(res_split, res_ndhwc),
+              b, cin, cout, d, h, w, act, _layout(in_split, not in_ncdhw), _layout(out_split, out_ndhwc), _layout(res_split, res_ndhwc),
               _stream(y), profile_as="osb_conv3d_k3_tc_ncdhw_fwd" if in_ncdhw else "osb_conv3d_k3_tc_fwd")
         return y
     shape = (b, d, h, w, cout) if out_ndhwc else (b, cout, d, h, w)
@@ -706,17 +713,23 @@
     return bool(_lib.lib.osb_conv3d_s2_tc_supported(int(cin), int(cout), int(d), int(h), int(w)))
 
 
-def conv3d_k3_s2_tc(x_ndhwc, w_split, scale=None, shift=None, residual=None, act=ACT_NONE, out_ndhwc=False, res_ndhwc=False):
+def conv3d_k3_s2_tc(x_ndhwc, w_split, scale=None, shift=None, residual=None, act=ACT_NONE, out_ndhwc=False, res_ndhwc=False,
+                    out_split=False):
     assert x_ndhwc.is_cuda and x_ndhwc.dtype == torch.float32 and x_ndhwc.is_contiguous() and x_ndhwc.dim() == 5
     b, d, h, w, cin = x_ndhwc.shape
     cout = w_split.cout
     wptr, scale = _tc_args(w_split, cin, 16, scale)
     do, ho, wo = d // 2, h // 2, w // 2
-    shape = (b, do, ho, wo, cout) if out_ndhwc else (b, cout, do, ho, wo)
-    y = torch.empty(shape, dtype=torch.float32, device=x_ndhwc.device)
+    assert out_ndhwc or not out_split
+    shape = (b, do, ho, wo, 2 * cout if out_split else cout) if out_ndhwc else (b, cout, do, ho, wo)
+    y = torch.empty(shape, dtype=torch.float16 if out_split else torch.float32, device=x_ndhwc.device)
     if residual is not None:
         want = (b, do, ho, wo, cout) if res_ndhwc else (b, cout, do, ho, wo)
-        assert tuple(residual.shape) == want and residual.is_contiguous()
+        assert tuple(residual.shape) == want and residual.is_contiguous() and residual.dtype == torch.float32
+    if out_split:
+        _call("osb_conv3d_k3_s2_tc_split_fwd", x_ndhwc.data_ptr(), wptr, _ptr(scale), _ptr(shift), _ptr(residual), y.data_ptr(),
+              b, cin, cout, d, h, w, act, LAYOUT_SPLIT, _layout(False, res_ndhwc), _stream(y), profile_as="osb_conv3d_k3_s2_tc_fwd")
+        return y
     _call("osb_conv3d_k3_s2_tc_fwd", x_ndhwc.data_ptr(), wptr, _ptr(scale), _ptr(shift), _ptr(residual),
           y.data_ptr(), b, cin, cout, d, h, w, act, 1 if out_ndhwc else 0, 1 if res_ndhwc else 0, _stream(y))
     return y
@@ -920,16 +933,32 @@
     return int(_lib.lib.osb_conv2d_tc_kc(int(cin), int(cout), int(w), int(dilation)))
 
 
-def conv2d_k3_tc(x_nhwc, w_split, scale=None, shift=None, residual=None, act=ACT_NONE, dilation=1, out_nhwc=True, res_nhwc=True):
-    assert x_nhwc.is_cuda and x_nhwc.dtype == torch.float32 and x_nhwc.is_contiguous() and x_nhwc.dim() == 4
+def conv2d_k3_tc(x_nhwc, w_split, scale=None, shift=None, residual=None, act=ACT_NONE, dilation=1, out_nhwc=True, res_nhwc=True,
+                 out_split=False):
+    assert x_nhwc.is_cuda and x_nhwc.dtype in (torch.float32, torch.float16) and x_nhwc.is_contiguous() and x_nhwc.dim() == 4
+    in_split = x_nhwc.dtype == torch.float16
     b, h, w, cin = x_nhwc.shape
+    if in_split:
+        cin = w_split.data.shape[1] * w_split.kc
+        if x_nhwc.shape[3] != 2 * cin:
+            raise ValueError("conv2d_k3_tc: an fp16 input is read as split activations, 2 * Cin = %d entries per pixel for this "
+                             "weight; got %d" % (2 * cin, x_nhwc.shape[3]))
     cout = w_split.cout
     kc = conv2d_tc_kc(cin, cout, w, dilation)
     assert kc
     wptr, scale = _tc_args(w_split, cin, kc, scale)
-    y = torch.empty((b, h, w, cout) if out_nhwc else (b, cout, h, w), dtype=torch.float32, device=x_nhwc.device)
+    res_split = residual is not None and residual.dtype == torch.float16
+    assert out_nhwc or not out_split
+    shape = (b, h, w, 2 * cout if out_split else cout) if out_nhwc else (b, cout, h, w)
+    y = torch.empty(shape, dtype=torch.float16 if out_split else torch.float32, device=x_nhwc.device)
     if residual is not None:
-        assert residual.is_contiguous() and residual.numel() == y.numel()
+        assert residual.is_contiguous() and residual.dtype in (torch.float32, torch.float16)
+        assert tuple(residual.shape) == (b, h, w, 2 * cout) and res_nhwc if res_split else residual.numel() == b * h * w * cout
+    if in_split or out_split or res_split:
+        _call("osb_conv2d_k3_tc_split_fwd", x_nhwc.data_ptr(), wptr, _ptr(scale), _ptr(shift), _ptr(residual), y.data_ptr(), b, cin,
+              cout, h, w, dilation, act, _layout(in_split, True), _layout(out_split, out_nhwc), _layout(res_split, res_nhwc),
+              _stream(y), profile_as="osb_conv2d_k3_tc_fwd")
+        return y
     _call("osb_conv2d_k3_tc_fwd", x_nhwc.data_ptr(), wptr, _ptr(scale), _ptr(shift), _ptr(residual), y.data_ptr(), b, cin,
           cout, h, w, dilation, act, int(out_nhwc), int(res_nhwc), _stream(y))
     return y
```

New measurement: 305.2, median of 6. +2.4%, better.
